# microsoft/ANCE

Measured on AMD Instinct MI355X. Metric: passages_encoded_per_sec, higher is better.
Workload: dtype f16 pair operands on the fp16 MFMA, f32 accumulate (fp32-grade: <= 2e-5 from the reference's fp32 forward); 1 GPU; MS MARCO passage 8841823 x 768-d, roberta-base rdot_nll FirstP seq_len=128, encode + brute-force IP top-200 (BASELINE configs[1]); encode_block_per_gpu=16384, query_block=32768, layers=12, parallelism=dp1 (corpus rows sharded, top-k all-to-all by query owner + merge)

## Files before the change

ance_amd/_lib.py:

```python
import ctypes
import os
import subprocess

_HERE = os.path.dirname(os.path.abspath(__file__))
LIB_PATH = os.environ.get("ANCE_AMD_LIB") or os.path.join(_HERE, "libance_amd.so")
CSRC = os.path.join(_HERE, "csrc")

ANCE_OK = 0
ANCE_E_INVALID = -1
ABI_VERSION = 7

c_i32p = ctypes.POINTER(ctypes.c_int32)
c_i64p = ctypes.POINTER(ctypes.c_int64)
c_f32p = ctypes.POINTER(ctypes.c_float)


class AnceEncoderDesc(ctypes.Structure):
    _fields_ = [
        ("arch", ctypes.c_int32), ("n_layers", ctypes.c_int32), ("hidden", ctypes.c_int32),
        ("n_heads", ctypes.c_int32), ("intermediate", ctypes.c_int32), ("vocab_size", ctypes.c_int32),
        ("max_position", ctypes.c_int32), ("pad_token_id", ctypes.c_int32), ("ln_eps", ctypes.c_float),
        ("has_head", ctypes.c_int32), ("max_seq_len", ctypes.c_int32), ("max_tokens", ctypes.c_int32),
        ("precision", ctypes.c_int32),
    ]


class AnceGemmDebugArgs(ctypes.Structure):
    _fields_ = [
        ("a", ctypes.c_void_p), ("b", ctypes.c_void_p), ("lda", ctypes.c_int32), ("ldb", ctypes.c_int32),
        ("M", ctypes.c_int32), ("N", ctypes.c_int32), ("K", ctypes.c_int32),
        ("bias", ctypes.c_void_p), ("csum", ctypes.c_void_p), ("part_in", ctypes.c_void_p), ("ln_eps", ctypes.c_float),
        ("tok_lo", ctypes.c_void_p), ("scale", ctypes.c_float), ("scale_cols", ctypes.c_int32), ("col_map", ctypes.c_void_p),
        ("n_valid", ctypes.c_int32), ("ldc", ctypes.c_int32), ("out", ctypes.c_void_p), ("res_hi", ctypes.c_void_p),
        ("res_lo", ctypes.c_void_p), ("res_gamma", ctypes.c_void_p), ("res_beta", ctypes.c_void_p), ("out_lo", ctypes.c_void_p),
        ("part_out", ctypes.c_void_p), ("ldr", ctypes.c_int32), ("wscale_inv", ctypes.c_void_p), ("n_split", ctypes.c_int32),
    ]


class AnceAttnDebugArgs(ctypes.Structure):
    _fields_ = [
        ("kind", ctypes.c_int32), ("n_heads", ctypes.c_int32), ("n_seq", ctypes.c_int32), ("max_seq_len", ctypes.c_int32),
        ("cls_only", ctypes.c_int32), ("q_compact", ctypes.c_int32), ("h_desc", ctypes.c_void_p), ("d_desc", ctypes.c_void_p),
        ("d_desc_bytes", ctypes.c_int64), ("qk", ctypes.c_void_p), ("ld_qk", ctypes.c_int32), ("qk_rows", ctypes.c_int32),
        ("vt", ctypes.c_void_p), ("ld_vt", ctypes.c_int32), ("ctx", ctypes.c_void_p), ("ld_ctx", ctypes.c_int32),
        ("ctx_rows", ctypes.c_int32),
    ]


class AnceLambTensor(ctypes.Structure):
    _fields_ = [("p", ctypes.c_void_p), ("g", ctypes.c_void_p), ("m", ctypes.c_void_p), ("v", ctypes.c_void_p),
                ("numel", ctypes.c_int64), ("group", ctypes.c_int32), ("reserved", ctypes.c_int32)]


class AnceAdamwTensor(ctypes.Structure):
    _fields_ = [("p", ctypes.c_void_p), ("g", ctypes.c_void_p), ("m", ctypes.c_void_p), ("v", ctypes.c_void_p),
                ("step", ctypes.c_void_p), ("numel", ctypes.c_int64), ("group", ctypes.c_int32), ("reserved", ctypes.c_int32)]


class AnceLambGroup(ctypes.Structure):
    _fields_ = [("lr", ctypes.c_double), ("beta1", ctypes.c_double), ("beta2", ctypes.c_double), ("eps", ctypes.c_double),
                ("weight_decay", ctypes.c_double)]


class AnceGatherSegment(ctypes.Structure):
    _fields_ = [("d_records", ctypes.c_void_p), ("n_records", ctypes.c_int64), ("d_index", ctypes.c_void_p),
                ("n_index", ctypes.c_int64), ("d_ids", ctypes.c_void_p), ("d_mask", ctypes.c_void_p), ("d_types", ctypes.c_void_p),
                ("L", ctypes.c_int32), ("mask_rule", ctypes.c_int32), ("type_rule", ctypes.c_int32), ("reserved", ctypes.c_int32)]


class AnceAttnTrainArgs(ctypes.Structure):
    _fields_ = [("q", ctypes.c_void_p), ("k", ctypes.c_void_p), ("v", ctypes.c_void_p), ("ctx", ctypes.c_void_p),
                ("ld_q", ctypes.c_int32), ("ld_k", ctypes.c_int32), ("ld_v", ctypes.c_int32), ("ld_ctx", ctypes.c_int32),
                ("d_seq_first", ctypes.c_void_p), ("d_seq_len", ctypes.c_void_p), ("n_seq", ctypes.c_int32),
                ("max_seq_len", ctypes.c_int32), ("n_rows", ctypes.c_int32), ("n_heads", ctypes.c_int32),
                ("seq_rows", ctypes.c_int32), ("reserved", ctypes.c_int32),
                ("dropout_p", ctypes.c_float), ("training", ctypes.c_int32), ("seed", ctypes.c_uint64), ("offset", ctypes.c_uint64),
                ("d_workspace", ctypes.c_void_p), ("workspace_bytes", ctypes.c_size_t)]


class AnceAttnGradArgs(ctypes.Structure):
    _fields_ = [("dctx", ctypes.c_void_p), ("dq", ctypes.c_void_p), ("dk", ctypes.c_void_p), ("dv", ctypes.c_void_p),
                ("ld_dctx", ctypes.c_int32), ("ld_dq", ctypes.c_int32), ("ld_dk", ctypes.c_int32), ("ld_dv", ctypes.c_int32)]


ANCE_DTYPE_F32, ANCE_DTYPE_F16, ANCE_DTYPE_BF16 = 0, 1, 2


class AnceAttn16Args(ctypes.Structure):
    _fields_ = [("q", ctypes.c_void_p), ("k", ctypes.c_void_p), ("v", ctypes.c_void_p), ("ctx", ctypes.c_void_p),
                ("ld_q", ctypes.c_int32), ("ld_k", ctypes.c_int32), ("ld_v", ctypes.c_int32), ("ld_ctx", ctypes.c_int32),
                ("d_seq_first", ctypes.c_void_p), ("d_seq_len", ctypes.c_void_p), ("n_seq", ctypes.c_int32),
                ("max_seq_len", ctypes.c_int32), ("n_rows", ctypes.c_int32), ("n_heads", ctypes.c_int32),
                ("seq_rows", ctypes.c_int32), ("dtype", ctypes.c_int32),
                ("dropout_p", ctypes.c_float), ("training", ctypes.c_int32), ("seed", ctypes.c_uint64), ("offset", ctypes.c_uint64),
                ("d_workspace", ctypes.c_void_p), ("workspace_bytes", ctypes.c_size_t)]


class AnceAttn16GradArgs(ctypes.Structure):
    _fields_ = [("dctx", ctypes.c_void_p), ("dq", ctypes.c_void_p), ("dk", ctypes.c_void_p), ("dv", ctypes.c_void_p),
                ("ld_dctx", ctypes.c_int32), ("ld_dq", ctypes.c_int32), ("ld_dk", ctypes.c_int32), ("ld_dv", ctypes.c_int32)]


class AnceLayerTailArgs(ctypes.Structure):
    _fields_ = [("x", ctypes.c_void_p), ("res", ctypes.c_void_p), ("bias", ctypes.c_void_p), ("gamma", ctypes.c_void_p),
                ("beta", ctypes.c_void_p), ("y", ctypes.c_void_p), ("ld_x", ctypes.c_int32), ("ld_res", ctypes.c_int32),
                ("ld_y", ctypes.c_int32), ("H", ctypes.c_int32), ("n_rows", ctypes.c_int32), ("eps", ctypes.c_float),
                ("dropout_p", ctypes.c_float), ("training", ctypes.c_int32), ("seed", ctypes.c_uint64), ("offset", ctypes.c_uint64),
                ("d_workspace", ctypes.c_void_p), ("workspace_bytes", ctypes.c_size_t)]


class AnceLayerTailGradArgs(ctypes.Structure):
    _fields_ = [("dy", ctypes.c_void_p), ("dx", ctypes.c_void_p), ("dres", ctypes.c_void_p), ("dgamma", ctypes.c_void_p),
                ("dbeta", ctypes.c_void_p), ("dbias", ctypes.c_void_p), ("ld_dy", ctypes.c_int32), ("ld_dx", ctypes.c_int32),
                ("ld_dres", ctypes.c_int32), ("reserved", ctypes.c_int32)]


class AnceBiasGeluArgs(ctypes.Structure):
    _fields_ = [("x", ctypes.c_void_p), ("bias", ctypes.c_void_p), ("y", ctypes.c_void_p), ("ld_x", ctypes.c_int32),
                ("ld_y", ctypes.c_int32), ("N", ctypes.c_int32), ("n_rows", ctypes.c_int32), ("d_workspace", ctypes.c_void_p),
                ("workspace_bytes", ctypes.c_size_t)]


class AnceBiasGeluGradArgs(ctypes.Structure):
    _fields_ = [("dy", ctypes.c_void_p), ("dx", ctypes.c_void_p), ("dbias", ctypes.c_void_p), ("ld_dy", ctypes.c_int32),
                ("ld_dx", ctypes.c_int32)]


class AnceLayerTail16Args(ctypes.Structure):
    _fields_ = [("x", ctypes.c_void_p), ("res", ctypes.c_void_p), ("bias", ctypes.c_void_p), ("gamma", ctypes.c_void_p),
                ("beta", ctypes.c_void_p), ("y", ctypes.c_void_p), ("y16", ctypes.c_void_p), ("ld_x", ctypes.c_int32),
                ("ld_res", ctypes.c_int32), ("ld_y", ctypes.c_int32), ("ld_y16", ctypes.c_int32), ("H", ctypes.c_int32),
                ("n_rows", ctypes.c_int32), ("dtype", ctypes.c_int32), ("eps", ctypes.c_float), ("dropout_p", ctypes.c_float),
                ("training", ctypes.c_int32), ("seed", ctypes.c_uint64), ("offset", ctypes.c_uint64),
                ("d_workspace", ctypes.c_void_p), ("workspace_bytes", ctypes.c_size_t)]


class AnceLayerTail16GradArgs(ctypes.Structure):
    _fields_ = [("dy", ctypes.c_void_p), ("dy16", ctypes.c_void_p), ("dx", ctypes.c_void_p), ("dres", ctypes.c_void_p),
                ("dgamma", ctypes.c_void_p), ("dbeta", ctypes.c_void_p), ("dbias", ctypes.c_void_p), ("ld_dy", ctypes.c_int32),
                ("ld_dy16", ctypes.c_int32), ("ld_dx", ctypes.c_int32), ("ld_dres", ctypes.c_int32)]


class AnceBiasGelu16Args(ctypes.Structure):
    _fields_ = [("x", ctypes.c_void_p), ("bias", ctypes.c_void_p), ("y", ctypes.c_void_p), ("ld_x", ctypes.c_int32),
                ("ld_y", ctypes.c_int32), ("N", ctypes.c_int32), ("n_rows", ctypes.c_int32), ("dtype", ctypes.c_int32),
                ("reserved", ctypes.c_int32), ("d_workspace", ctypes.c_void_p), ("workspace_bytes", ctypes.c_size_t)]


class AnceBiasGelu16GradArgs(ctypes.Structure):
    _fields_ = [("dy", ctypes.c_void_p), ("dx", ctypes.c_void_p), ("dbias", ctypes.c_void_p), ("ld_dy", ctypes.c_int32),
                ("ld_dx", ctypes.c_int32)]


class AnceEmbedArgs(ctypes.Structure):
    _fields_ = [("ids", ctypes.c_void_p), ("type_ids", ctypes.c_void_p), ("word", ctypes.c_void_p), ("pos", ctypes.c_void_p),
                ("type", ctypes.c_void_p), ("gamma", ctypes.c_void_p), ("beta", ctypes.c_void_p), ("y", ctypes.c_void_p),
                ("positions", ctypes.c_void_p), ("n_seq", ctypes.c_int32), ("L", ctypes.c_int32), ("H", ctypes.c_int32),
                ("vocab", ctypes.c_int32), ("max_pos", ctypes.c_int32), ("n_types", ctypes.c_int32),
                ("position_mode", ctypes.c_int32), ("padding_idx", ctypes.c_int32), ("eps", ctypes.c_float),
                ("dropout_p", ctypes.c_float), ("training", ctypes.c_int32), ("reserved", ctypes.c_int32),
                ("seed", ctypes.c_uint64), ("offset", ctypes.c_uint64), ("d_workspace", ctypes.c_void_p),
                ("workspace_bytes", ctypes.c_size_t)]


class AnceEmbedGradArgs(ctypes.Structure):
    _fields_ = [("dy", ctypes.c_void_p), ("dword", ctypes.c_void_p), ("dpos", ctypes.c_void_p), ("dtype", ctypes.c_void_p),
                ("dgamma", ctypes.c_void_p), ("dbeta", ctypes.c_void_p), ("word_keys", ctypes.c_void_p), ("word_perm", ctypes.c_void_p),
                ("pos_keys", ctypes.c_void_p), ("pos_perm", ctypes.c_void_p), ("type_keys", ctypes.c_void_p),
                ("type_perm", ctypes.c_void_p)]


class AncePackArgs(ctypes.Structure):
    _fields_ = [("ids", ctypes.c_void_p), ("type_ids", ctypes.c_void_p), ("d_seq_len", ctypes.c_void_p), ("d_seq_off", ctypes.c_void_p),
                ("d_seq_kept", ctypes.c_void_p), ("d_dropped", ctypes.c_void_p), ("packed_ids", ctypes.c_void_p),
                ("packed_type_ids", ctypes.c_void_p), ("packed_positions", ctypes.c_void_p), ("n_seq", ctypes.c_int32),
                ("L", ctypes.c_int32), ("rows", ctypes.c_int32), ("position_mode", ctypes.c_int32), ("padding_idx", ctypes.c_int32),
                ("vocab", ctypes.c_int32), ("max_pos", ctypes.c_int32), ("reserved", ctypes.c_int32)]


class AnceFirstRowsArgs(ctypes.Structure):
    _fields_ = [("rows_matrix", ctypes.c_void_p), ("first", ctypes.c_void_p), ("d_seq_off", ctypes.c_void_p),
                ("d_seq_kept", ctypes.c_void_p), ("ld_rows", ctypes.c_int32), ("ld_first", ctypes.c_int32), ("n_seq", ctypes.c_int32),
                ("rows", ctypes.c_int32), ("H", ctypes.c_int32), ("dtype", ctypes.c_int32)]


class AncePackedGatherSegment(ctypes.Structure):
    _fields_ = [("d_records", ctypes.c_void_p), ("n_records", ctypes.c_int64), ("d_index", ctypes.c_void_p),
                ("n_index", ctypes.c_int64), ("d_cum", ctypes.c_void_p), ("packed_ids", ctypes.c_void_p),
                ("packed_positions", ctypes.c_void_p), ("d_seq_off", ctypes.c_void_p), ("d_seq_kept", ctypes.c_void_p),
                ("d_dropped", ctypes.c_void_p), ("L", ctypes.c_int32), ("chunk_len", ctypes.c_int32), ("rows", ctypes.c_int32),
                ("position_mode", ctypes.c_int32), ("padding_idx", ctypes.c_int32), ("vocab", ctypes.c_int32),
                ("max_pos", ctypes.c_int32), ("reserved", ctypes.c_int32)]


EMBED_SEGMENT_CHUNK = 64
EMBED_POSITION_MODES = {"absolute": 0, "roberta": 1}

LAYER_TAIL_ROWS_PER_WORKGROUP = 16

GATHER_MASK_LENGTH, GATHER_MASK_NONZERO = 0, 1
GATHER_TYPES_ZERO, GATHER_TYPES_LENGTH = 0, 1
GATHER_REFERENCE, GATHER_WIDE = 0, 1

PRECISION_CODES = {None: 0, "split": 1, "fp16": 2, "fp32": 3}
PRECISION_NAMES = {1: "split", 2: "fp16", 3: "fp32"}


SYMBOLS = {
    "ance_abi_version": (ctypes.c_int, []),
    "ance_last_error": (ctypes.c_char_p, []),
    "ance_profile_enable": (None, [ctypes.c_int]),
    "ance_profile_read": (ctypes.c_int, [ctypes.POINTER(ctypes.c_double), ctypes.POINTER(ctypes.c_double),
                                         ctypes.POINTER(ctypes.c_longlong), ctypes.c_int]),
    "ance_ip_topk_workspace_bytes": (ctypes.c_size_t, [ctypes.c_int64, ctypes.c_int64, ctypes.c_int, ctypes.c_int]),
    "ance_ip_topk": (ctypes.c_int, [ctypes.c_void_p, ctypes.c_int64, ctypes.c_int64, ctypes.c_void_p, ctypes.c_int64,
                                    ctypes.c_int, ctypes.c_int, ctypes.c_void_p, ctypes.c_void_p, ctypes.c_void_p,
                                    ctypes.c_size_t, ctypes.c_void_p]),
    "ance_ip_topk_scan_workspace_bytes": (ctypes.c_size_t, [ctypes.c_int64, ctypes.c_int64, ctypes.c_int, ctypes.c_int]),
    "ance_ip_topk_scan": (ctypes.c_int, [ctypes.c_void_p, ctypes.c_int64, ctypes.c_int64, ctypes.c_void_p, ctypes.c_int64,
                                         ctypes.c_int, ctypes.c_int, ctypes.c_void_p, ctypes.c_void_p, ctypes.c_void_p,
                                         ctypes.c_size_t, ctypes.c_void_p]),
    "ance_ip_index_bytes": (ctypes.c_size_t, [ctypes.c_int64, ctypes.c_int]),
    "ance_ip_index_build": (ctypes.c_int, [ctypes.c_void_p, ctypes.c_int64, ctypes.c_int, ctypes.c_void_p, ctypes.c_size_t,
                                           ctypes.c_void_p]),
    "ance_ip_topk_indexed_workspace_bytes": (ctypes.c_size_t, [ctypes.c_int64, ctypes.c_int64, ctypes.c_int, ctypes.c_int]),
    "ance_ip_topk_indexed": (ctypes.c_int, [ctypes.c_void_p, ctypes.c_int64, ctypes.c_int64, ctypes.c_void_p, ctypes.c_void_p,
                                            ctypes.c_int64, ctypes.c_int, ctypes.c_int, ctypes.c_void_p, ctypes.c_void_p,
                                            ctypes.c_void_p, ctypes.c_size_t, ctypes.c_void_p]),
    "ance_topk_merge_workspace_bytes": (ctypes.c_size_t, [ctypes.c_int, ctypes.c_int64, ctypes.c_int]),
    "ance_topk_merge": (ctypes.c_int, [ctypes.c_void_p, ctypes.c_void_p, ctypes.c_int, ctypes.c_int64, ctypes.c_int,
                                       ctypes.c_void_p, ctypes.c_void_p, ctypes.c_void_p, ctypes.c_size_t,
                                       ctypes.c_void_p]),
    "ance_ip_score_rows": (ctypes.c_int, [ctypes.c_void_p, ctypes.c_int64, ctypes.c_void_p, ctypes.c_int64, ctypes.c_int,
                                          ctypes.c_void_p, ctypes.c_void_p, ctypes.c_void_p, ctypes.c_void_p]),
    "ance_encoder_weight_bytes": (ctypes.c_size_t, [ctypes.POINTER(AnceEncoderDesc)]),
    "ance_encoder_workspace_bytes": (ctypes.c_size_t, [ctypes.POINTER(AnceEncoderDesc)]),
    "ance_encoder_create": (ctypes.c_int, [ctypes.POINTER(AnceEncoderDesc), ctypes.POINTER(ctypes.c_void_p),
                                           ctypes.c_int, ctypes.c_void_p, ctypes.c_size_t, ctypes.c_void_p,
                                           ctypes.c_size_t, ctypes.c_void_p, ctypes.POINTER(ctypes.c_void_p)]),
    "ance_encoder_destroy": (None, [ctypes.c_void_p]),
    "ance_encoder_precision": (ctypes.c_int, [ctypes.c_void_p]),
    "ance_encoder_range_faults": (ctypes.c_int, [ctypes.c_void_p, ctypes.c_void_p, ctypes.c_int, ctypes.c_void_p]),
    "ance_encode_records": (ctypes.c_int, [ctypes.c_void_p, ctypes.c_void_p, ctypes.c_void_p, ctypes.c_int64,
                                           ctypes.c_int, ctypes.c_int, ctypes.c_void_p, ctypes.c_void_p]),
    "ance_encode_ids": (ctypes.c_int, [ctypes.c_void_p, ctypes.c_void_p, ctypes.c_int64, ctypes.c_void_p,
                                       ctypes.c_void_p, ctypes.c_int64, ctypes.c_int, ctypes.c_int, ctypes.c_void_p,
                                       ctypes.c_void_p]),
    "ance_encoder_flops_per_sequence": (ctypes.c_double, [ctypes.c_int]),
    "ance_host_py_shuffle": (ctypes.c_int, [ctypes.c_void_p, ctypes.c_int64, ctypes.c_void_p]),
    "ance_host_select_negatives": (ctypes.c_int, [ctypes.c_void_p, ctypes.c_void_p, ctypes.c_int64, ctypes.c_int,
                                                  ctypes.c_void_p, ctypes.c_int64, ctypes.c_void_p, ctypes.c_void_p,
                                                  ctypes.c_int, ctypes.c_int, ctypes.c_int, ctypes.c_void_p,
                                                  ctypes.c_void_p, ctypes.POINTER(ctypes.c_double)]),
    "ance_host_write_ann_training": (ctypes.c_int, [ctypes.c_char_p, ctypes.c_void_p, ctypes.c_int64, ctypes.c_void_p,
                                                    ctypes.c_void_p, ctypes.c_void_p, ctypes.c_void_p, ctypes.c_void_p,
                                                    ctypes.c_int, ctypes.POINTER(ctypes.c_int64)]),
    "ance_reload_env": (None, []),
    "ance_debug_search_stamps": (None, [ctypes.c_void_p]),
    "ance_debug_gemm": (ctypes.c_int, [ctypes.c_int, ctypes.c_int, ctypes.c_void_p, ctypes.c_void_p, ctypes.c_int,
                                       ctypes.c_int, ctypes.c_int, ctypes.c_void_p, ctypes.c_void_p, ctypes.c_void_p,
                                       ctypes.c_void_p]),
    "ance_search_bad_image_calls": (ctypes.c_int, [ctypes.POINTER(ctypes.c_ulonglong)]),
    "ance_nll_forward": (ctypes.c_int, [ctypes.c_void_p, ctypes.c_void_p, ctypes.c_void_p, ctypes.c_void_p, ctypes.c_void_p,
                                        ctypes.c_int64, ctypes.c_int, ctypes.c_int, ctypes.c_void_p, ctypes.c_void_p, ctypes.c_void_p,
                                        ctypes.c_void_p]),
    "ance_debug_gemm_split": (ctypes.c_int, [ctypes.c_int, ctypes.c_void_p, ctypes.c_void_p, ctypes.c_int, ctypes.c_int, ctypes.c_int,
                                             ctypes.c_void_p, ctypes.c_void_p, ctypes.c_void_p, ctypes.c_void_p, ctypes.c_float,
                                             ctypes.c_void_p, ctypes.c_void_p, ctypes.c_void_p, ctypes.c_void_p, ctypes.c_void_p]),
    "ance_debug_gemm_hw": (ctypes.c_int, [ctypes.c_int, ctypes.c_int, ctypes.POINTER(AnceGemmDebugArgs), ctypes.c_void_p]),
    "ance_debug_attention": (ctypes.c_int, [ctypes.POINTER(AnceAttnDebugArgs), ctypes.c_void_p]),
    "ance_lamb_workspace_bytes": (ctypes.c_size_t, [ctypes.c_int, ctypes.c_int, ctypes.c_int64]),
    "ance_lamb_step": (ctypes.c_int, [ctypes.POINTER(AnceLambTensor), ctypes.c_int, ctypes.POINTER(AnceLambGroup), ctypes.c_int,
                                      ctypes.c_int, ctypes.c_void_p, ctypes.c_void_p, ctypes.c_size_t, ctypes.c_void_p]),
    "ance_lamb_clipped_workspace_bytes": (ctypes.c_size_t, [ctypes.c_int, ctypes.c_int, ctypes.c_int64]),
    "ance_lamb_step_clipped": (ctypes.c_int, [ctypes.POINTER(AnceLambTensor), ctypes.c_int, ctypes.POINTER(AnceLambGroup), ctypes.c_int,
                                              ctypes.c_int, ctypes.c_double, ctypes.c_void_p, ctypes.c_void_p, ctypes.c_void_p,
                                              ctypes.c_size_t, ctypes.c_void_p]),
    "ance_lamb_amp_workspace_bytes": (ctypes.c_size_t, [ctypes.c_int, ctypes.c_int, ctypes.c_int64]),
    "ance_lamb_step_amp": (ctypes.c_int, [ctypes.POINTER(AnceLambTensor), ctypes.c_int, ctypes.POINTER(AnceLambGroup), ctypes.c_int,
                                          ctypes.c_int, ctypes.c_double, ctypes.c_void_p, ctypes.c_void_p, ctypes.c_void_p,
                                          ctypes.c_void_p, ctypes.c_void_p, ctypes.c_void_p, ctypes.c_void_p, ctypes.c_size_t,
                                          ctypes.c_void_p]),
    "ance_adamw_workspace_bytes": (ctypes.c_size_t, [ctypes.c_int, ctypes.c_int, ctypes.c_int64, ctypes.c_int]),
    "ance_adamw_step": (ctypes.c_int, [ctypes.POINTER(AnceAdamwTensor), ctypes.c_int, ctypes.POINTER(AnceLambGroup), ctypes.c_int,
                                       ctypes.c_int, ctypes.c_double, ctypes.c_void_p, ctypes.c_void_p, ctypes.c_void_p,
                                       ctypes.c_void_p, ctypes.c_void_p, ctypes.c_size_t, ctypes.c_void_p]),
    "ance_nll_backward": (ctypes.c_int, [ctypes.c_void_p, ctypes.c_void_p, ctypes.c_void_p, ctypes.c_void_p, ctypes.c_void_p,
                                         ctypes.c_int64, ctypes.c_int, ctypes.c_int, ctypes.c_void_p, ctypes.c_void_p, ctypes.c_void_p,
                                         ctypes.c_void_p, ctypes.c_void_p]),
    "ance_inbatch_nll_workspace_bytes": (ctypes.c_size_t, [ctypes.c_int64, ctypes.c_int64, ctypes.c_int]),
    "ance_inbatch_nll_forward": (ctypes.c_int, [ctypes.c_void_p, ctypes.c_void_p, ctypes.c_void_p, ctypes.c_int64, ctypes.c_int64,
                                                ctypes.c_int, ctypes.c_void_p, ctypes.c_void_p, ctypes.c_void_p, ctypes.c_size_t,
                                                ctypes.c_void_p]),
    "ance_inbatch_nll_backward": (ctypes.c_int, [ctypes.c_void_p, ctypes.c_void_p, ctypes.c_void_p, ctypes.c_int64, ctypes.c_int64,
                                                 ctypes.c_int, ctypes.c_void_p, ctypes.c_void_p, ctypes.c_void_p, ctypes.c_void_p,
                                                 ctypes.c_size_t, ctypes.c_void_p]),
    "ance_gather_batch": (ctypes.c_int, [ctypes.POINTER(AnceGatherSegment), ctypes.c_int, ctypes.c_int64, ctypes.c_int64, ctypes.c_int,
                                         ctypes.c_void_p]),
    "ance_record_lengths": (ctypes.c_int, [ctypes.c_void_p, ctypes.c_int64, ctypes.c_int, ctypes.c_int, ctypes.c_int, ctypes.c_void_p,
                                           ctypes.c_void_p]),
    "ance_gather_batch_packed": (ctypes.c_int, [ctypes.POINTER(AncePackedGatherSegment), ctypes.c_int, ctypes.c_int64, ctypes.c_int64,
                                                ctypes.c_void_p, ctypes.c_void_p]),
    "ance_attention_workspace_bytes": (ctypes.c_size_t, [ctypes.c_int64, ctypes.c_int]),
    "ance_attention_forward": (ctypes.c_int, [ctypes.POINTER(AnceAttnTrainArgs), ctypes.c_void_p]),
    "ance_attention_backward": (ctypes.c_int, [ctypes.POINTER(AnceAttnTrainArgs), ctypes.POINTER(AnceAttnGradArgs), ctypes.c_void_p]),
    "ance_attention16_workspace_bytes": (ctypes.c_size_t, [ctypes.c_int64, ctypes.c_int]),
    "ance_attention16_forward": (ctypes.c_int, [ctypes.POINTER(AnceAttn16Args), ctypes.c_void_p]),
    "ance_attention16_backward": (ctypes.c_int, [ctypes.POINTER(AnceAttn16Args), ctypes.POINTER(AnceAttn16GradArgs), ctypes.c_void_p]),
    "ance_layer_tail_rows_per_workgroup": (ctypes.c_int, []),
    "ance_layer_tail_workspace_bytes": (ctypes.c_size_t, [ctypes.c_int64, ctypes.c_int]),
    "ance_bias_gelu_workspace_bytes": (ctypes.c_size_t, [ctypes.c_int64, ctypes.c_int]),
    "ance_layer_tail_forward": (ctypes.c_int, [ctypes.POINTER(AnceLayerTailArgs), ctypes.c_void_p]),
    "ance_layer_tail_backward": (ctypes.c_int, [ctypes.POINTER(AnceLayerTailArgs), ctypes.POINTER(AnceLayerTailGradArgs), ctypes.c_void_p]),
    "ance_bias_gelu_forward": (ctypes.c_int, [ctypes.POINTER(AnceBiasGeluArgs), ctypes.c_void_p]),
    "ance_bias_gelu_backward": (ctypes.c_int, [ctypes.POINTER(AnceBiasGeluArgs), ctypes.POINTER(AnceBiasGeluGradArgs), ctypes.c_void_p]),
    "ance_layer_tail16_workspace_bytes": (ctypes.c_size_t, [ctypes.c_int64, ctypes.c_int]),
    "ance_bias_gelu16_workspace_bytes": (ctypes.c_size_t, [ctypes.c_int64, ctypes.c_int]),
    "ance_layer_tail16_forward": (ctypes.c_int, [ctypes.POINTER(AnceLayerTail16Args), ctypes.c_void_p]),
    "ance_layer_tail16_backward": (ctypes.c_int, [ctypes.POINTER(AnceLayerTail16Args), ctypes.POINTER(AnceLayerTail16GradArgs), ctypes.c_void_p]),
    "ance_bias_gelu16_forward": (ctypes.c_int, [ctypes.POINTER(AnceBiasGelu16Args), ctypes.c_void_p]),
    "ance_bias_gelu16_backward": (ctypes.c_int, [ctypes.POINTER(AnceBiasGelu16Args), ctypes.POINTER(AnceBiasGelu16GradArgs), ctypes.c_void_p]),
    "ance_embed_segment_chunk": (ctypes.c_int, []),
    "ance_embed_workspace_bytes": (ctypes.c_size_t, [ctypes.c_int64, ctypes.c_int]),
    "ance_embed_forward": (ctypes.c_int, [ctypes.POINTER(AnceEmbedArgs), ctypes.c_void_p]),
    "ance_embed_backward": (ctypes.c_int, [ctypes.POINTER(AnceEmbedArgs), ctypes.POINTER(AnceEmbedGradArgs), ctypes.c_void_p]),
    "ance_attention_forward_dstream": (ctypes.c_int, [ctypes.POINTER(AnceAttnTrainArgs), ctypes.c_void_p, ctypes.c_void_p]),
    "ance_attention_backward_dstream": (ctypes.c_int, [ctypes.POINTER(AnceAttnTrainArgs), ctypes.POINTER(AnceAttnGradArgs), ctypes.c_void_p, ctypes.c_void_p]),
    "ance_attention16_forward_dstream": (ctypes.c_int, [ctypes.POINTER(AnceAttn16Args), ctypes.c_void_p, ctypes.c_void_p]),
    "ance_attention16_backward_dstream": (ctypes.c_int, [ctypes.POINTER(AnceAttn16Args), ctypes.POINTER(AnceAttn16GradArgs), ctypes.c_void_p, ctypes.c_void_p]),
    "ance_attention_row0_workspace_bytes": (ctypes.c_size_t, [ctypes.c_int64, ctypes.c_int]),
    "ance_attention_row0_forward": (ctypes.c_int, [ctypes.POINTER(AnceAttn16Args), ctypes.c_void_p]),
    "ance_attention_row0_backward": (ctypes.c_int, [ctypes.POINTER(AnceAttn16Args), ctypes.POINTER(AnceAttn16GradArgs), ctypes.c_void_p]),
    "ance_attention_row0_forward_dstream": (ctypes.c_int, [ctypes.POINTER(AnceAttn16Args), ctypes.c_void_p, ctypes.c_void_p]),
    "ance_attention_row0_backward_dstream": (ctypes.c_int, [ctypes.POINTER(AnceAttn16Args), ctypes.POINTER(AnceAttn16GradArgs), ctypes.c_void_p, ctypes.c_void_p]),
    "ance_layer_tail_forward_dstream": (ctypes.c_int, [ctypes.POINTER(AnceLayerTailArgs), ctypes.c_void_p, ctypes.c_void_p]),
    "ance_layer_tail_backward_dstream": (ctypes.c_int, [ctypes.POINTER(AnceLayerTailArgs), ctypes.POINTER(AnceLayerTailGradArgs), ctypes.c_void_p, ctypes.c_void_p]),
    "ance_layer_tail16_forward_dstream": (ctypes.c_int, [ctypes.POINTER(AnceLayerTail16Args), ctypes.c_void_p, ctypes.c_void_p]),
    "ance_layer_tail16_backward_dstream": (ctypes.c_int, [ctypes.POINTER(AnceLayerTail16Args), ctypes.POINTER(AnceLayerTail16GradArgs), ctypes.c_void_p, ctypes.c_void_p]),
    "ance_embed_forward_dstream": (ctypes.c_int, [ctypes.POINTER(AnceEmbedArgs), ctypes.c_void_p, ctypes.c_void_p]),
    "ance_embed_backward_dstream": (ctypes.c_int, [ctypes.POINTER(AnceEmbedArgs), ctypes.POINTER(AnceEmbedGradArgs), ctypes.c_void_p, ctypes.c_void_p]),
    "ance_pack_tokens": (ctypes.c_int, [ctypes.POINTER(AncePackArgs), ctypes.c_void_p]),
    "ance_embed_rows_forward": (ctypes.c_int, [ctypes.POINTER(AnceEmbedArgs), ctypes.c_void_p]),
    "ance_embed_rows_backward": (ctypes.c_int, [ctypes.POINTER(AnceEmbedArgs), ctypes.POINTER(AnceEmbedGradArgs), ctypes.c_void_p]),
    "ance_embed_rows_forward_dstream": (ctypes.c_int, [ctypes.POINTER(AnceEmbedArgs), ctypes.c_void_p, ctypes.c_void_p]),
    "ance_embed_rows_backward_dstream": (ctypes.c_int, [ctypes.POINTER(AnceEmbedArgs), ctypes.POINTER(AnceEmbedGradArgs), ctypes.c_void_p, ctypes.c_void_p]),
    "ance_first_rows_gather": (ctypes.c_int, [ctypes.POINTER(AnceFirstRowsArgs), ctypes.c_void_p]),
    "ance_first_rows_scatter": (ctypes.c_int, [ctypes.POINTER(AnceFirstRowsArgs), ctypes.c_void_p]),
    "ance_dropout_stream_advance": (ctypes.c_int, [ctypes.c_void_p, ctypes.c_uint64, ctypes.c_void_p]),
    "ance_lamb_plan_table_bytes": (ctypes.c_size_t, [ctypes.c_int, ctypes.c_int, ctypes.c_int64]),
    "ance_lamb_plan_build": (ctypes.c_int, [ctypes.POINTER(AnceLambTensor), ctypes.c_int, ctypes.POINTER(AnceLambGroup), ctypes.c_void_p,
                                            ctypes.c_int, ctypes.c_void_p, ctypes.c_size_t, ctypes.POINTER(ctypes.c_int64),
                                            ctypes.POINTER(ctypes.c_size_t)]),
    "ance_lamb_step_planned": (ctypes.c_int, [ctypes.c_int, ctypes.c_int, ctypes.c_int64, ctypes.c_int, ctypes.c_double, ctypes.c_void_p,
                                              ctypes.c_void_p, ctypes.c_void_p, ctypes.c_void_p, ctypes.c_void_p, ctypes.c_void_p,
                                              ctypes.c_void_p, ctypes.c_size_t, ctypes.c_void_p]),
    "ance_adamw_plan_table_bytes": (ctypes.c_size_t, [ctypes.c_int, ctypes.c_int, ctypes.c_int64]),
    "ance_adamw_plan_build": (ctypes.c_int, [ctypes.POINTER(AnceAdamwTensor), ctypes.c_int, ctypes.POINTER(AnceLambGroup), ctypes.c_void_p,
                                             ctypes.c_int, ctypes.c_void_p, ctypes.c_size_t, ctypes.POINTER(ctypes.c_int64),
                                             ctypes.POINTER(ctypes.c_size_t)]),
    "ance_adamw_step_planned": (ctypes.c_int, [ctypes.c_int, ctypes.c_int, ctypes.c_int64, ctypes.c_int, ctypes.c_double, ctypes.c_void_p,
                                               ctypes.c_void_p, ctypes.c_void_p, ctypes.c_void_p, ctypes.c_void_p, ctypes.c_size_t,
                                               ctypes.c_void_p]),
    "ance_debug_staging_sends": (ctypes.c_longlong, []),
    "ance_linear_warmup_step": (ctypes.c_int, [ctypes.c_void_p, ctypes.c_void_p, ctypes.c_void_p, ctypes.c_int, ctypes.c_int64,
                                               ctypes.c_int64, ctypes.c_void_p]),
    "ance_pair_layout": (None, [ctypes.c_int, ctypes.c_int, ctypes.POINTER(ctypes.c_int), ctypes.POINTER(ctypes.c_int),
                                ctypes.POINTER(ctypes.c_float)]),
}

_lib = None


class AnceLibraryError(RuntimeError):
    pass


class AnceRangeError(AnceLibraryError):
    """The split (default) arithmetic met a value outside the fp16 range -- its stated precondition -- or produced NaN rows."""


def build(verbose=False, force=False):
    cmd = ["make", "-C", CSRC, "-j8"] + (["-B"] if force else [])
    res = subprocess.run(cmd, stdout=subprocess.PIPE, stderr=subprocess.STDOUT, text=True)
    if verbose or res.returncode != 0:
        print(res.stdout)
    if res.returncode != 0:
        raise AnceLibraryError("hipcc build of libance_amd.so failed")
    return LIB_PATH


def lib():
    global _lib
    if _lib is not None:
        return _lib
    if not os.path.exists(LIB_PATH):
        raise AnceLibraryError(
            "%s not found: the HIP extension is required (run `python -c 'import __graft_entry__ as g; g.build()'` "
            "or `make -C ance_amd/csrc`); there is no CPU fallback" % LIB_PATH)
    try:
        import torch
    except Exception:
        pass
    try:
        L = ctypes.CDLL(LIB_PATH)
    except OSError as e:
        raise AnceLibraryError("cannot load %s: %s" % (LIB_PATH, e))
    for name, (res, args) in SYMBOLS.items():
        try:
            fn = getattr(L, name)
        except AttributeError:
            raise AnceLibraryError("%s does not export %s" % (LIB_PATH, name))
        fn.restype = res
        fn.argtypes = args
    if L.ance_abi_version() != ABI_VERSION:
        raise AnceLibraryError("ABI version mismatch: library %d, binding %d" % (L.ance_abi_version(), ABI_VERSION))
    _lib = L
    return L


def reload_env():
    lib().ance_reload_env()


def check(rc, what):
    if rc != ANCE_OK:
        msg = lib().ance_last_error()
        raise AnceLibraryError("%s failed (%d): %s" % (what, rc, msg.decode() if msg else ""))


PROFILE_CATEGORIES = ("plan", "embed_ln", "gemm_qk", "gemm_vt", "attention", "gemm_attn_out", "layernorm",
                      "gemm_ffn1", "gemm_ffn2", "head", "ip_topk_scan", "topk_finalize", "ip_topk_rescore")


def profile_enable(on=True):
    lib().ance_profile_enable(1 if on else 0)


def profile_read():
    n = len(PROFILE_CATEGORIES)
    ms = (ctypes.c_double * n)()
    work = (ctypes.c_double * n)()
    cnt = (ctypes.c_longlong * n)()
    lib().ance_profile_read(ms, work, cnt, n)
    return {c: dict(ms=ms[i], work=work[i], count=int(cnt[i])) for i, c in enumerate(PROFILE_CATEGORIES)}


def current_stream_ptr():
    import torch
    return ctypes.c_void_p(torch.cuda.current_stream().cuda_stream)


def require_cuda_tensor(t, dtype, what):
    import torch
    if not isinstance(t, torch.Tensor) or not t.is_cuda:
        raise AnceLibraryError("%s must be a CUDA(HIP) tensor" % what)
    if t.dtype != dtype:
        raise AnceLibraryError("%s must have dtype %s, got %s" % (what, dtype, t.dtype))
    if not t.is_contiguous():
        raise AnceLibraryError("%s must be contiguous" % what)
    return t
```

ance_amd/csrc/attention.h:

```cpp
#pragma once
#include "common.h"

namespace ance {

struct AttnArgs {
    const _Float16 *qk;
    const _Float16 *vt;
    _Float16 *ctx;
    const int4 *desc;
    int ld_qk, ld_vt, ld_ctx;
    int n_heads;
    int cls_only;
    int q_compact;
};

size_t attention_lds_bytes(int max_seq_len, int n_waves);
int launch_attention_split(const float *qkv, _Float16 *ctx_pair, const int4 *desc, int n_seq, int n_heads, int max_seq_len,
                           int cls_only, hipStream_t stream);
int launch_attention(const AttnArgs &args, int n_seq, int max_seq_len, hipStream_t stream);

}
```

ance_amd/csrc/attention.hip:

```cpp
#include <stdio.h>
#include <stdlib.h>
#include <type_traits>
#include <vector>

#include "common.h"
#include "attention.h"
#include "precise32.h"

namespace ance {
namespace {

constexpr int HD = 64;

__device__ __forceinline__ int kswz(int row, int chunk) { return chunk ^ ((row >> 1) & 7); }

__device__ __forceinline__ void wave_lds_sync() {
    __builtin_amdgcn_fence(__ATOMIC_SEQ_CST, "wavefront");
    __builtin_amdgcn_wave_barrier();
}

__device__ __forceinline__ void attend_qblock(const AttnArgs &A, const _Float16 *Ks, const _Float16 *Vs, const f16x8 (&qf)[4], int s,
                                              int h, int tok0, int T, int Tk, int vld, int qb0, int q_end, int g, int i,
                                              _Float16 *slab) {
    const int nkb = Tk >> 5;
    float m_run = -INFINITY, l_run = 0.0f;
    f32x16 o0 = {0}, o1 = {0};
    for (int kb = 0; kb < nkb; ++kb) {
        const int krow = kb * 32 + i;
        const int ksw = (krow >> 1) & 7;
        f32x16 st = {0};
#pragma unroll
        for (int sx = 0; sx < 4; ++sx) {
            const f16x8 kf = *reinterpret_cast<const f16x8 *>(Ks + krow * HD + (((4 * g + sx) ^ ksw) * 8));
            st = __builtin_amdgcn_mfma_f32_32x32x16_f16(kf, qf[sx], st, 0, 0, 0);
        }
        const int key_base = kb * 32 + 4 * g;
        float bm = -INFINITY;
#pragma unroll
        for (int r = 0; r < 16; ++r) {
            const int key = key_base + (r & 3) + 8 * (r >> 2);
            if (kb == nkb - 1) st[r] = key < T ? st[r] : -INFINITY;
            bm = fmaxf(bm, st[r]);
        }
        bm = fmaxf(bm, __shfl_xor(bm, 32));
        const float m_new = fmaxf(m_run, bm);
        const float alpha = __builtin_amdgcn_exp2f(m_run - m_new);
        float psum = 0.0f;
        float p[16];
#pragma unroll
        for (int r = 0; r < 16; ++r) {
            p[r] = __builtin_amdgcn_exp2f(st[r] - m_new);
            psum += p[r];
        }
        l_run = l_run * alpha + psum;
        m_run = m_new;
#pragma unroll
        for (int r = 0; r < 16; ++r) {
            o0[r] *= alpha;
            o1[r] *= alpha;
        }
#pragma unroll
        for (int u = 0; u < 2; ++u) {
            f16x8 pf;
#pragma unroll
            for (int j = 0; j < 8; ++j) pf[j] = (_Float16)p[8 * u + j];
            const int kc = kb * 32 + 16 * u + 4 * g;
            const _Float16 *v0 = Vs + i * vld + kc;
            const _Float16 *v1 = Vs + (i + 32) * vld + kc;
            const f16x4 a0 = *reinterpret_cast<const f16x4 *>(v0);
            const f16x4 a1 = *reinterpret_cast<const f16x4 *>(v0 + 8);
            const f16x4 c0 = *reinterpret_cast<const f16x4 *>(v1);
            const f16x4 c1 = *reinterpret_cast<const f16x4 *>(v1 + 8);
            const f16x8 vf0 = {a0[0], a0[1], a0[2], a0[3], a1[0], a1[1], a1[2], a1[3]};
            const f16x8 vf1 = {c0[0], c0[1], c0[2], c0[3], c1[0], c1[1], c1[2], c1[3]};
            o0 = __builtin_amdgcn_mfma_f32_32x32x16_f16(vf0, pf, o0, 0, 0, 0);
            o1 = __builtin_amdgcn_mfma_f32_32x32x16_f16(vf1, pf, o1, 0, 0, 0);
        }
    }
    const float l_tot = l_run + __shfl_xor(l_run, 32);
    const float inv = 1.0f / l_tot;
    {
        const int l = g * 32 + i;
#pragma unroll
        for (int db = 0; db < 2; ++db) {
            const f32x16 &o = db == 0 ? o0 : o1;
#pragma unroll
            for (int rq = 0; rq < 4; ++rq) {
                const f16x4 v = {(_Float16)(o[4 * rq + 0] * inv), (_Float16)(o[4 * rq + 1] * inv),
                                 (_Float16)(o[4 * rq + 2] * inv), (_Float16)(o[4 * rq + 3] * inv)};
                *reinterpret_cast<f16x4 *>(slab + i * HD + kswz(i, db * 4 + rq) * 8 + 4 * g) = v;
            }
        }
        wave_lds_sync();
#pragma unroll
        for (int j = 0; j < 4; ++j) {
            const int row = j * 8 + (l >> 3), ch = l & 7;
            if (qb0 + row < q_end) {
                const size_t orow = A.cls_only ? (size_t)s : (size_t)(tok0 + qb0 + row);
                *reinterpret_cast<f16x8 *>(A.ctx + orow * A.ld_ctx + h * HD + ch * 8) =
                    *reinterpret_cast<const f16x8 *>(slab + row * HD + kswz(row, ch) * 8);
            }
        }
        wave_lds_sync();
    }
}

template <int NW>
__global__ void __launch_bounds__(64 * NW, 3) attention_kernel(const AttnArgs A) {
    extern __shared__ __attribute__((aligned(16))) float smem_f[];
    constexpr int NT = 64 * NW;
    const int u = blockIdx.x / A.n_heads;
    const int h = blockIdx.x - u * A.n_heads;
    const int4 dsc = A.desc[u];
    const int tok0 = dsc.x;
    const int T = dsc.y;
    const int vcol0 = dsc.z;
    const int s = dsc.w;
    const int Tk = (T + 31) & ~31;
    const int vld = Tk + 4;
    _Float16 *Ks = reinterpret_cast<_Float16 *>(smem_f);
    _Float16 *Vs = Ks + (size_t)Tk * HD;

    const int tid = threadIdx.x;
    const int w = tid >> 6, l = tid & 63, g = l >> 5, i = l & 31;
    const int H = A.n_heads * HD;
    _Float16 *slab = Vs + (size_t)HD * vld + w * (32 * HD);

    const int q_end = A.cls_only ? 1 : T;
    f16x8 qf[4];
    auto q_row = [&](int r) { return A.q_compact ? (size_t)s : (size_t)(tok0 + min(r, T - 1)); };
    auto q_request = [&](int qb0) {
#pragma unroll
        for (int j = 0; j < 4; ++j) {
            const int row = j * 8 + (l >> 3);
            qf[j] = *reinterpret_cast<const f16x8 *>(A.qk + q_row(qb0 + row) * A.ld_qk + h * HD + (l & 7) * 8);
        }
    };
    auto q_to_fragments = [&]() {
#pragma unroll
        for (int j = 0; j < 4; ++j) {
            const int row = j * 8 + (l >> 3);
            *reinterpret_cast<f16x8 *>(slab + row * HD + kswz(row, l & 7) * 8) = qf[j];
        }
        wave_lds_sync();
#pragma unroll
        for (int sx = 0; sx < 4; ++sx) qf[sx] = *reinterpret_cast<const f16x8 *>(slab + i * HD + kswz(i, 4 * g + sx) * 8);
        wave_lds_sync();
    };
    if (w * 32 < q_end) q_request(w * 32);

    {
        const _Float16 *kbase = A.qk + (size_t)tok0 * A.ld_qk + H + h * HD + (tid & 7) * 8;
        const _Float16 *vbase = A.vt + (size_t)(h * HD) * A.ld_vt + vcol0;
        for (int base = 0; base < Tk; base += 32 * NW) {
            f16x8 kv[4], vv[4];
#pragma unroll
            for (int j = 0; j < 4; ++j) {
                const int row = base + j * (8 * NW) + (tid >> 3);
                const int ev = j * NT + tid, dd = ev / (4 * NW);
                const int key0 = base + (ev - dd * (4 * NW)) * 8;
                kv[j] = f16x8{0, 0, 0, 0, 0, 0, 0, 0};
                vv[j] = f16x8{0, 0, 0, 0, 0, 0, 0, 0};
                if (row < T) kv[j] = *reinterpret_cast<const f16x8 *>(kbase + (size_t)row * A.ld_qk);
                if (key0 < T) vv[j] = *reinterpret_cast<const f16x8 *>(vbase + (size_t)dd * A.ld_vt + key0);
            }
#pragma unroll
            for (int j = 0; j < 4; ++j) {
                const int row = base + j * (8 * NW) + (tid >> 3);
                const int ev = j * NT + tid, dd = ev / (4 * NW);
                const int key0 = base + (ev - dd * (4 * NW)) * 8;
                if (row < Tk) *reinterpret_cast<f16x8 *>(Ks + row * HD + kswz(row, tid & 7) * 8) = kv[j];
                if (key0 < Tk) {
                    if (key0 + 8 > T) {
#pragma unroll
                        for (int e = 0; e < 8; ++e)
                            if (key0 + e >= T) vv[j][e] = (_Float16)0.0f;
                    }
                    _Float16 *dst = Vs + dd * vld + key0;
                    *reinterpret_cast<f16x4 *>(dst) = f16x4{vv[j][0], vv[j][1], vv[j][2], vv[j][3]};
                    *reinterpret_cast<f16x4 *>(dst + 4) = f16x4{vv[j][4], vv[j][5], vv[j][6], vv[j][7]};
                }
            }
        }
    }
    if (w * 32 < q_end) q_to_fragments();
    __syncthreads();

    for (int qb0 = w * 32; qb0 < q_end; qb0 += 32 * NW) {
        if (qb0 != w * 32) {
            q_request(qb0);
            q_to_fragments();
        }
        attend_qblock(A, Ks, Vs, qf, s, h, tok0, T, Tk, vld, qb0, q_end, g, i, slab);
    }
}



constexpr int VS = HD;
__device__ __forceinline__ int vswz(int key, int d) { return d ^ (((key >> 1) & 1) << 5); }
typedef short s16x4_t __attribute__((ext_vector_type(4)));
typedef s16x4_t __attribute__((address_space(3))) lds_s16x4_t;
__device__ __forceinline__ f16x4 lds_read_tr16(const _Float16 *p) {
    const s16x4_t v = __builtin_amdgcn_ds_read_tr16_b64_v4i16((lds_s16x4_t *)(p));
    return __builtin_bit_cast(f16x4, v);
}

__device__ __forceinline__ void permlane32_swap(float &x, float &y) {
    asm volatile("s_nop 1\n\tv_permlane32_swap_b32 %0, %1\n\ts_nop 1" : "+v"(x), "+v"(y));
}

template <int NW>
__global__ void __launch_bounds__(64 * NW, 2) attention_split_kernel(const float *qkv, _Float16 *ctx_pair, const int4 *desc, int n_heads,
                                                                     int cls_only, int kchunk) {
    extern __shared__ __attribute__((aligned(16))) float smem_f[];
    const int u = blockIdx.x / n_heads;
    const int h = blockIdx.x - u * n_heads;
    const int4 dsc = desc[u];
    const int tok0 = dsc.x, T = dsc.y, s = dsc.w;
    const int Tk = (T + 31) & ~31;
    const int kc = Tk < kchunk ? Tk : kchunk;
    _Float16 *Kh = reinterpret_cast<_Float16 *>(smem_f);
    _Float16 *Kl = Kh + (size_t)kc * HD;
    _Float16 *Vh = Kl + (size_t)kc * HD;
    _Float16 *Vl = Vh + (size_t)kc * VS;
    const int tid = threadIdx.x;
    const int w = tid >> 6, l = tid & 63, g = l >> 5, i = l & 31;
    constexpr int NT = 64 * NW;
    const int ld = 3 * n_heads * HD;
    constexpr float SC = 2048.0f, SI = 1.0f / 2048.0f;
    auto stage = [&](int k0, auto unr_tag) {
        constexpr int UNR = decltype(unr_tag)::value;
        for (int e0 = tid; e0 < kc * 8; e0 += UNR * NT) {
            f32x4 kv[UNR][4];
#pragma unroll
            for (int it = 0; it < UNR; ++it) {
                const int e = e0 + it * NT;
                const int kl_ = e >> 3, ch = e & 7, key = k0 + kl_;
#pragma unroll
                for (int q = 0; q < 4; ++q) kv[it][q] = f32x4{0.f, 0.f, 0.f, 0.f};
                if (e < kc * 8 && key < T) {
                    const float *kp = qkv + (size_t)(tok0 + key) * ld + n_heads * HD + h * HD + ch * 8;
                    kv[it][0] = *reinterpret_cast<const f32x4 *>(kp);
                    kv[it][1] = *reinterpret_cast<const f32x4 *>(kp + 4);
                    kv[it][2] = *reinterpret_cast<const f32x4 *>(kp + n_heads * HD);
                    kv[it][3] = *reinterpret_cast<const f32x4 *>(kp + n_heads * HD + 4);
                }
            }
#pragma unroll
            for (int it = 0; it < UNR; ++it) {
                const int e = e0 + it * NT;
                if (e >= kc * 8) break;
                const int kl_ = e >> 3, ch = e & 7;
                const f32x4 k0v = kv[it][0], k1v = kv[it][1], v0 = kv[it][2], v1 = kv[it][3];
                const f16x4 a0 = cvt_f16x4_pinned(k0v), a1 = cvt_f16x4_pinned(k1v), b0 = cvt_f16x4_pinned(v0), b1 = cvt_f16x4_pinned(v1);
                f16x8 kh, kl;
#pragma unroll
                for (int j = 0; j < 4; ++j) {
                    kh[j] = a0[j]; kh[4 + j] = a1[j];
                    kl[j] = (_Float16)((k0v[j] - (float)a0[j]) * SC);
                    kl[4 + j] = (_Float16)((k1v[j] - (float)a1[j]) * SC);
                }
                *reinterpret_cast<f16x8 *>(Kh + kl_ * HD + kswz(kl_, ch) * 8) = kh;
                *reinterpret_cast<f16x8 *>(Kl + kl_ * HD + kswz(kl_, ch) * 8) = kl;
                f16x8 vh, vl;
#pragma unroll
                for (int j = 0; j < 4; ++j) {
                    vh[j] = b0[j]; vh[4 + j] = b1[j];
                    vl[j] = (_Float16)((v0[j] - (float)b0[j]) * SC);
                    vl[4 + j] = (_Float16)((v1[j] - (float)b1[j]) * SC);
                }
                *reinterpret_cast<f16x8 *>(Vh + kl_ * VS + vswz(kl_, ch * 8)) = vh;
                *reinterpret_cast<f16x8 *>(Vl + kl_ * VS + vswz(kl_, ch * 8)) = vl;
            }
        }
    };
    const bool single = Tk <= kc;
    const int q_end = cls_only ? 1 : T;
    const float qscale = 0.125f * 1.44269504088896340736f;
    for (int qp0 = 0; qp0 < q_end; qp0 += 32 * NW) {
        const int qb0 = qp0 + w * 32;
        const bool active = qb0 < q_end;
        f16x8 qh[4], ql[4];
        {
            const float *qp = qkv + (cls_only ? (size_t)s : (size_t)(tok0 + min(qb0 + i, T - 1))) * ld + h * HD + 32 * g;
            f32x4 xq[8];
#pragma unroll
            for (int sx = 0; sx < 8; ++sx) xq[sx] = *reinterpret_cast<const f32x4 *>(qp + sx * 4);
            if (single && qp0 == 0) {
                stage(0, std::integral_constant<int, 4>{});
                __syncthreads();
            }
#pragma unroll
            for (int sx = 0; sx < 4; ++sx) {
                f32x4 x0 = xq[2 * sx], x1 = xq[2 * sx + 1];
                x0 = x0 * qscale;
                x1 = x1 * qscale;
                const f16x4 a0 = cvt_f16x4_pinned(x0), a1 = cvt_f16x4_pinned(x1);
#pragma unroll
                for (int j = 0; j < 4; ++j) {
                    qh[sx][j] = a0[j]; qh[sx][4 + j] = a1[j];
                    ql[sx][j] = (_Float16)((x0[j] - (float)a0[j]) * SC);
                    ql[sx][4 + j] = (_Float16)((x1[j] - (float)a1[j]) * SC);
                }
            }
        }
        float m_run = -INFINITY, l_run = 0.0f;
        f32x16 om0 = {0}, om1 = {0}, oc0 = {0}, oc1 = {0};
        for (int k0 = 0; k0 < Tk; k0 += kc) {
            if (!single) {
                __syncthreads();
                stage(k0, std::integral_constant<int, 1>{});
                __syncthreads();
            }
            if (!active) continue;
            const int nkb = min(kc, Tk - k0) >> 5;
            for (int kb = 0; kb < nkb; ++kb) {
                const int krow = kb * 32 + i;
                const int ksw = (krow >> 1) & 7;
                f32x16 st = {0};
                f16x8 kfh[4];
#pragma unroll
                for (int sx = 0; sx < 4; ++sx) {
                    kfh[sx] = *reinterpret_cast<const f16x8 *>(Kh + krow * HD + (((4 * g + sx) ^ ksw) * 8));
                    const f16x8 kfl = *reinterpret_cast<const f16x8 *>(Kl + krow * HD + (((4 * g + sx) ^ ksw) * 8));
                    st = __builtin_amdgcn_mfma_f32_32x32x16_f16(kfh[sx], ql[sx], st, 0, 0, 0);
                    st = __builtin_amdgcn_mfma_f32_32x32x16_f16(kfl, qh[sx], st, 0, 0, 0);
                }
                st *= SI;
#pragma unroll
                for (int sx = 0; sx < 4; ++sx) st = __builtin_amdgcn_mfma_f32_32x32x16_f16(kfh[sx], qh[sx], st, 0, 0, 0);
                const int key_base = k0 + kb * 32 + 4 * g;
                float bm = -INFINITY;
#pragma unroll
                for (int r = 0; r < 16; ++r) {
                    const int key = key_base + (r & 3) + 8 * (r >> 2);
                    if (k0 + kb * 32 + 32 > T) st[r] = key < T ? st[r] : -INFINITY;
                    bm = fmaxf(bm, st[r]);
                }
                bm = fmaxf(bm, __shfl_xor(bm, 32));
                const float m_new = fmaxf(m_run, bm);
                const float alpha = __builtin_amdgcn_exp2f(m_run - m_new);
                float psum = 0.0f;
                float p[16];
#pragma unroll
                for (int r = 0; r < 16; ++r) {
                    p[r] = __builtin_amdgcn_exp2f(st[r] - m_new);
                    psum += p[r];
                }
                l_run = l_run * alpha + psum;
                m_run = m_new;
                om0 *= alpha; om1 *= alpha; oc0 *= alpha; oc1 *= alpha;
#pragma unroll
                for (int uu = 0; uu < 2; ++uu) {
                    const f16x4 h0 = cvt_f16x4_pinned(f32x4{p[8 * uu], p[8 * uu + 1], p[8 * uu + 2], p[8 * uu + 3]});
                    const f16x4 h1 = cvt_f16x4_pinned(f32x4{p[8 * uu + 4], p[8 * uu + 5], p[8 * uu + 6], p[8 * uu + 7]});
                    f16x8 ph, pl;
#pragma unroll
                    for (int j = 0; j < 4; ++j) {
                        ph[j] = h0[j]; ph[4 + j] = h1[j];
                        pl[j] = (_Float16)((p[8 * uu + j] - (float)h0[j]) * SC);
                        pl[4 + j] = (_Float16)((p[8 * uu + 4 + j] - (float)h1[j]) * SC);
                    }
                    const int kcol = kb * 32 + 16 * uu + 4 * g;
                    auto vfrag = [&](const _Float16 *V, int row) {
                        const int q = l & 15, key = kcol + (q >> 2);
                        const _Float16 *vp = V + key * VS + vswz(key, (row - i) + 16 * ((l >> 4) & 1) + 4 * (q & 3));
                        const f16x4 a = lds_read_tr16(vp), b = lds_read_tr16(vp + 8 * VS);
                        return f16x8{a[0], a[1], a[2], a[3], b[0], b[1], b[2], b[3]};
                    };
                    const f16x8 v0h = vfrag(Vh, i), v1h = vfrag(Vh, i + 32), v0l = vfrag(Vl, i), v1l = vfrag(Vl, i + 32);
                    oc0 = __builtin_amdgcn_mfma_f32_32x32x16_f16(v0h, pl, oc0, 0, 0, 0);
                    oc0 = __builtin_amdgcn_mfma_f32_32x32x16_f16(v0l, ph, oc0, 0, 0, 0);
                    oc1 = __builtin_amdgcn_mfma_f32_32x32x16_f16(v1h, pl, oc1, 0, 0, 0);
                    oc1 = __builtin_amdgcn_mfma_f32_32x32x16_f16(v1l, ph, oc1, 0, 0, 0);
                    om0 = __builtin_amdgcn_mfma_f32_32x32x16_f16(v0h, ph, om0, 0, 0, 0);
                    om1 = __builtin_amdgcn_mfma_f32_32x32x16_f16(v1h, ph, om1, 0, 0, 0);
                }
            }
        }
        if (!active) continue;
        const float l_tot = l_run + __shfl_xor(l_run, 32);
        const float inv = 1.0f / l_tot;
        {
            const bool store = qb0 + i < q_end;
            const size_t orow = cls_only ? (size_t)s : (size_t)(tok0 + min(qb0 + i, T - 1));
            _Float16 *orp = ctx_pair + orow * (size_t)(2 * n_heads * HD);
#pragma unroll
            for (int db = 0; db < 2; ++db) {
                const f32x16 &om = db == 0 ? om0 : om1;
                const f32x16 &oc = db == 0 ? oc0 : oc1;
#pragma unroll
                for (int k2 = 0; k2 < 2; ++k2) {
                    f32x4 va, vb;
#pragma unroll
                    for (int j = 0; j < 4; ++j) {
                        const float xa = __builtin_fmaf(oc[8 * k2 + j], SI, om[8 * k2 + j]) * inv;
                        const float xb = __builtin_fmaf(oc[8 * k2 + 4 + j], SI, om[8 * k2 + 4 + j]) * inv;
                        float sa = xa, sb = xb;
                        permlane32_swap(sa, sb);
                        va[j] = sa;
                        vb[j] = sb;
                    }
                    if (store) {
                        f16x4 ha, ra, hb, rb;
                        pair_split4(va, &ha, &ra);
                        pair_split4(vb, &hb, &rb);
                        const int n = h * HD + db * 32 + 16 * k2 + 8 * g;
                        *reinterpret_cast<f16x8 *>(orp + pair_hi_col(n, n_heads * HD)) = f16x8{ha[0], ha[1], ha[2], ha[3], hb[0], hb[1], hb[2], hb[3]};
                        *reinterpret_cast<f16x8 *>(orp + pair_lo_col(n, n_heads * HD)) = f16x8{ra[0], ra[1], ra[2], ra[3], rb[0], rb[1], rb[2], rb[3]};
                    }
                }
            }
        }
    }
}

}

size_t attention_split_lds_bytes(int max_seq_len) {
    const int Tk = (max_seq_len + 31) & ~31;
    return (size_t)2 * Tk * HD * 2 + (size_t)2 * Tk * VS * 2;
}

int launch_attention_split(const float *qkv, _Float16 *ctx_pair, const int4 *desc, int n_seq, int n_heads, int max_seq_len,
                           int cls_only, hipStream_t st) {
    if (n_seq <= 0) return ANCE_OK;
    const int Tk = (max_seq_len + 31) & ~31;
    const int kchunk = Tk <= 256 ? Tk : 256;
    const size_t lds = attention_split_lds_bytes(kchunk);
    int dev = 0;
    (void)hipGetDevice(&dev);
    static size_t attr_set[64] = {0};
    const bool tracked = dev >= 0 && dev < 64;
    if (!tracked || lds > __atomic_load_n(&attr_set[dev], __ATOMIC_ACQUIRE)) {
        if (hipFuncSetAttribute(reinterpret_cast<const void *>(attention_split_kernel<4>), hipFuncAttributeMaxDynamicSharedMemorySize,
                                (int)lds) != hipSuccess)
            return check_launch("attention_split attr");
        if (tracked) __atomic_store_n(&attr_set[dev], lds, __ATOMIC_RELEASE);
    }
    hipLaunchKernelGGL((attention_split_kernel<4>), dim3((unsigned)n_seq * n_heads), dim3(256), lds, st, qkv, ctx_pair, desc, n_heads,
                       cls_only, kchunk);
    return ANCE_OK;
}

size_t attention_lds_bytes(int max_seq_len, int n_waves) {
    const int Tk = (max_seq_len + 31) & ~31;
    return (size_t)Tk * HD * 2 + (size_t)HD * (Tk + 4) * 2 + (size_t)n_waves * 32 * HD * 2;
}

int launch_attention(const AttnArgs &A, int n_seq, int max_seq_len, hipStream_t st) {
    if (n_seq <= 0) return ANCE_OK;
    const size_t lds = attention_lds_bytes(max_seq_len, 4);
    if (lds > 160 * 1024) {
        set_last_error("attention: sequence too long for LDS");
        return ANCE_E_INVALID;
    }
    int dev = 0;
    (void)hipGetDevice(&dev);
    static size_t attr_set[64] = {0};
    const bool tracked = dev >= 0 && dev < 64;
    if (!tracked || lds > __atomic_load_n(&attr_set[dev], __ATOMIC_ACQUIRE)) {
        if (hipFuncSetAttribute(reinterpret_cast<const void *>(attention_kernel<4>),
                                hipFuncAttributeMaxDynamicSharedMemorySize, (int)lds) != hipSuccess)
            return check_launch("attention attr");
        if (tracked) __atomic_store_n(&attr_set[dev], lds, __ATOMIC_RELEASE);
    }
    hipLaunchKernelGGL((attention_kernel<4>), dim3((unsigned)n_seq * A.n_heads), dim3(256), lds, st, A);
    return ANCE_OK;
}

}

extern "C" int ance_debug_attention(const AnceAttnDebugArgs *a, void *stream) {
    using namespace ance;
    auto refuse = [](const char *why) {
        char buf[160];
        snprintf(buf, sizeof(buf), "ance_debug_attention: invalid argument (%s)", why);
        set_last_error(buf);
        return ANCE_E_INVALID;
    };
    if (!a) return refuse("null args");
    if (a->kind < 0 || a->kind > 2) return refuse("kind");
    if (a->n_heads != 12 && a->n_heads != 16) return refuse("n_heads");
    if (a->n_seq < 1 || a->n_seq > (1 << 20)) return refuse("n_seq");
    if (a->max_seq_len < 1 || a->max_seq_len > 512) return refuse("max_seq_len");
    if (!a->h_desc || !a->d_desc || !a->qk || !a->ctx || (a->kind == 0 && !a->vt)) return refuse("null pointer");
    const int64_t H = 64 * (int64_t)a->n_heads, n = a->n_seq;
    const int64_t desc_bytes = a->kind == 2 ? 4 * (n + 1) : 16 * n;
    if (a->d_desc_bytes < desc_bytes || (uintptr_t)a->d_desc % 16) return refuse("d_desc");
    if ((uintptr_t)a->qk % 16 || (uintptr_t)a->ctx % 16 || (a->kind == 0 && (uintptr_t)a->vt % 16)) return refuse("alignment");
    if (a->qk_rows < 1 || a->ctx_rows < 1) return refuse("rows");
    if (a->kind == 0) {
        if (a->ld_qk % 8 || a->ld_qk < 2 * H || a->ld_vt % 8 || a->ld_vt < 8 || a->ld_ctx % 8 || a->ld_ctx < H) return refuse("stride");
    } else {
        if (a->ld_qk != 3 * H || a->ld_ctx != (a->kind == 1 ? 2 * H : H)) return refuse("stride");
    }
    if (a->kind == 2 && (a->cls_only || a->q_compact)) return refuse("cls_only on kind 2");
    if (a->kind == 1 && a->q_compact != a->cls_only) return refuse("kind 1: q_compact != cls_only");
    if (a->kind == 0 && a->q_compact && !a->cls_only) return refuse("q_compact without cls_only");
    const int32_t *d = a->h_desc;
    if (a->kind == 2) {
        if (d[0] < 0) return refuse("tokens outside the allocation");
        for (int64_t s = 0; s < n; ++s) {
            const int64_t len = (int64_t)d[s + 1] - d[s];
            if (len < 1 || len > a->max_seq_len) return refuse("length");
        }
        if (d[n] > a->qk_rows || d[n] > a->ctx_rows) return refuse("tokens outside the allocation");
    } else {
        std::vector<char> seen((size_t)n, 0);
        const bool compact = a->cls_only && (a->q_compact || a->kind == 1);
        for (int64_t u = 0; u < n; ++u) {
            const int64_t tok0 = d[4 * u], len = d[4 * u + 1], vcol = d[4 * u + 2], s = d[4 * u + 3];
            if (len < 1 || len > a->max_seq_len) return refuse("length");
            if (s < 0 || s >= n || seen[(size_t)s]) return refuse("sequence index");
            seen[(size_t)s] = 1;
            if (tok0 < 0 || tok0 + len > a->qk_rows) return refuse("tokens outside the allocation");
            if (compact && s >= a->qk_rows) return refuse("Q row s past the allocation");
            if (a->cls_only ? s >= a->ctx_rows : tok0 + len > a->ctx_rows) return refuse("output row past the allocation");
            if (a->kind == 0 && (vcol < 0 || vcol % 8 || vcol + ((len + 7) & ~7) > a->ld_vt)) return refuse("V^T columns");
        }
    }
    hipStream_t st = (hipStream_t)stream;
    if (hipMemcpyAsync(a->d_desc, a->h_desc, (size_t)desc_bytes, hipMemcpyHostToDevice, st) != hipSuccess)
        return check_launch("ance_debug_attention: descriptors");
    int rc;
    if (a->kind == 0) {
        AttnArgs A;
        A.qk = (const _Float16 *)a->qk; A.vt = (const _Float16 *)a->vt; A.ctx = (_Float16 *)a->ctx; A.desc = (const int4 *)a->d_desc;
        A.ld_qk = a->ld_qk; A.ld_vt = a->ld_vt; A.ld_ctx = a->ld_ctx; A.n_heads = a->n_heads;
        A.cls_only = a->cls_only ? 1 : 0; A.q_compact = a->q_compact ? 1 : 0;
        rc = launch_attention(A, a->n_seq, a->max_seq_len, st);
    } else if (a->kind == 1) {
        rc = launch_attention_split((const float *)a->qk, (_Float16 *)a->ctx, (const int4 *)a->d_desc, a->n_seq, a->n_heads,
                                    a->max_seq_len, a->cls_only ? 1 : 0, st);
    } else {
        rc = launch_attention32((const float *)a->qk, (float *)a->ctx, (const int *)a->d_desc, a->n_seq, a->n_heads, st);
    }
    return rc ? rc : check_launch("ance_debug_attention");
}
```

ance_amd/csrc/common.h:

```cpp
#pragma once
#include <hip/hip_runtime.h>
#include <stdint.h>
#include <float.h>
#include <stdio.h>

#include "../../include/ance_amd.h"

typedef float f32x4 __attribute__((ext_vector_type(4)));
typedef float f32x16 __attribute__((ext_vector_type(16)));
typedef _Float16 f16x4 __attribute__((ext_vector_type(4)));
typedef _Float16 f16x8 __attribute__((ext_vector_type(8)));
typedef unsigned long long u64;

namespace ance {

void set_last_error(const char *msg);
int check_launch(const char *what);
inline int refuse(const char *fn, const char *why) {
    char buf[200];
    snprintf(buf, sizeof(buf), "%s: invalid argument (%s)", fn, why);
    set_last_error(buf);
    return ANCE_E_INVALID;
}

enum ProfCat {
    PC_PLAN = 0, PC_EMBED, PC_GEMM_QK, PC_GEMM_VT, PC_ATTN, PC_GEMM_OUT, PC_LN, PC_GEMM_FFN1, PC_GEMM_FFN2, PC_HEAD,
    PC_SCAN, PC_FINALIZE, PC_RESCORE, PC_COUNT
};
bool prof_enabled();
void prof_begin(int cat, hipStream_t st, double work);
void prof_end(hipStream_t st);
struct ProfScope {
    hipStream_t st;
    bool on;
    ProfScope(int cat, hipStream_t s, double work = 0.0) : st(s), on(prof_enabled()) {
        if (on) prof_begin(cat, st, work);
    }
    ~ProfScope() {
        if (on) prof_end(st);
    }
};

__host__ __device__ inline uint32_t order_f32(float s) {
    s = s + 0.0f;
    uint32_t u = __builtin_bit_cast(uint32_t, s);
    return (u & 0x80000000u) ? ~u : (u | 0x80000000u);
}
__host__ __device__ inline float unorder_f32(uint32_t o) {
    uint32_t u = (o & 0x80000000u) ? (o & 0x7FFFFFFFu) : ~o;
    return __builtin_bit_cast(float, u);
}
__host__ __device__ inline u64 pack_key(float s, uint32_t row) {
    return ((u64)order_f32(s) << 32) | (u64)(0xFFFFFFFFu - row);
}
__host__ __device__ inline float key_score(u64 k) { return unorder_f32((uint32_t)(k >> 32)); }
__host__ __device__ inline uint32_t key_row(u64 k) { return 0xFFFFFFFFu - (uint32_t)(k & 0xFFFFFFFFull); }

__device__ __forceinline__ f16x4 cvt_f16x4_pinned(const f32x4 v) {
    f16x4 h = f16x4{(_Float16)v[0], (_Float16)v[1], (_Float16)v[2], (_Float16)v[3]};
    asm volatile("" : "+v"(h));
    return h;
}

constexpr float PAIR_LO_SCALE = 1.0f, PAIR_LO_INV = 1.0f;
__host__ __device__ __forceinline__ int pair_hi_col(int n, int W) { (void)W; return ((n >> 5) << 6) + (n & 31); }
__host__ __device__ __forceinline__ int pair_lo_col(int n, int W) { (void)W; return ((n >> 5) << 6) + (n & 31) + 32; }
__device__ __forceinline__ void pair_split4(const f32x4 v, f16x4 *hi, f16x4 *lo) {
#pragma clang fp contract(off)
    const f16x4 h = cvt_f16x4_pinned(v);
    *hi = h;
    *lo = f16x4{(_Float16)((v[0] - (float)h[0]) * PAIR_LO_SCALE), (_Float16)((v[1] - (float)h[1]) * PAIR_LO_SCALE),
                (_Float16)((v[2] - (float)h[2]) * PAIR_LO_SCALE), (_Float16)((v[3] - (float)h[3]) * PAIR_LO_SCALE)};
}
__device__ __forceinline__ void pair_store4(const f32x4 v, _Float16 *row, int W, int n) {
    f16x4 h, r;
    pair_split4(v, &h, &r);
    *reinterpret_cast<f16x4 *>(row + pair_hi_col(n, W)) = h;
    *reinterpret_cast<f16x4 *>(row + pair_lo_col(n, W)) = r;
}
__device__ __forceinline__ f32x4 pair_load4(const _Float16 *row, int W, int n) {
    const f16x4 h = *reinterpret_cast<const f16x4 *>(row + pair_hi_col(n, W)), r = *reinterpret_cast<const f16x4 *>(row + pair_lo_col(n, W));
    return f32x4{(float)h[0] + (float)r[0] * PAIR_LO_INV, (float)h[1] + (float)r[1] * PAIR_LO_INV, (float)h[2] + (float)r[2] * PAIR_LO_INV,
                 (float)h[3] + (float)r[3] * PAIR_LO_INV};
}

constexpr float RANGE_LIMIT = 65504.0f;
__device__ __forceinline__ void range_track4(const f32x4 v, float *mx) {
    float m = *mx;
    asm("v_max3_f32 %0, |%1|, |%2|, %0" : "+v"(m) : "v"(v[0]), "v"(v[1]));
    asm("v_max3_f32 %0, |%1|, |%2|, %0" : "+v"(m) : "v"(v[2]), "v"(v[3]));
    *mx = m;
}
__device__ __forceinline__ void range_report(float mx, unsigned *faults) {
    const u64 bad = __builtin_amdgcn_ballot_w64(!(mx <= RANGE_LIMIT));
    if (bad != 0 && faults != nullptr && (threadIdx.x & 63) == (unsigned)__builtin_ctzll(bad)) atomicAdd(faults, (unsigned)__builtin_popcountll(bad));
}

__device__ inline int lane_id() { return (int)(threadIdx.x & 63); }

inline size_t align_up(size_t v, size_t a) { return (v + a - 1) / a * a; }

inline int attr_device_bit() {
    int dev = 0;
    (void)hipGetDevice(&dev);
    return (dev < 0 || dev >= 63) ? -1 : dev;
}
inline bool attr_needed(unsigned long long *done) {
    const int bit = attr_device_bit();
    return bit < 0 || !(__atomic_load_n(done, __ATOMIC_ACQUIRE) & (1ull << bit));
}
inline void attr_mark(unsigned long long *done) {
    const int bit = attr_device_bit();
    if (bit >= 0) (void)__atomic_fetch_or(done, 1ull << bit, __ATOMIC_RELEASE);
}

}
```

ance_amd/csrc/encoder.hip:

```cpp
#include <stdlib.h>
#include <type_traits>
#include <vector>

#include "attention.h"
#include "common.h"
#include "encoder_kernels.h"
#include "encoder_plan.h"
#include "gemm_f16.h"
#include "precise32.h"

namespace ance {
namespace {

template <typename F>
auto with_hidden(int hidden, F &&f) {
    return hidden == 1024 ? f(std::integral_constant<int, 1024>()) : f(std::integral_constant<int, 768>());
}

constexpr int S_CAP_MAX = 8192;
constexpr int FETCH_CHUNK = 262144;
constexpr int MAX_LANES = 2;


bool precise_env() {
    const char *p = getenv("ANCE_ENCODER_PRECISE");
    return p && p[0] == '1';
}

bool split_env() {
    if (precise_env()) return false;
    const char *s = getenv("ANCE_ENCODER_SPLIT");
    if (s && s[0] == '1') return true;
    if (s && s[0] == '0') return false;
    const char *f = getenv("ANCE_ENCODER_FP16");
    return !(f && f[0] == '1');
}

int resolve_precision(const AnceEncoderDesc *d) {
    if (d->precision == ANCE_PRECISION_SPLIT || d->precision == ANCE_PRECISION_FP16 || d->precision == ANCE_PRECISION_FP32)
        return d->precision;
    if (precise_env()) return ANCE_PRECISION_FP32;
    return split_env() ? ANCE_PRECISION_SPLIT : ANCE_PRECISION_FP16;
}

struct LayerW {
    _Float16 *wqk, *wv, *wo, *w1, *w2;
    _Float16 *wqkv_s, *wo_s, *w1_s, *w2_s;
    float *bqkv_s, *cqkv_s, *b1_s, *c1_s;
    float *sc_s;
    float *bqk, *bv, *bo, *b1, *b2, *ln1w, *ln1b, *ln2w, *ln2b;
    float *cqk, *cv, *c1;
    float *wqkv32, *bqkv32, *wo32, *w132, *w232;
};

struct Arena {
    size_t off = 0;
    char *base = nullptr;
    template <typename T>
    T *take(size_t n) {
        T *p = base ? reinterpret_cast<T *>(base + off) : nullptr;
        off = align_up(off + n * sizeof(T), 256);
        return p;
    }
};

}
}

using namespace ance;

struct AnceEncoder {
    AnceEncoderDesc d;
    float *word, *pos, *type0, *eln_w, *eln_b;
    std::vector<LayerW> layers;
    float *head_w, *head_b, *norm_w, *norm_b;
    int tcap, vcap, scap;
    int *lens_fetch;
    unsigned *faults;
    struct Lane {
        int *seq_off, *seq_vtcol, *seq_len, *tok_id, *tok_pos, *tok_vtcol;
        int4 *desc;
        struct Fp16 {
            Rows<FORM_PLANES> xa, xb;
            _Float16 *qk, *vt, *ctx, *ffn;
            Rows<FORM_PLANES> cls(int S_pad, int H) const {
                _Float16 *const lo = ffn + (size_t)S_pad * H;
                return {ffn, lo, reinterpret_cast<float *>(lo + (size_t)S_pad * H)};
            }
        } f16;
        struct Split {
            Rows<FORM_PAIR> xa, xb;
            float *qkv;
            _Float16 *ctx, *ffn;
            Rows<FORM_PAIR> cls(int S_pad, int H) const { return {ffn, reinterpret_cast<float *>(ffn + (size_t)S_pad * 2 * H)}; }
        } sp;
        struct Fp32 {
            Rows<FORM_F32> xa, xb;
            float *h, *ha, *qkv, *ctx, *ffn;
        } f32;
    } lane[MAX_LANES];
    int n_lanes;
    hipStream_t side[MAX_LANES];
    hipEvent_t ev_fork, ev_join[MAX_LANES];
    std::vector<int32_t> host_lens;
    bool cls_tail;
    int mode;
};

namespace {

bool desc_ok(const AnceEncoderDesc *d) {
    if (!d || d->n_heads <= 0 || d->hidden != 64 * d->n_heads || (d->hidden != 768 && d->hidden != 1024)) return false;
    if (d->hidden == 1024 && (d->arch != ANCE_ARCH_ROBERTA || d->has_head != 1 || d->intermediate % 256 != 0)) return false;
    return d->intermediate > 0 && d->intermediate % 128 == 0 &&
           d->n_layers >= 1 && d->vocab_size > 0 && d->max_position > 0 && d->max_seq_len >= 1 &&
           d->max_seq_len <= 512 && d->max_tokens >= 512 && d->max_tokens % 256 == 0 && d->precision >= 0 && d->precision <= 3 &&
           (d->arch == ANCE_ARCH_ROBERTA || d->arch == ANCE_ARCH_BERT || d->arch == ANCE_ARCH_SEED);
}

void layout_weights(const AnceEncoderDesc *d, Arena &a, AnceEncoder *e) {
    const size_t I = d->intermediate;
    const int H = d->hidden, HP = 2 * H;
    const int mode = resolve_precision(d);
    float *word = a.take<float>((size_t)d->vocab_size * H);
    float *pos = a.take<float>((size_t)d->max_position * H);
    float *type0 = a.take<float>(H);
    float *ew = a.take<float>(H), *eb = a.take<float>(H);
    if (e) { e->word = word; e->pos = pos; e->type0 = type0; e->eln_w = ew; e->eln_b = eb; e->layers.resize(d->n_layers); }
    for (int i = 0; i < d->n_layers; ++i) {
        LayerW w;
        w.wqk = a.take<_Float16>((size_t)2 * H * H);
        w.bqk = a.take<float>(2 * H);
        w.wv = a.take<_Float16>((size_t)H * H);
        w.bv = a.take<float>(H);
        w.wo = a.take<_Float16>((size_t)H * H);
        w.bo = a.take<float>(H);
        w.ln1w = a.take<float>(H);
        w.ln1b = a.take<float>(H);
        w.w1 = a.take<_Float16>(I * H);
        w.b1 = a.take<float>(I);
        w.w2 = a.take<_Float16>((size_t)H * I);
        w.b2 = a.take<float>(H);
        w.ln2w = a.take<float>(H);
        w.ln2b = a.take<float>(H);
        w.cqk = a.take<float>(2 * H);
        w.cv = a.take<float>(H);
        w.c1 = a.take<float>(I);
        w.wqkv_s = w.wo_s = w.w1_s = w.w2_s = nullptr;
        w.bqkv_s = w.cqkv_s = w.b1_s = w.c1_s = w.sc_s = nullptr;
        if (mode == ANCE_PRECISION_SPLIT) {
            w.sc_s = a.take<float>(8);
            w.wqkv_s = a.take<_Float16>((size_t)3 * H * HP);
            w.bqkv_s = a.take<float>(3 * H);
            w.cqkv_s = a.take<float>(3 * H);
            w.wo_s = a.take<_Float16>((size_t)H * HP);
            w.w1_s = a.take<_Float16>(I * HP);
            w.b1_s = a.take<float>(I);
            w.c1_s = a.take<float>(I);
            w.w2_s = a.take<_Float16>((size_t)H * 2 * I);
        }
        w.wqkv32 = w.bqkv32 = w.wo32 = w.w132 = w.w232 = nullptr;
        if (mode == ANCE_PRECISION_FP32) {
            w.wqkv32 = a.take<float>((size_t)3 * H * H);
            w.bqkv32 = a.take<float>(3 * H);
            w.wo32 = a.take<float>((size_t)H * H);
            w.w132 = a.take<float>(I * H);
            w.w232 = a.take<float>((size_t)H * I);
        }
        if (e) e->layers[i] = w;
    }
    float *hw = nullptr, *hb = nullptr, *nw = nullptr, *nb = nullptr;
    if (d->has_head) {
        hw = a.take<float>((size_t)HEAD_OUT * H);
        hb = a.take<float>(HEAD_OUT);
        nw = a.take<float>(HEAD_OUT);
        nb = a.take<float>(HEAD_OUT);
    }
    if (e) { e->head_w = hw; e->head_b = hb; e->norm_w = nw; e->norm_b = nb; }
}

void layout_workspace(const AnceEncoderDesc *d, Arena &a, AnceEncoder *e) {
    const int tcap = d->max_tokens;
    const int scap = tcap < S_CAP_MAX ? tcap : S_CAP_MAX;
    const int vcap = (int)align_up((size_t)tcap + tcap / 4 + 256, 256);
    const int mode = resolve_precision(d);
    const size_t H = d->hidden, I = d->intermediate;
    unsigned *faults = a.take<unsigned>(64);
    int *lens_fetch = a.take<int>(FETCH_CHUNK);
    if (e) { e->tcap = tcap; e->scap = scap; e->vcap = vcap; e->lens_fetch = lens_fetch; e->faults = faults; }
    auto halves = [](float *p) { return reinterpret_cast<_Float16 *>(p); };
    for (int ln = 0; ln < MAX_LANES; ++ln) {
        AnceEncoder::Lane L;
        L.seq_off = a.take<int>(scap + 1); L.seq_vtcol = a.take<int>(scap); L.seq_len = a.take<int>(scap);
        L.tok_id = a.take<int>(tcap); L.tok_pos = a.take<int>(tcap); L.tok_vtcol = a.take<int>(tcap);
        L.desc = a.take<int4>(scap);
        float *const preB = a.take<float>(tcap * H), *const preA = a.take<float>(tcap * H);
        float *const statsA = a.take<float>((size_t)tcap * 2), *const statsB = a.take<float>((size_t)tcap * 2);
        (void)a.take<_Float16>(tcap * H);
        _Float16 *const qk16 = a.take<_Float16>(tcap * 2 * H);
        _Float16 *const vt16 = a.take<_Float16>(H * vcap);
        _Float16 *const ctx16 = a.take<_Float16>(tcap * H);
        _Float16 *const ffn16 = a.take<_Float16>(tcap * I);
        float *const partA = a.take<float>((size_t)tcap * PART_FLOATS), *const partB = a.take<float>((size_t)tcap * PART_FLOATS);
        const bool f32 = mode == ANCE_PRECISION_FP32, wide = f32 || mode == ANCE_PRECISION_SPLIT;
        float *const h32 = f32 ? a.take<float>(tcap * H) : nullptr, *const ha32 = f32 ? a.take<float>(tcap * H) : nullptr;
        float *const qkv32 = wide ? a.take<float>(tcap * 3 * H) : nullptr, *const ctx32 = wide ? a.take<float>(tcap * H) : nullptr;
        float *const ffn32 = wide ? a.take<float>(tcap * I) : nullptr;
        if (!e) continue;
        L.f16 = {{halves(preA), halves(preA) + tcap * H, partA}, {halves(preB), halves(preB) + tcap * H, partB}, qk16, vt16, ctx16, ffn16};
        L.sp = {{halves(preA), partA}, {halves(preB), partB}, qkv32, halves(ctx32), halves(ffn32)};
        L.f32 = {{preA, statsA}, {preB, statsB}, h32, ha32, qkv32, ctx32, ffn32};
        e->lane[ln] = L;
    }
}

void cvt16(const void *src, _Float16 *dst, size_t n, hipStream_t st) {
    const unsigned blocks = (unsigned)((n + 256 * 8 - 1) / (256 * 8));
    hipLaunchKernelGGL(cvt_f32_f16_kernel, dim3(blocks > 4096 ? 4096 : (blocks ? blocks : 1)), dim3(256), 0, st,
                       (const float *)src, dst, n);
}
void cpy32(const void *src, float *dst, size_t n, hipStream_t st) {
    (void)hipMemcpyAsync(dst, src, n * sizeof(float), hipMemcpyDeviceToDevice, st);
}

template <int H, int FORM>
void encoder_output(AnceEncoder *e, const AnceEncoder::Lane &LN, hipStream_t st, const MicroPlan &mb, float *out,
                    const Rows<FORM> &pre, int compact) {
    const AnceEncoderDesc &D = e->d;
    const LayerW &WL = e->layers[D.n_layers - 1];
    ProfScope ps(PC_HEAD, st);
    if (D.has_head) {
        hipLaunchKernelGGL((head_gemm_kernel<H, FORM>), dim3((mb.S + 31) / 32, HEAD_OUT / 128), dim3(256), HEAD_LDS_BYTES<H>, st, pre,
                           D.ln_eps, WL.ln2w, WL.ln2b, LN.seq_off, compact, mb.S, e->head_w, e->head_b, out);
        hipLaunchKernelGGL(head_ln_kernel, dim3((mb.S + 3) / 4), dim3(256), 0, st, out, mb.S, e->norm_w, e->norm_b, e->faults);
    } else {
        hipLaunchKernelGGL((head_kernel<H, FORM>), dim3(mb.S), dim3(256), 0, st, pre, D.ln_eps, WL.ln2w, WL.ln2b, LN.seq_off, compact,
                           out, e->faults);
    }
}

template <int H>
int forward_fp32(AnceEncoder *e, const AnceEncoder::Lane &LN, hipStream_t st, const MicroPlan &mb, float *out) {
    const AnceEncoderDesc &D = e->d;
    const AnceEncoder::Lane::Fp32 &V = LN.f32;
    const int I = D.intermediate, T = mb.T, Tpad = mb.Tpad;
    float *const no_stats = nullptr;
    {
        ProfScope pe(PC_EMBED, st);
        hipLaunchKernelGGL(embed32_kernel<H>, dim3(Tpad / 4), dim3(256), 0, st, LN.tok_id, LN.tok_pos, Tpad, e->word, e->pos,
                           e->type0, D.vocab_size, D.max_position, V.xb.x);
        hipLaunchKernelGGL(ln32_kernel<H>, dim3(Tpad / 4), dim3(256), 0, st, V.xb.x, Tpad, e->eln_w, e->eln_b, D.ln_eps, V.h, no_stats);
    }
    for (int li = 0; li < D.n_layers; ++li) {
        const LayerW &W = e->layers[li];
        const bool last = li == D.n_layers - 1;
        if (ProfScope ps(PC_GEMM_QK, st, 2.0 * T * (3.0 * H) * H);
            int rc = launch_gemm32(P_EPI_BIAS, V.h, H, W.wqkv32, H, W.bqkv32, nullptr, 0, V.qkv, 3 * H, Tpad, 3 * H, H, st))
            return rc;
        if (ProfScope ps(PC_ATTN, st); int rc = launch_attention32(V.qkv, V.ctx, LN.seq_off, mb.S, D.n_heads, st)) return rc;
        if (ProfScope ps(PC_GEMM_OUT, st, 2.0 * T * (double)H * H);
            int rc = launch_gemm32(P_EPI_RES, V.ctx, H, W.wo32, H, W.bo, V.h, H, V.xa.x, H, Tpad, H, H, st))
            return rc;
        {
            ProfScope ps(PC_LN, st);
            hipLaunchKernelGGL(ln32_kernel<H>, dim3(Tpad / 4), dim3(256), 0, st, V.xa.x, Tpad, W.ln1w, W.ln1b, D.ln_eps, V.ha, no_stats);
        }
        if (ProfScope ps(PC_GEMM_FFN1, st, 2.0 * T * (double)I * H);
            int rc = launch_gemm32(P_EPI_GELU, V.ha, H, W.w132, H, W.b1, nullptr, 0, V.ffn, I, Tpad, I, H, st))
            return rc;
        if (ProfScope ps(PC_GEMM_FFN2, st, 2.0 * T * (double)I * H);
            int rc = launch_gemm32(P_EPI_RES, V.ffn, I, W.w232, I, W.b2, V.ha, H, V.xb.x, H, Tpad, H, I, st))
            return rc;
        {
            ProfScope ps(PC_LN, st);
            hipLaunchKernelGGL(ln32_kernel<H>, dim3(Tpad / 4), dim3(256), 0, st, V.xb.x, Tpad, W.ln2w, W.ln2b, D.ln_eps, V.h,
                               last ? V.xb.stats : no_stats);
        }
    }
    encoder_output<H>(e, LN, st, mb, out, V.xb, 0);
    return ANCE_OK;
}


template <int H, int FORM>
GemmArgs folded_args(const Rows<FORM> &x, int M, float eps, const _Float16 *B, int N, const float *bias, const float *csum,
                     const float *wscale_inv = nullptr, unsigned *faults = nullptr) {
    constexpr int ld = FORM == FORM_PAIR ? 2 * H : H;
    GemmArgs G = {};
    if constexpr (FORM == FORM_PAIR) G.A = x.xp;
    else { G.A = x.hi; G.tok_lo = x.lo; }
    G.lda = ld; G.B = B; G.ldb = ld; G.M = M; G.N = N; G.K = H;
    G.bias = bias; G.csum = csum; G.part_in = x.part; G.ln_eps = eps; G.wscale_inv = wscale_inv; G.range_faults = faults;
    return G;
}

template <int H>
GemmArgs qk_args(const Rows<FORM_PLANES> &x, int M, float eps, const LayerW &W, int c0, int n, _Float16 *qk) {
    GemmArgs G = folded_args<H>(x, M, eps, W.wqk + (size_t)c0 * H, n, W.bqk + c0, W.cqk + c0);
    G.out16 = qk + c0; G.ldc = 2 * H;
    G.scale = 0.125f * 1.44269504088896340736f; G.scale_cols = c0 == 0 ? H : 0;
    return G;
}
template <int H>
GemmArgs qkv_args(const Rows<FORM_PAIR> &x, int M, float eps, const LayerW &W, int c0, int n, float *qkv, unsigned *faults) {
    GemmArgs G = folded_args<H>(x, M, eps, W.wqkv_s + (size_t)c0 * 2 * H, n, W.bqkv_s + c0, W.cqkv_s + c0, W.sc_s + 4, faults);
    G.out32 = qkv + c0; G.ldc = 3 * H;
    return G;
}

template <int H>
GemmArgs vt_args(const Rows<FORM_PLANES> &x, int Tpad, int T, float eps, const LayerW &W, _Float16 *vt, int ldvt, const int *col_map) {
    GemmArgs G = {};
    G.A = W.wv; G.lda = H; G.B = x.hi; G.tok_lo = x.lo; G.ldb = H; G.M = H; G.N = Tpad; G.K = H;
    G.bias = W.bv; G.csum = W.cv; G.part_in = x.part; G.ln_eps = eps;
    G.out16 = vt; G.ldc = ldvt; G.col_map = col_map; G.n_valid = T;
    return G;
}

template <int H, int FORM>
GemmArgs ffn1_args(const Rows<FORM> &xa, int M, float eps, const LayerW &W, int I, _Float16 *ffn, int n_split, unsigned *faults) {
    constexpr bool P = FORM == FORM_PAIR;
    GemmArgs G = folded_args<H>(xa, M, eps, P ? W.w1_s : W.w1, I, P ? W.b1_s : W.b1, P ? W.c1_s : W.c1, P ? W.sc_s + 6 : nullptr, faults);
    G.out16 = ffn; G.ldc = P ? 2 * I : I; G.n_split = n_split;
    return G;
}

template <int H, int FORM>
GemmArgs resln_args(const _Float16 *A, const _Float16 *B, int K, const float *bias, int M, const Rows<FORM> &res, const float *gamma,
                    const float *beta, float eps, const Rows<FORM> &out, const float *wscale_inv, unsigned *faults) {
    constexpr int w = FORM == FORM_PAIR ? 2 : 1;
    GemmArgs G = {};
    G.A = A; G.lda = w * K; G.B = B; G.ldb = w * K; G.M = M; G.N = H; G.K = K; G.bias = bias; G.ldc = w * H;
    G.res_gamma = gamma; G.res_beta = beta; G.part_in = res.part; G.ln_eps = eps; G.part_out = out.part;
    G.wscale_inv = wscale_inv; G.range_faults = faults;
    if constexpr (FORM == FORM_PAIR) { G.res_hi = res.xp; G.ldr = 2 * H; G.out16 = out.xp; }
    else { G.res_hi = res.hi; G.res_lo = res.lo; G.out16 = out.hi; G.out_lo = out.lo; }
    return G;
}

template <int H>
int forward_split(AnceEncoder *e, const AnceEncoder::Lane &LN, hipStream_t st, const MicroPlan &mb, float *out) {
    constexpr int HP = 2 * H;
    const AnceEncoderDesc &D = e->d;
    const AnceEncoder::Lane::Split &V = LN.sp;
    const int I = D.intermediate, S = mb.S, T = mb.T, Tpad = mb.Tpad;
    {
        ProfScope pe(PC_EMBED, st);
        hipLaunchKernelGGL((embed_kernel<H, FORM_PAIR>), dim3(Tpad / 4), dim3(256), 0, st, LN.tok_id, LN.tok_pos, Tpad, e->word,
                           e->pos, e->type0, D.vocab_size, D.max_position, V.xb, e->faults);
    }
    const bool cls_tail = e->cls_tail;
    const int S_pad = (int)align_up((size_t)S, 256);
    const Rows<FORM_PAIR> cls = V.cls(S_pad, H);
    const int n_split = (I / 256) % 2 == 0 ? 2 : 0;
    for (int li = 0; li < D.n_layers; ++li) {
        const LayerW &W = e->layers[li];
        const bool tail = cls_tail && li == D.n_layers - 1;
        const int Mrows = tail ? S_pad : Tpad;
        const double Mwork = tail ? (double)S : (double)T;
        const float eps_b = li == 0 ? D.ln_eps * (EMB_SCALE * EMB_SCALE) : D.ln_eps;
        const float *const gamma_b = li == 0 ? e->eln_w : e->layers[li - 1].ln2w, *const beta_b = li == 0 ? e->eln_b : e->layers[li - 1].ln2b;
        if (tail) {
            ProfScope ps(PC_LN, st);
            hipLaunchKernelGGL((gather_cls_kernel<H, FORM_PAIR>), dim3(S_pad / 4), dim3(256), 0, st, V.xb, LN.seq_off, S, S_pad, cls);
        }
        {
            ProfScope ps(PC_GEMM_QK, st, tail ? 2.0 * T * (2.0 * H) * H + 2.0 * S * (double)H * H : 2.0 * T * (3.0 * H) * H);
            const int c0 = tail ? H : 0;
            int rc = launch_gemm_f16(EPI_S_QKV, qkv_args<H>(V.xb, Tpad, eps_b, W, c0, 3 * H - c0, V.qkv, e->faults), st, H);
            if (tail && !rc) rc = launch_gemm_f16(EPI_S_QKV, qkv_args<H>(cls, S_pad, eps_b, W, 0, H, V.qkv, e->faults), st, H);
            if (rc) return rc;
        }
        {
            ProfScope ps(PC_ATTN, st);
            if (tail && S_pad > S)
                (void)hipMemsetAsync(V.ctx + (size_t)S * HP, 0, (size_t)(S_pad - S) * HP * sizeof(_Float16), st);
            if (int rc = launch_attention_split(V.qkv, V.ctx, LN.desc, S, D.n_heads, mb.maxlen, tail ? 1 : 0, st)) return rc;
        }
        if (ProfScope ps(PC_GEMM_OUT, st, 2.0 * Mwork * (double)H * H);
            int rc = launch_gemm_f16(EPI_S_RESLN, resln_args<H>(V.ctx, W.wo_s, H, W.bo, Mrows, tail ? cls : V.xb, gamma_b, beta_b, eps_b,
                                                                V.xa, W.sc_s + 5, e->faults), st, H))
            return rc;
        if (ProfScope ps(PC_GEMM_FFN1, st, 2.0 * Mwork * (double)I * H);
            int rc = launch_gemm_f16(EPI_S_GELU, ffn1_args<H>(V.xa, Mrows, D.ln_eps, W, I, V.ffn, n_split, e->faults), st, H))
            return rc;
        if (ProfScope ps(PC_GEMM_FFN2, st, 2.0 * Mwork * (double)I * H);
            int rc = launch_gemm_f16(EPI_S_RESLN, resln_args<H>(V.ffn, W.w2_s, I, W.b2, Mrows, V.xa, W.ln1w, W.ln1b, D.ln_eps, V.xb,
                                                                W.sc_s + 7, e->faults), st, H))
            return rc;
    }
    encoder_output<H>(e, LN, st, mb, out, V.xb, cls_tail ? 1 : 0);
    return ANCE_OK;
}

template <int H>
int forward_fp16(AnceEncoder *e, const AnceEncoder::Lane &LN, hipStream_t st, const MicroPlan &mb, float *out) {
    const AnceEncoderDesc &D = e->d;
    const AnceEncoder::Lane::Fp16 &V = LN.f16;
    const int I = D.intermediate, S = mb.S, T = mb.T, Tpad = mb.Tpad;
    {
        ProfScope pe(PC_EMBED, st);
        hipLaunchKernelGGL((embed_kernel<H, FORM_PLANES>), dim3(Tpad / 4), dim3(256), 0, st, LN.tok_id, LN.tok_pos, Tpad, e->word,
                           e->pos, e->type0, D.vocab_size, D.max_position, V.xb, (unsigned *)nullptr);
    }
    const bool cls_tail = e->cls_tail;
    const int S_pad = (int)align_up((size_t)S, 256);
    const Rows<FORM_PLANES> cls = V.cls(S_pad, H);
    const int n_split = (I / 256) % 2 == 0 ? 2 : 0;
    for (int li = 0; li < D.n_layers; ++li) {
        const LayerW &W = e->layers[li];
        const bool tail = cls_tail && li == D.n_layers - 1;
        const int Mrows = tail ? S_pad : Tpad;
        const double Mwork = tail ? (double)S : (double)T;
        const float *const gamma_b = li == 0 ? e->eln_w : e->layers[li - 1].ln2w, *const beta_b = li == 0 ? e->eln_b : e->layers[li - 1].ln2b;
        if (tail) {
            ProfScope ps(PC_LN, st);
            hipLaunchKernelGGL((gather_cls_kernel<H, FORM_PLANES>), dim3(S_pad / 4), dim3(256), 0, st, V.xb, LN.seq_off, S, S_pad, cls);
        }
        {
            ProfScope ps(PC_GEMM_QK, st, tail ? 2.0 * T * (double)H * H + 2.0 * S * (double)H * H : 2.0 * T * (2.0 * H) * H);
            const int c0 = tail ? H : 0;
            int rc = launch_gemm_f16(EPI_QK_F, qk_args<H>(V.xb, Tpad, D.ln_eps, W, c0, 2 * H - c0, V.qk), st, H);
            if (tail && !rc) rc = launch_gemm_f16(EPI_QK_F, qk_args<H>(cls, S_pad, D.ln_eps, W, 0, H, V.qk), st, H);
            if (rc) return rc;
        }
        if (ProfScope ps(PC_GEMM_VT, st, 2.0 * T * (double)H * H);
            int rc = launch_gemm_f16(EPI_VT_F, vt_args<H>(V.xb, Tpad, T, D.ln_eps, W, V.vt, mb.ldvt, LN.tok_vtcol), st, H))
            return rc;
        AttnArgs A;
        A.qk = V.qk; A.vt = V.vt; A.ctx = V.ctx; A.desc = LN.desc;
        A.ld_qk = 2 * H; A.ld_vt = mb.ldvt; A.ld_ctx = H; A.n_heads = D.n_heads; A.cls_only = tail ? 1 : 0; A.q_compact = tail ? 1 : 0;
        if (ProfScope ps(PC_ATTN, st, 0.0); int rc = launch_attention(A, S, mb.maxlen, st)) return rc;
        if (ProfScope ps(PC_GEMM_OUT, st, 2.0 * Mwork * (double)H * H);
            int rc = launch_gemm_f16(EPI_RESLN, resln_args<H>(V.ctx, W.wo, H, W.bo, Mrows, tail ? cls : V.xb, gamma_b, beta_b, D.ln_eps,
                                                              V.xa, nullptr, nullptr), st, H))
            return rc;
        if (ProfScope ps(PC_GEMM_FFN1, st, 2.0 * Mwork * (double)I * H);
            int rc = launch_gemm_f16(EPI_GELU_F, ffn1_args<H>(V.xa, Mrows, D.ln_eps, W, I, V.ffn, n_split, nullptr), st, H))
            return rc;
        if (ProfScope ps(PC_GEMM_FFN2, st, 2.0 * Mwork * (double)I * H);
            int rc = launch_gemm_f16(EPI_RESLN, resln_args<H>(V.ffn, W.w2, I, W.b2, Mrows, V.xa, W.ln1w, W.ln1b, D.ln_eps, V.xb,
                                                              nullptr, nullptr), st, H))
            return rc;
    }
    encoder_output<H>(e, LN, st, mb, out, V.xb, cls_tail ? 1 : 0);
    return ANCE_OK;
}

struct LaneFork {
    AnceEncoder *e;
    hipStream_t caller_st;
    bool forked = false;
    void fork() {
        (void)hipEventRecord(e->ev_fork, caller_st);
        for (int ln = 0; ln < e->n_lanes; ++ln) (void)hipStreamWaitEvent(e->side[ln], e->ev_fork, 0);
        forked = true;
    }
    void join_lanes() {
        for (int ln = 0; forked && ln < e->n_lanes; ++ln) {
            (void)hipEventRecord(e->ev_join[ln], e->side[ln]);
            (void)hipStreamWaitEvent(caller_st, e->ev_join[ln], 0);
        }
        forked = false;
    }
    ~LaneFork() { join_lanes(); }
};

int encode_impl(AnceEncoder *e, const int32_t *base, int64_t ld, const int32_t *d_lens, const int32_t *h_lens, int hdr,
                int64_t n, int L, int n_chunks, float *d_out, hipStream_t caller_st) {
    if (!e || !base || !d_out || n < 0 || L < 1 || n_chunks < 1 || L % n_chunks) {
        set_last_error("ance_encode: invalid argument");
        return ANCE_E_INVALID;
    }
    const int Lc = L / n_chunks;
    if (Lc > e->d.max_seq_len) {
        set_last_error("ance_encode: chunk length exceeds desc.max_seq_len");
        return ANCE_E_INVALID;
    }
    const AnceEncoderDesc &D = e->d;
    const bool seed = D.arch == ANCE_ARCH_SEED;
    if (seed && n_chunks != 1) {
        set_last_error("ance_encode: ANCE_ARCH_SEED encodes whole records (n_chunks must be 1)");
        return ANCE_E_INVALID;
    }
    int mb_index = 0;
    LaneFork lanes{e, caller_st};

    for (int64_t r0 = 0; r0 < n; r0 += FETCH_CHUNK) {
        const int nr = (int)((n - r0) < FETCH_CHUNK ? (n - r0) : FETCH_CHUNK);
        const int32_t *hl;
        if (h_lens) {
            hl = h_lens + r0;
        } else {
            e->host_lens.resize(nr);
            hipLaunchKernelGGL(fetch_lens_kernel, dim3((nr + 255) / 256), dim3(256), 0, caller_st, base, ld, d_lens, r0, nr, L,
                               e->lens_fetch);
            if (hipMemcpyAsync(e->host_lens.data(), e->lens_fetch, (size_t)nr * 4, hipMemcpyDeviceToHost, caller_st) != hipSuccess ||
                hipStreamSynchronize(caller_st) != hipSuccess)
                return check_launch("ance_encode: length read-back");
            hl = e->host_lens.data();
        }
        if (seed)
            for (int i = 0; i < nr; ++i)
                if (hl[i] <= 0) {
                    set_last_error("ance_encode: empty record under ANCE_ARCH_SEED (the reference defines no output for it)");
                    return ANCE_E_INVALID;
                }
        if (e->n_lanes > 1 && !lanes.forked) lanes.fork();
        const int64_t gs_end = (int64_t)nr * n_chunks;
        int64_t gs = 0;
        while (gs < gs_end) {
            const AnceEncoder::Lane &LN = e->lane[mb_index % e->n_lanes];
            hipStream_t st = e->n_lanes > 1 ? e->side[mb_index % e->n_lanes] : caller_st;
            ++mb_index;
            const MicroPlan mb = plan_micro_batch(hl, gs, gs_end, n_chunks, L, Lc, e->scap, e->tcap, e->vcap, seed);
            if (mb.S == 0) {
                set_last_error("ance_encode: max_tokens too small for one sequence");
                return ANCE_E_INVALID;
            }
            PlanArgs P;
            P.base = base; P.ld = ld; P.lens = d_lens; P.hdr = hdr;
            P.g0 = r0 * n_chunks + gs; P.S = mb.S; P.L = L; P.n_chunks = n_chunks; P.Lc = Lc;
            P.pad_id = D.pad_token_id; P.arch = D.arch; P.T = mb.T; P.Tpad = mb.Tpad; P.vt_spare = mb.V;
            P.seq_off = LN.seq_off; P.seq_vtcol = LN.seq_vtcol; P.seq_len = LN.seq_len;
            P.tok_id = LN.tok_id; P.tok_pos = LN.tok_pos; P.tok_vtcol = LN.tok_vtcol;
            P.desc = LN.desc; P.faults = e->faults;
            {
                ProfScope ps(PC_PLAN, st);
                if (seed) hipLaunchKernelGGL(seed_count_kernel, dim3((mb.S + 3) / 4), dim3(256), 0, st, P);
                hipLaunchKernelGGL(plan_kernel, dim3(1), dim3(1024), 0, st, P);
                const int nb_seq = (mb.S + 3) / 4, nb_pad = ((seed ? mb.Tpad : mb.Tpad - mb.T) + 255) / 256;
                hipLaunchKernelGGL(pack_kernel, dim3(nb_seq > nb_pad ? nb_seq : nb_pad), dim3(256), 0, st, P);
            }
            float *const out = d_out + (size_t)(r0 * n_chunks + gs) * HEAD_OUT;
            const int rc = with_hidden(D.hidden, [&](auto h) {
                constexpr int H = decltype(h)::value;
                return e->mode == ANCE_PRECISION_FP32    ? forward_fp32<H>(e, LN, st, mb, out)
                       : e->mode == ANCE_PRECISION_SPLIT ? forward_split<H>(e, LN, st, mb, out)
                                                         : forward_fp16<H>(e, LN, st, mb, out);
            });
            if (rc) return rc;
            gs = mb.next;
        }
        if (r0 + FETCH_CHUNK < n && !h_lens) lanes.join_lanes();
    }
    lanes.join_lanes();
    return check_launch("ance_encode");
}

}

extern "C" size_t ance_encoder_weight_bytes(const AnceEncoderDesc *desc) {
    if (!desc_ok(desc)) return 0;
    Arena a;
    layout_weights(desc, a, nullptr);
    return a.off + 256;
}

extern "C" size_t ance_encoder_workspace_bytes(const AnceEncoderDesc *desc) {
    if (!desc_ok(desc)) return 0;
    Arena a;
    layout_workspace(desc, a, nullptr);
    return a.off + 256;
}

extern "C" int ance_encoder_create(const AnceEncoderDesc *desc, const void *const *w, int n_weights, void *d_weight_arena,
                                   size_t weight_bytes, void *d_workspace, size_t workspace_bytes, void *stream,
                                   AnceEncoder **out) {
    if (!desc_ok(desc) || !w || !out || !d_weight_arena || !d_workspace ||
        n_weights != ANCE_ENCODER_N_WEIGHTS(desc->n_layers, desc->has_head)) {
        set_last_error("ance_encoder_create: invalid descriptor or weight list");
        return ANCE_E_INVALID;
    }
    for (int i = 0; i < n_weights; ++i)
        if (!w[i]) {
            set_last_error("ance_encoder_create: null weight pointer");
            return ANCE_E_INVALID;
        }
    if (weight_bytes < ance_encoder_weight_bytes(desc) || workspace_bytes < ance_encoder_workspace_bytes(desc)) {
        set_last_error("ance_encoder_create: arena or workspace too small");
        return ANCE_E_WORKSPACE;
    }
    AnceEncoder *e = new (std::nothrow) AnceEncoder();
    if (!e) return ANCE_E_NOMEM;
    e->d = *desc;
    {
        const char *ct = getenv("ANCE_CLS_TAIL");
        e->cls_tail = !(ct && ct[0] == '0');
        e->mode = resolve_precision(desc);
        const char *ns = getenv("ANCE_ENCODER_STREAMS");
        e->n_lanes = (ns && ns[0] >= '1' && ns[0] <= '0' + MAX_LANES) ? ns[0] - '0' : 2;
    }
    for (int ln = 0; ln < MAX_LANES; ++ln) {
        e->side[ln] = nullptr;
        e->ev_join[ln] = nullptr;
    }
    e->ev_fork = nullptr;
    if (e->n_lanes > 1) {
        bool ok = hipEventCreateWithFlags(&e->ev_fork, hipEventDisableTiming) == hipSuccess;
        for (int ln = 0; ln < e->n_lanes && ok; ++ln)
            ok = hipStreamCreateWithFlags(&e->side[ln], hipStreamNonBlocking) == hipSuccess &&
                 hipEventCreateWithFlags(&e->ev_join[ln], hipEventDisableTiming) == hipSuccess;
        if (!ok) {
            delete e;
            return check_launch("ance_encoder_create: streams");
        }
    }
    const int H = desc->hidden, HP = 2 * H;
    const hipError_t head_attr = with_hidden(H, [&](auto h) {
        constexpr int HW = decltype(h)::value;
        const void *k = e->mode == ANCE_PRECISION_FP32    ? reinterpret_cast<const void *>(head_gemm_kernel<HW, FORM_F32>)
                        : e->mode == ANCE_PRECISION_SPLIT ? reinterpret_cast<const void *>(head_gemm_kernel<HW, FORM_PAIR>)
                                                          : reinterpret_cast<const void *>(head_gemm_kernel<HW, FORM_PLANES>);
        return hipFuncSetAttribute(k, hipFuncAttributeMaxDynamicSharedMemorySize, (int)HEAD_LDS_BYTES<HW>);
    });
    if (head_attr != hipSuccess) {
        delete e;
        return check_launch("ance_encoder_create: head attr");
    }
    Arena wa, xa;
    wa.base = reinterpret_cast<char *>(align_up((uintptr_t)d_weight_arena, 256));
    xa.base = reinterpret_cast<char *>(align_up((uintptr_t)d_workspace, 256));
    layout_weights(desc, wa, e);
    layout_workspace(desc, xa, e);
    hipStream_t st = (hipStream_t)stream;
    (void)hipMemsetAsync(xa.base, 0, xa.off, st);

    const size_t I = desc->intermediate;
    cpy32(w[0], e->word, (size_t)desc->vocab_size * H, st);
    cpy32(w[1], e->pos, (size_t)desc->max_position * H, st);
    cpy32(w[2], e->type0, H, st);
    cpy32(w[3], e->eln_w, H, st);
    cpy32(w[4], e->eln_b, H, st);
    for (int i = 0; i < desc->n_layers; ++i) {
        const void *const *p = w + 5 + 16 * i;
        LayerW &L = e->layers[i];
        const float *gin = (const float *)(i == 0 ? w[3] : w[5 + 16 * (i - 1) + 14]);
        const float *bin = (const float *)(i == 0 ? w[4] : w[5 + 16 * (i - 1) + 15]);
        cpy32(p[7], L.bo, H, st);
        cpy32(p[8], L.ln1w, H, st);
        cpy32(p[9], L.ln1b, H, st);
        cpy32(p[13], L.b2, H, st);
        cpy32(p[14], L.ln2w, H, st);
        cpy32(p[15], L.ln2b, H, st);
        if (e->mode == ANCE_PRECISION_FP16) {
            auto foldw = [&](const void *W, const void *b, const float *g, const float *be, int N, _Float16 *W16, float *cs,
                             float *bo) {
                with_hidden(H, [&](auto h) {
                    hipLaunchKernelGGL(fold_weight_kernel<decltype(h)::value>, dim3((N + 3) / 4), dim3(256), 0, st, (const float *)W,
                                       (const float *)b, g, be, N, W16, cs, bo);
                });
            };
            foldw(p[0], p[1], gin, bin, H, L.wqk, L.cqk, L.bqk);
            foldw(p[2], p[3], gin, bin, H, L.wqk + (size_t)H * H, L.cqk + H, L.bqk + H);
            foldw(p[4], p[5], gin, bin, H, L.wv, L.cv, L.bv);
            foldw(p[10], p[11], (const float *)p[8], (const float *)p[9], (int)I, L.w1, L.c1, L.b1);
            cvt16(p[6], L.wo, (size_t)H * H, st);
            cvt16(p[12], L.w2, (size_t)H * I, st);
        } else if (e->mode == ANCE_PRECISION_SPLIT) {
            unsigned *slots = reinterpret_cast<unsigned *>(L.sc_s);
            (void)hipMemsetAsync(L.sc_s, 0, 4 * sizeof(float), st);
            auto mx = [&](const void *W, const float *g, int N, int K, int slot) {
                hipLaunchKernelGGL(wabsmax_kernel, dim3(256), dim3(256), 0, st, (const float *)W, g, N, K, slots + slot);
            };
            auto sw = [&](const void *W, const void *b, const float *g, const float *be, int N, int K, int slot, _Float16 *Wp, float *cs,
                          float *bo) {
                hipLaunchKernelGGL(split_weight_kernel, dim3((N + 3) / 4), dim3(256), 0, st, (const float *)W, (const float *)b, g, be,
                                   N, K, (const unsigned *)(slots + slot), Wp, cs, bo, L.sc_s + 4 + slot);
            };
            mx(p[0], gin, H, H, 0);
            mx(p[2], gin, H, H, 0);
            mx(p[4], gin, H, H, 0);
            mx(p[6], nullptr, H, H, 1);
            mx(p[10], (const float *)p[8], (int)I, H, 2);
            mx(p[12], nullptr, H, (int)I, 3);
            sw(p[0], p[1], gin, bin, H, H, 0, L.wqkv_s, L.cqkv_s, L.bqkv_s);
            sw(p[2], p[3], gin, bin, H, H, 0, L.wqkv_s + (size_t)H * HP, L.cqkv_s + H, L.bqkv_s + H);
            sw(p[4], p[5], gin, bin, H, H, 0, L.wqkv_s + (size_t)2 * H * HP, L.cqkv_s + 2 * H, L.bqkv_s + 2 * H);
            sw(p[6], nullptr, nullptr, nullptr, H, H, 1, L.wo_s, nullptr, nullptr);
            sw(p[10], p[11], (const float *)p[8], (const float *)p[9], (int)I, H, 2, L.w1_s, L.c1_s, L.b1_s);
            sw(p[12], nullptr, nullptr, nullptr, H, (int)I, 3, L.w2_s, nullptr, nullptr);
        } else {
            cpy32(p[0], L.wqkv32, (size_t)H * H, st);
            cpy32(p[2], L.wqkv32 + (size_t)H * H, (size_t)H * H, st);
            cpy32(p[4], L.wqkv32 + (size_t)2 * H * H, (size_t)H * H, st);
            cpy32(p[1], L.bqkv32, H, st);
            cpy32(p[3], L.bqkv32 + H, H, st);
            cpy32(p[5], L.bqkv32 + 2 * H, H, st);
            cpy32(p[6], L.wo32, (size_t)H * H, st);
            cpy32(p[10], L.w132, I * H, st);
            cpy32(p[11], L.b1, I, st);
            cpy32(p[12], L.w232, (size_t)H * I, st);
        }
    }
    if (desc->has_head) {
        const void *const *p = w + 5 + 16 * desc->n_layers;
        cpy32(p[0], e->head_w, (size_t)HEAD_OUT * H, st);
        cpy32(p[1], e->head_b, HEAD_OUT, st);
        cpy32(p[2], e->norm_w, HEAD_OUT, st);
        cpy32(p[3], e->norm_b, HEAD_OUT, st);
    }
    int rc = check_launch("ance_encoder_create");
    if (rc) {
        delete e;
        return rc;
    }
    *out = e;
    return ANCE_OK;
}

extern "C" void ance_encoder_destroy(AnceEncoder *enc) {
    if (!enc) return;
    for (int ln = 0; ln < MAX_LANES; ++ln) {
        if (enc->side[ln]) {
            (void)hipStreamSynchronize(enc->side[ln]);
            (void)hipStreamDestroy(enc->side[ln]);
        }
        if (enc->ev_join[ln]) (void)hipEventDestroy(enc->ev_join[ln]);
    }
    if (enc->ev_fork) (void)hipEventDestroy(enc->ev_fork);
    delete enc;
}

extern "C" int ance_encoder_precision(const AnceEncoder *enc) {
    if (!enc) return ANCE_E_INVALID;
    return enc->mode;
}

extern "C" int ance_encoder_range_faults(AnceEncoder *enc, uint32_t *h_out, int reset, void *stream) {
    if (!enc || !h_out) {
        set_last_error("ance_encoder_range_faults: invalid argument");
        return ANCE_E_INVALID;
    }
    hipStream_t st = (hipStream_t)stream;
    if (hipMemcpyAsync(h_out, enc->faults, 2 * sizeof(uint32_t), hipMemcpyDeviceToHost, st) != hipSuccess)
        return check_launch("ance_encoder_range_faults");
    if (reset) (void)hipMemsetAsync(enc->faults, 0, 2 * sizeof(uint32_t), st);
    return check_launch("ance_encoder_range_faults");
}

extern "C" int ance_encode_records(AnceEncoder *enc, const void *d_records, const int32_t *h_lens, int64_t n, int L,
                                   int n_chunks, float *d_out, void *stream) {
    return encode_impl(enc, (const int32_t *)d_records, (int64_t)L + 1, nullptr, h_lens, 1, n, L, n_chunks, d_out,
                       (hipStream_t)stream);
}

extern "C" int ance_encode_ids(AnceEncoder *enc, const int32_t *d_ids, int64_t ld_ids, const int32_t *d_lens,
                               const int32_t *h_lens, int64_t n, int L, int n_chunks, float *d_out, void *stream) {
    if (!d_lens) {
        set_last_error("ance_encode_ids: d_lens is required");
        return ANCE_E_INVALID;
    }
    return encode_impl(enc, d_ids, ld_ids, d_lens, h_lens, 0, n, L, n_chunks, d_out, (hipStream_t)stream);
}

extern "C" double ance_encoder_flops_per_sequence(int T) {
    const double t = T;
    return 169869312.0 * t + 36864.0 * t * t + 1179648.0;
}
```

ance_amd/csrc/gemm256_epilogue_split.h:

```cpp
#pragma once
#include "gemm256_epilogue.h"

namespace ance {

__device__ __forceinline__ f16x8 cat_f16x4(const f16x4 a, const f16x4 b) { return f16x8{a[0], a[1], a[2], a[3], b[0], b[1], b[2], b[3]}; }
__device__ __forceinline__ void epi_pair_store8_nt(const f32x4 va, const f32x4 vb, _Float16 *row, int W, int n) {
    f16x4 ha, ra, hb, rb;
    pair_split4(va, &ha, &ra);
    pair_split4(vb, &hb, &rb);
    __builtin_nontemporal_store(cat_f16x4(ha, hb), reinterpret_cast<f16x8 *>(row + pair_hi_col(n, W)));
    __builtin_nontemporal_store(cat_f16x4(ra, rb), reinterpret_cast<f16x8 *>(row + pair_lo_col(n, W)));
}

__device__ __forceinline__ float quad_sum(float x) {
    x += __builtin_amdgcn_update_dpp(0.f, x, 0xB1, 0xF, 0xF, true);
    x += __builtin_amdgcn_update_dpp(0.f, x, 0x4E, 0xF, 0xF, true);
    return x;
}
__device__ __forceinline__ float half_mirror(float x) { return __builtin_amdgcn_update_dpp(0.f, x, 0x141, 0xF, 0xF, true); }
__device__ __forceinline__ float sum8(const f32x4 a, const f32x4 b) { return ((a[0] + a[1]) + (a[2] + a[3])) + ((b[0] + b[1]) + (b[2] + b[3])); }
__device__ __forceinline__ float sumsq8(const f32x4 a, const f32x4 b, float m) {
    const float a0 = a[0] - m, a1 = a[1] - m, a2 = a[2] - m, a3 = a[3] - m, b0 = b[0] - m, b1 = b[1] - m, b2 = b[2] - m, b3 = b[3] - m;
    return ((a0 * a0 + a1 * a1) + (a2 * a2 + a3 * a3)) + ((b0 * b0 + b1 * b1) + (b2 * b2 + b3 * b3));
}

template <int EPI, int PASS_COLS>
struct SplitLanes {
    static constexpr int CPL = EPI == EPI_S_QKV ? 4 : 8, NV = CPL / 4;
    static constexpr int LPR = PASS_COLS / CPL, RPI = 64 / LPR, ITS = 32 / RPI;
};

template <int EPI>
__device__ __forceinline__ void split_piece_store(const GemmArgs &G, const float *sp, f32x4 (&a)[SplitLanes<EPI, 64>::NV],
                                                  const f32x4 (&b)[SplitLanes<EPI, 64>::NV], const f32x4 (&c)[SplitLanes<EPI, 64>::NV],
                                                  float mean, float rstd, float winv, size_t row, int n, float *vmax) {
#pragma clang fp contract(off)
    constexpr int NV = SplitLanes<EPI, 64>::NV;
    if constexpr (EPI != EPI_S_RESLN) {
#pragma unroll
        for (int h = 0; h < NV; ++h) a[h] = *reinterpret_cast<const f32x4 *>(sp + 4 * h);
    }
    const float mr = mean * rstd, rw = rstd * winv;
#pragma unroll
    for (int h = 0; h < NV; ++h) {
        if constexpr (EPI != EPI_S_RESLN) {
#pragma unroll
            for (int e = 0; e < 4; ++e) a[h][e] = __builtin_fmaf(a[h][e], rw, __builtin_fmaf(-mr, c[h][e], b[h][e]));
            if constexpr (EPI == EPI_S_GELU) a[h] = gelu_exact4(a[h]);
        }
        range_track4(a[h], vmax);
    }
    if constexpr (EPI == EPI_S_QKV) __builtin_nontemporal_store(a[0], reinterpret_cast<f32x4 *>(G.out32 + row * G.ldc + n));
    else epi_pair_store8_nt(a[0], a[NV - 1], G.out16 + row * G.ldc, G.N, n);
}

template <int EPI, int HW = 768>
__device__ __forceinline__ void gemm256_epilogue_split(const GemmArgs &G, f32x4 (&acc)[4][8], float *smem_f, int m0, int n0,
                                                       int w, int l, float winv) {
#pragma clang fp contract(off)
    const int i = l & 15, c4 = 4 * (l >> 4);
    const int wm = w >> 2, wn = w & 3;
    const int mw0 = m0 + wm * 128, nw0 = n0 + wn * 64;
    float *slab = smem_f + w * 4096;
    constexpr int LS = 68;
    typedef SplitLanes<EPI, 64> LN;
    constexpr int CPL = LN::CPL, NV = LN::NV, LPR = LN::LPR, RPI = LN::RPI, ITS = LN::ITS;
    const int cl = l % LPR, rl_ = l / LPR;
    const int nc = nw0 + cl * CPL;
    const float *pb = smem_f + EPB_OFF;
    const float *vp = pb + EPB_VEC + wn * 64 + cl * CPL;
    f32x4 v0[NV], v1[NV], v2[NV];
#pragma unroll
    for (int h = 0; h < NV; ++h) {
        v0[h] = *reinterpret_cast<const f32x4 *>(vp + 4 * h);
        v1[h] = *reinterpret_cast<const f32x4 *>(vp + 256 + 4 * h);
        v2[h] = f32x4{0.f, 0.f, 0.f, 0.f};
        if constexpr (EPI == EPI_S_RESLN) v2[h] = *reinterpret_cast<const f32x4 *>(vp + 512 + 4 * h);
    }
    const int n_parts = G.N >> 6, slice = nw0 >> 6;
    float vmax = 0.f;
#pragma unroll
    for (int y = 0; y < 4; ++y) {
        f16x8 rh[ITS], rl[ITS];
        float mean[ITS], rstd[ITS];
#pragma unroll
        for (int it = 0; it < ITS; ++it) {
            const int rr = it * RPI + rl_;
            if constexpr (EPI == EPI_S_RESLN) {
                const _Float16 *rp = G.res_hi + (size_t)(mw0 + y * 32 + rr) * G.ldr;
                rh[it] = *reinterpret_cast<const f16x8 *>(rp + pair_hi_col(nc, G.N));
                rl[it] = *reinterpret_cast<const f16x8 *>(rp + pair_lo_col(nc, G.N));
            }
            mean[it] = pb[EPB_STATS + 2 * (wm * 128 + y * 32 + rr)];
            rstd[it] = pb[EPB_STATS + 2 * (wm * 128 + y * 32 + rr) + 1];
        }
        epi_sync();
#pragma unroll
        for (int yb = 0; yb < 2; ++yb)
#pragma unroll
            for (int x = 0; x < 4; ++x) *reinterpret_cast<f32x4 *>(slab + (yb * 16 + i) * LS + x * 16 + c4) = acc[x][2 * y + yb];
        epi_sync();
        f32x4 vv[ITS][NV];
#pragma unroll
        for (int it = 0; it < ITS; ++it) {
            const int rr = it * RPI + rl_;
            const size_t row = (size_t)(mw0 + y * 32 + rr);
            const float *sp = slab + rr * LS + cl * CPL;
            if constexpr (EPI == EPI_S_RESLN) {
#pragma unroll
                for (int h = 0; h < NV; ++h) {
                    f32x4 a = *reinterpret_cast<const f32x4 *>(sp + 4 * h);
#pragma unroll
                    for (int e = 0; e < 4; ++e) {
                        const float ga = rstd[it] * v1[h][e];
                        const float ra = (float)rh[it][4 * h + e] + (float)rl[it][4 * h + e] * PAIR_LO_INV;
                        a[e] = __builtin_fmaf(a[e], winv, __builtin_fmaf(ra - mean[it], ga, v0[h][e] + v2[h][e]));
                    }
                    vv[it][h] = a;
                }
            }
            split_piece_store<EPI>(G, sp, vv[it], v0, v1, mean[it], rstd[it], winv, row, nc, &vmax);
        }
        if constexpr (EPI == EPI_S_RESLN) {
            float s4[ITS], q4[ITS];
#pragma unroll
            for (int it = 0; it < ITS; ++it) {
                const float s = quad_sum(sum8(vv[it][0], vv[it][NV - 1]));
                s4[it] = (s + half_mirror(s)) * (1.0f / 64.0f);
            }
#pragma unroll
            for (int it = 0; it < ITS; ++it) {
                const float q = quad_sum(sumsq8(vv[it][0], vv[it][NV - 1], s4[it]));
                q4[it] = q + half_mirror(q);
            }
            static_assert(ITS == 4 && LPR >= 4, "one lane per row group");
            const float ss = cl == 0 ? s4[0] : cl == 1 ? s4[1] : cl == 2 ? s4[2] : s4[3];
            const float qq = cl == 0 ? q4[0] : cl == 1 ? q4[1] : cl == 2 ? q4[2] : q4[3];
            if constexpr (HW == 1024) {
                if (cl < ITS) epb_park_part(smem_f, wm * 128 + y * 32 + cl * RPI + rl_, wn, ss, qq);
            } else if (cl < ITS) {
                *reinterpret_cast<float2 *>(G.part_out + ((size_t)(mw0 + y * 32 + cl * RPI + rl_) * n_parts + slice) * 2) = make_float2(ss, qq);
            }
        }
    }
    if constexpr (EPI == EPI_S_RESLN && HW == 1024) epb_merge_parts(G, smem_f, m0, n0, w * 64 + l);
    range_report(vmax, G.range_faults);
}

template <int EPI>
__device__ __forceinline__ void gemm256_epilogue_split32(const GemmArgs &G, f32x4 (&acc)[4][8], float *slab, const float *stats,
                                                         const float *vec, int m0, int n0, int w, int l, float winv) {
    static_assert(EPI == EPI_S_QKV || EPI == EPI_S_GELU, "the RESLN GEMMs run the launch-per-tile kernel (DESIGN_REJECTED.md round 6)");
    const int i = l & 15, c4 = 4 * (l >> 4);
    const int wm = w >> 2, wn = w & 3;
    const int mw0 = m0 + wm * 128, nw0 = n0 + wn * 64;
    constexpr int LS = EPS_LS;
    typedef SplitLanes<EPI, 32> LN;
    constexpr int CPL = LN::CPL, NV = LN::NV, LPR = LN::LPR, RPI = LN::RPI, ITS = LN::ITS;
    const int cl = l % LPR, rl_ = l / LPR;
    float vmax = 0.f;
#pragma unroll
    for (int p = 0; p < 8; ++p) {
        const int y = p >> 1, x = p & 1;
        const float *vp = vec + wn * 64 + x * 32 + cl * CPL;
        f32x4 v0[NV], v1[NV];
#pragma unroll
        for (int h = 0; h < NV; ++h) {
            v0[h] = *reinterpret_cast<const f32x4 *>(vp + 4 * h);
            v1[h] = *reinterpret_cast<const f32x4 *>(vp + 256 + 4 * h);
        }
        epi_sync();
#pragma unroll
        for (int yb = 0; yb < 2; ++yb)
#pragma unroll
            for (int xb = 0; xb < 2; ++xb) *reinterpret_cast<f32x4 *>(slab + (yb * 16 + i) * LS + xb * 16 + c4) = acc[2 * x + xb][2 * y + yb];
        epi_sync();
#pragma unroll
        for (int it = 0; it < ITS; ++it) {
            const int rr = it * RPI + rl_;
            const float mean = stats[2 * (wm * 128 + y * 32 + rr)], rstd = stats[2 * (wm * 128 + y * 32 + rr) + 1];
            f32x4 vv[NV];
            split_piece_store<EPI>(G, slab + rr * LS + cl * CPL, vv, v0, v1, mean, rstd, winv, (size_t)(mw0 + y * 32 + rr), nw0 + x * 32 + cl * CPL, &vmax);
        }
    }
    range_report(vmax, G.range_faults);
}

}
```

ance_amd/csrc/gemm256_f16.hip:

```cpp
#include "common.h"
#include "gemm_f16.h"
#include "gemm256_epilogue.h"
#include "gemm256_epilogue_split.h"
#include "gemm256_tile.h"
#include "pipe256.h"
#include <stdlib.h>

namespace ance {
namespace {

#ifdef ANCE_MEASURE
__device__ unsigned long long *g_gemm_stamps = nullptr;
#define GSTAMP(slot) do { if (stamps_ && tid == 0) stamps_[(size_t)blockIdx.x * 8 + (slot)] = __builtin_amdgcn_s_memrealtime(); } while (0)
#else
#define GSTAMP(slot) do { } while (0)
#endif

template <int EPI, int HW = 768>
__global__ void __launch_bounds__(G256_THREADS, 2) gemm256_f16_desc_kernel(const GemmArgs G) {
    extern __shared__ __attribute__((aligned(16))) float smem_f[];
    _Float16 *smem = reinterpret_cast<_Float16 *>(smem_f);
    int mt, nt;
    if (!tile_of_block(G, blockIdx.x, &mt, &nt)) return;
    const int m0 = mt * TM, n0 = nt * TN;
    const int tid = threadIdx.x;
    const int w = __builtin_amdgcn_readfirstlane(tid >> 6);
    const int l = tid & 63;
    f32x16 acc[2][4];
#pragma unroll
    for (int x = 0; x < 2; ++x)
#pragma unroll
        for (int y = 0; y < 4; ++y) acc[x][y] = f32x16{0};
    Pipe256T<PipeSrcDesc> P;
    P.init(smem, w, l);
    P.S.ra = pipe_rows_rsrc(G.A, m0, G.lda);
    P.S.rb = pipe_rows_rsrc(G.B, n0, G.ldb);
    pipe_fill_voff(P.S.voff, w, l, G.lda, G.ldb);
    constexpr bool EPB = EPI >= EPI_RESLN;
#ifdef ANCE_MEASURE
    unsigned long long *stamps_ = (EPI == EPI_RESLN && G.stamp) ? g_gemm_stamps : nullptr;
#endif
    GSTAMP(0);
    if constexpr (EPB) epb_issue<EPI>(G, smem_f, m0, n0, w, l);
    constexpr bool FOLDK = EPI == EPI_QK_F || EPI == EPI_GELU_F || EPI == EPI_VT_F;
    if constexpr (FOLDK) {
        P.run(G.K / TK, acc);
        GSTAMP(1);
        const bool wide = epb_stats<HW>(G, smem_f, tid);
        if (wide && G.tok_lo) {
            Pipe256T<PipeSrcDesc, false, true> P2;
            P2.init(smem, w, l);
            P2.S = P.S;
            const float *st = smem_f + EPB_OFF + EPB_STATS;
            const int i = l & 31;
            auto tok_wide = [&](int t) { return __builtin_fabsf(st[2 * t]) * st[2 * t + 1] > FOLD_WIDE_MEAN; };
            if constexpr (EPI == EPI_VT_F) {
                P2.S.rb = pipe_rows_rsrc(G.tok_lo, n0, G.ldb);
                P2.keep_b = (tok_wide((w & 3) * 64 + i) ? 1u : 0u) | (tok_wide((w & 3) * 64 + 32 + i) ? 2u : 0u);
            } else {
                P2.S.ra = pipe_rows_rsrc(G.tok_lo, m0, G.lda);
                unsigned k = 0;
#pragma unroll
                for (int y = 0; y < 4; ++y) k |= tok_wide((w >> 2) * 128 + y * 32 + i) ? (1u << y) : 0u;
                P2.keep_a = k;
            }
            P2.run(G.K / TK, acc);
        }
    } else {
        P.run(G.K / TK, acc);
        GSTAMP(1);
        if constexpr (EPB) (void)epb_stats<HW>(G, smem_f, tid);
    }
    GSTAMP(2);
#ifdef ANCE_MEASURE
    gemm256_epilogue<EPI, HW>(G, acc, smem_f, m0, n0, w, l, stamps_ ? stamps_ + (size_t)blockIdx.x * 8 + 4 : nullptr);
    asm volatile("s_waitcnt vmcnt(0)" ::: "memory");
#else
    gemm256_epilogue<EPI, HW>(G, acc, smem_f, m0, n0, w, l);
#endif
    GSTAMP(3);
}

template <int EPI, int HW = 768>
__global__ void __launch_bounds__(G256_THREADS, 2) gemm256_split_kernel(const GemmArgs G) {
    extern __shared__ __attribute__((aligned(16))) float smem_f[];
    _Float16 *smem = reinterpret_cast<_Float16 *>(smem_f);
    int mt, nt;
    if (!tile_of_block(G, blockIdx.x, &mt, &nt)) return;
    const int m0 = mt * TM, n0 = nt * TN;
    const int tid = threadIdx.x;
    const int w = __builtin_amdgcn_readfirstlane(tid >> 6);
    const int l = tid & 63;
    f32x4 acc[4][8];
#pragma unroll
    for (int x = 0; x < 4; ++x)
#pragma unroll
        for (int y = 0; y < 8; ++y) acc[x][y] = f32x4{0.f, 0.f, 0.f, 0.f};
    Pipe256T<PipeSrcDesc, true> P;
    P.init(smem, w, l);
    P.S.ra = pipe_rows_rsrc(G.A, m0, G.lda);
    P.S.rb = pipe_rows_rsrc(G.B, n0, G.ldb);
    pipe_fill_voff(P.S.voff, w, l, G.lda, G.ldb);
    const float winv = G.wscale_inv ? *G.wscale_inv : 1.0f;
#ifdef ANCE_MEASURE
    unsigned long long *stamps_ = G.stamp ? g_gemm_stamps : nullptr;
#endif
    GSTAMP(0);
    epb_issue<EPI>(G, smem_f, m0, n0, w, l);
    P.run(G.K / 32, acc);
    GSTAMP(1);
    (void)epb_stats<HW>(G, smem_f, tid);
    GSTAMP(2);
    gemm256_epilogue_split<EPI, HW>(G, acc, smem_f, m0, n0, w, l, winv);
#ifdef ANCE_MEASURE
    if (stamps_) asm volatile("s_waitcnt vmcnt(0)" ::: "memory");
#endif
    GSTAMP(3);
}

template <int EPI, int HW = 768>
__global__ void __launch_bounds__(G256_THREADS, 2) gemm256_split_stream_kernel(const GemmArgs G) {
    extern __shared__ __attribute__((aligned(16))) float smem_f[];
    _Float16 *smem = reinterpret_cast<_Float16 *>(smem_f);
    const int tid = threadIdx.x;
    const int w = __builtin_amdgcn_readfirstlane(tid >> 6);
    const int l = tid & 63;
    const int xcd = blockIdx.x & 7, slot = blockIdx.x >> 3, nslots = gridDim.x >> 3;
    const int n_blocks = gemm256_virtual_blocks(G);
    int round = 0;
    auto next_tile = [&](int *mt, int *nt) -> bool {
        for (;;) {
            const int b = ((round * nslots + slot) << 3) | xcd;
            if (b >= n_blocks) return false;
            ++round;
            if (tile_of_block(G, b, mt, nt)) return true;
        }
    };
    int mt, nt;
    if (!next_tile(&mt, &nt)) return;
    Pipe256T<PipeSrcStream, true> P;
    P.init(smem, w, l);
    P.S.ra = pipe_rows_rsrc(G.A, 0, G.lda, (uint32_t)G.M);
    P.S.rb = pipe_rows_rsrc(G.B, 0, G.ldb, (uint32_t)G.N);
    pipe_fill_voff(P.S.voff, w, l, G.lda, G.ldb);
    const int NK = G.K / 32;
    P.S.NK = NK;
    P.S.a_cur = P.S.a_nxt = (uint32_t)mt * 256u * (uint32_t)G.lda * 2u;
    P.S.b_cur = P.S.b_nxt = (uint32_t)nt * 256u * (uint32_t)G.ldb * 2u;
    const float winv = G.wscale_inv ? *G.wscale_inv : 1.0f;
    pb_issue<EPI>(G, smem_f + EPS_R, smem_f + EPS_VEC, mt * TM, nt * TN, w, l);
    if constexpr (ANCE_STREAM_LOOSE_FIRST) P.prologue_landed(); else P.prologue();
    P.enter();
    for (;;) {
        int mtn = 0, ntn = 0;
        const bool have_n = next_tile(&mtn, &ntn);
        f32x4 acc[4][8];
#pragma unroll
        for (int x = 0; x < 4; ++x)
#pragma unroll
            for (int y = 0; y < 8; ++y) acc[x][y] = f32x4{0.f, 0.f, 0.f, 0.f};
        if (have_n) {
            P.S.a_nxt = (uint32_t)mtn * 256u * (uint32_t)G.lda * 2u;
            P.S.b_nxt = (uint32_t)ntn * 256u * (uint32_t)G.ldb * 2u;
        }
        constexpr int F = ANCE_STREAM_LOOSE_FIRST ? EPS_FOREIGN_OPS : 0;
        constexpr int VM0F = 6 + F > 63 ? 63 : 6 + F, VM1F = 2 + F > 63 ? 63 : 2 + F;
        if (have_n) P.template tiles_streaming<VM0F, VM1F>(NK, acc); else P.template tiles_final<VM0F, VM1F>(NK, acc);
        P.leave();
        int lf = l;
        asm volatile("" : "+v"(lf));
        const int tf = (w << 6) | lf;
        const GemmArgs Ge = kernarg_reload(G);
        if (tf < 256) (void)pb_token_stats<HW>(smem_f + EPS_R, smem_f + EPS_STATS, tf, Ge.ln_eps);
        eps_barrier();
        gemm256_epilogue_split32<EPI>(Ge, acc, eps_slab(smem_f, w), smem_f + EPS_STATS, smem_f + EPS_VEC, mt * TM, nt * TN, w, lf, winv);
        if (!have_n) break;
        eps_barrier();
        mt = mtn;
        nt = ntn;
        P.S.a_cur = P.S.a_nxt;
        P.S.b_cur = P.S.b_nxt;
        pb_issue<EPI>(Ge, smem_f + EPS_R, smem_f + EPS_VEC, mt * TM, nt * TN, w, lf);
        P.enter();
    }
}

#ifdef ANCE_MEASURE
unsigned long long *g_gemm_stamps_host = nullptr;
int g_gemm_stamps_epi = EPI_RESLN;
#endif

int g_gemm_stream = -1;
int gemm_stream_mode() {
    if (g_gemm_stream < 0) {
        const char *e = getenv("ANCE_GEMM_STREAM");
        g_gemm_stream = (e && e[0] == '0') ? 0 : 1;
    }
    return g_gemm_stream;
}
int device_cu_count() {
    static int cus[64] = {0};
    int dev = 0;
    (void)hipGetDevice(&dev);
    if (dev < 0 || dev >= 64) dev = 0;
    if (cus[dev] == 0) {
        int n = 0;
        if (hipDeviceGetAttribute(&n, hipDeviceAttributeMultiprocessorCount, dev) != hipSuccess || n < 8) n = 256;
        cus[dev] = n;
    }
    return cus[dev];
}

typedef void (*gemm_kernel_t)(const GemmArgs);
template <int HW>
gemm_kernel_t gemm_kernel_of(int epi, bool stream) {
    if (stream) {
        switch (epi) {
            case EPI_S_QKV: return gemm256_split_stream_kernel<EPI_S_QKV, HW>;
            case EPI_S_GELU: return gemm256_split_stream_kernel<EPI_S_GELU, HW>;
            default: return nullptr;
        }
    }
    switch (epi) {
        case EPI_QK: return HW == 768 ? gemm256_f16_desc_kernel<EPI_QK> : nullptr;
        case EPI_GELU: return HW == 768 ? gemm256_f16_desc_kernel<EPI_GELU> : nullptr;
        case EPI_RES32: return HW == 768 ? gemm256_f16_desc_kernel<EPI_RES32> : nullptr;
        case EPI_RESLN: return gemm256_f16_desc_kernel<EPI_RESLN, HW>;
        case EPI_QK_F: return gemm256_f16_desc_kernel<EPI_QK_F, HW>;
        case EPI_GELU_F: return gemm256_f16_desc_kernel<EPI_GELU_F, HW>;
        case EPI_VT_F: return gemm256_f16_desc_kernel<EPI_VT_F, HW>;
        case EPI_S_QKV: return gemm256_split_kernel<EPI_S_QKV, HW>;
        case EPI_S_GELU: return gemm256_split_kernel<EPI_S_GELU, HW>;
        case EPI_S_RESLN: return gemm256_split_kernel<EPI_S_RESLN, HW>;
        default: return nullptr;
    }
}

bool dynamic_lds_ready(gemm_kernel_t k, unsigned long long *done, size_t bytes) {
    if (!attr_needed(done)) return true;
    if (hipFuncSetAttribute(reinterpret_cast<const void *>(k), hipFuncAttributeMaxDynamicSharedMemorySize, (int)bytes) != hipSuccess) return false;
    attr_mark(done);
    return true;
}

int launch256(int epi, const GemmArgs &G, hipStream_t st, int hw) {
    if (G.n_split != 0 && (G.n_split != 2 || ((G.N / TN) & 1) || epi < EPI_RESLN)) {
        set_last_error("gemm256: n_split needs an even number of N tiles and a descriptor-form kernel");
        return ANCE_E_INVALID;
    }
    const unsigned blocks = (unsigned)gemm256_virtual_blocks(G);
    const int wi = hw == 1024 ? 1 : 0;
    const bool known = epi >= 0 && epi < EPI_COUNT && (hw == 768 || hw == 1024);
    bool stream = (epi == EPI_S_QKV || epi == EPI_S_GELU) && gemm_stream_mode() == 1 && G.K >= 96 &&
                  (uint64_t)G.M * (uint64_t)G.lda * 2u < (1ull << 31) && (uint64_t)G.N * (uint64_t)G.ldb * 2u < (1ull << 31);
#ifdef ANCE_MEASURE
    const bool stamped = epi == g_gemm_stamps_epi && g_gemm_stamps_host;
    stream = stream && !stamped;
#endif
    const gemm_kernel_t k = !known ? nullptr : wi ? gemm_kernel_of<1024>(epi, stream) : gemm_kernel_of<768>(epi, stream);
    if (!k) {
        set_last_error("gemm256: bad epilogue or hidden width");
        return ANCE_E_INVALID;
    }
    const size_t lds = stream ? GS_LDS_BYTES : epi >= EPI_RESLN ? G256_EPB_LDS_BYTES : G256_LDS_BYTES;
    static unsigned long long attr_done[2][2][EPI_COUNT] = {{{0}}};
    if (!dynamic_lds_ready(k, &attr_done[stream][wi][epi], stream ? GS_LDS_BYTES : G256_EPB_LDS_BYTES)) return check_launch("gemm256 attr");
    if (stream) {
        const unsigned cus = (unsigned)device_cu_count() & ~7u;
        hipLaunchKernelGGL(k, dim3(blocks < cus ? blocks : cus), dim3(G256_THREADS), lds, st, G);
        return ANCE_OK;
    }
#ifdef ANCE_MEASURE
    if (stamped) {
        GemmArgs G2 = G;
        G2.stamp = 1;
        hipLaunchKernelGGL(k, dim3(blocks), dim3(G256_THREADS), lds, st, G2);
        return ANCE_OK;
    }
#endif
    hipLaunchKernelGGL(k, dim3(blocks), dim3(G256_THREADS), lds, st, G);
    return ANCE_OK;
}

}

void reload_gemm_knobs() { g_gemm_stream = -1; }

bool gemm256_applicable(const GemmArgs &G) {
    return G.M > 0 && G.N > 0 && G.K >= 2 * TK && G.M % TM == 0 && G.N % TN == 0 && G.K % TK == 0;
}

int launch_gemm_f16(int epi, const GemmArgs &G, hipStream_t st, int hw) {
    if (!gemm256_applicable(G)) {
        set_last_error("gemm_f16: M,N must be multiples of 256 and K a multiple of 64, >= 128");
        return ANCE_E_INVALID;
    }
    return launch256(epi, G, st, hw);
}

}

#ifdef ANCE_MEASURE
extern "C" void ance_debug_gemm_stamps(void *d_stamps) {
    ance::g_gemm_stamps_host = reinterpret_cast<unsigned long long *>(d_stamps);
    unsigned long long *p = ance::g_gemm_stamps_host;
    (void)hipMemcpyToSymbol(HIP_SYMBOL(ance::g_gemm_stamps), &p, sizeof(p));
}
extern "C" void ance_debug_gemm_stamps_epi(int epi) { ance::g_gemm_stamps_epi = epi; }
#endif
```

ance_amd/csrc/gemm256_hooks.hip:

```cpp
#include "common.h"
#include "gemm_f16.h"
#include <string.h>

extern "C" int ance_debug_gemm(int ablate, int epi, const void *d_a_f16, const void *d_b_f16, int M, int N, int K,
                               const float *d_bias, void *d_out, const float *d_res32, void *stream) {
    using namespace ance;
    if (ablate != 0 || !d_a_f16 || !d_b_f16 || !d_bias || !d_out || epi < 0 || epi > 2 || (epi == EPI_RES32 && !d_res32)) {
        set_last_error("ance_debug_gemm: invalid argument");
        return ANCE_E_INVALID;
    }
    GemmArgs G;
    memset(&G, 0, sizeof(G));
    G.A = (const _Float16 *)d_a_f16; G.lda = K; G.B = (const _Float16 *)d_b_f16; G.ldb = K;
    G.M = M; G.N = N; G.K = K; G.bias = d_bias; G.ldc = N; G.scale = 1.0f; G.scale_cols = 0;
    if (epi == EPI_RES32) { G.out32 = (float *)d_out; G.res32 = d_res32; }
    else G.out16 = (_Float16 *)d_out;
    ProfScope ps(PC_GEMM_FFN1, (hipStream_t)stream, 2.0 * M * (double)N * K);
    int rc = launch_gemm_f16(epi, G, (hipStream_t)stream);
    return rc ? rc : check_launch("ance_debug_gemm");
}

extern "C" int ance_debug_gemm_split(int epi, const void *d_a_pair, const void *d_b_pair, int M, int N, int K, const float *d_bias,
                                     const float *d_vec1, const float *d_vec2, const float *d_part, float ln_eps,
                                     const void *d_res_pair, void *d_out, float *d_part_out, const float *d_wscale_inv, void *stream) {
    using namespace ance;
    if (!d_a_pair || !d_b_pair || !d_bias || !d_vec1 || !d_part || !d_out || epi < EPI_S_QKV || epi > EPI_S_RESLN ||
        (epi == EPI_S_RESLN && (!d_vec2 || !d_res_pair || !d_part_out || (N != 768 && N != 1024))) || K % 64 != 0) {
        set_last_error("ance_debug_gemm_split: invalid argument");
        return ANCE_E_INVALID;
    }
    GemmArgs G;
    memset(&G, 0, sizeof(G));
    G.A = (const _Float16 *)d_a_pair; G.lda = 2 * K; G.B = (const _Float16 *)d_b_pair; G.ldb = 2 * K;
    G.M = M; G.N = N; G.K = K; G.bias = d_bias; G.part_in = d_part; G.ln_eps = ln_eps; G.wscale_inv = d_wscale_inv;
    if (epi == EPI_S_QKV) {
        G.csum = d_vec1; G.out32 = (float *)d_out; G.ldc = N;
    } else if (epi == EPI_S_GELU) {
        G.csum = d_vec1; G.out16 = (_Float16 *)d_out; G.ldc = 2 * N;
    } else {
        G.res_gamma = d_vec1; G.res_beta = d_vec2; G.res_hi = (const _Float16 *)d_res_pair; G.ldr = 2 * N;
        G.out16 = (_Float16 *)d_out; G.ldc = 2 * N; G.part_out = d_part_out;
    }
    int rc = launch_gemm_f16(epi, G, (hipStream_t)stream, epi == EPI_S_RESLN && N == 1024 ? 1024 : 768);
    return rc ? rc : check_launch("ance_debug_gemm_split");
}

extern "C" int ance_debug_gemm_hw(int epi, int hw, const AnceGemmDebugArgs *a, void *stream) {
    using namespace ance;
    const bool fold = epi == EPI_QK_F || epi == EPI_GELU_F || epi == EPI_VT_F;
    const bool bad = !a || (hw != 768 && hw != 1024) || epi < EPI_RESLN || epi > EPI_S_RESLN || (a->n_split != 0 && a->n_split != 2) ||
                     !a->a || !a->b || !a->bias || !a->part_in || !a->out ||
                     ((fold || epi == EPI_S_QKV || epi == EPI_S_GELU) && !a->csum) ||
                     (epi == EPI_QK_F && a->scale_cols % 64 != 0) ||
                     (epi == EPI_VT_F && !a->col_map) ||
                     (epi == EPI_RESLN && (!a->res_hi || !a->res_lo || !a->out_lo)) ||
                     ((epi == EPI_RESLN || epi == EPI_S_RESLN) && (!a->res_gamma || !a->res_beta || !a->part_out || a->N != hw)) ||
                     (epi == EPI_S_RESLN && !a->res_hi);
    if (bad) {
        set_last_error("ance_debug_gemm_hw: invalid argument");
        return ANCE_E_INVALID;
    }
    GemmArgs G;
    memset(&G, 0, sizeof(G));
    G.A = (const _Float16 *)a->a; G.B = (const _Float16 *)a->b; G.lda = a->lda; G.ldb = a->ldb;
    G.M = a->M; G.N = a->N; G.K = a->K;
    G.bias = a->bias; G.csum = a->csum; G.part_in = a->part_in; G.ln_eps = a->ln_eps; G.tok_lo = (const _Float16 *)a->tok_lo;
    G.scale = a->scale; G.scale_cols = a->scale_cols; G.col_map = a->col_map; G.n_valid = a->n_valid; G.ldc = a->ldc;
    if (epi == EPI_S_QKV) G.out32 = (float *)a->out;
    else G.out16 = (_Float16 *)a->out;
    G.res_hi = (const _Float16 *)a->res_hi; G.res_lo = (const _Float16 *)a->res_lo; G.res_gamma = a->res_gamma; G.res_beta = a->res_beta;
    G.out_lo = (_Float16 *)a->out_lo; G.part_out = a->part_out;
    G.ldr = a->ldr; G.wscale_inv = a->wscale_inv; G.n_split = a->n_split;
    int rc = launch_gemm_f16(epi, G, (hipStream_t)stream, hw);
    return rc ? rc : check_launch("ance_debug_gemm_hw");
}

extern "C" void ance_pair_layout(int n, int W, int *hi_col, int *lo_col, float *lo_scale) {
    if (hi_col) *hi_col = ance::pair_hi_col(n, W);
    if (lo_col) *lo_col = ance::pair_lo_col(n, W);
    if (lo_scale) *lo_scale = ance::PAIR_LO_SCALE;
}
```

ance_amd/csrc/gemm_f16.h:

```cpp
#pragma once
#include "common.h"

namespace ance {

enum { EPI_QK = 0, EPI_GELU = 1, EPI_RES32 = 2, EPI_VT = 3, EPI_RESLN = 4, EPI_QK_F = 5, EPI_GELU_F = 6, EPI_VT_F = 7,
       EPI_S_QKV = 8, EPI_S_GELU = 9, EPI_S_RESLN = 10, EPI_COUNT = 11 };

struct GemmArgs {
    const _Float16 *A;
    const _Float16 *B;
    int lda, ldb;
    int M, N, K;
    const float *bias;
    _Float16 *out16;
    float *out32;
    const float *res32;
    const float *res_gamma, *res_beta;
    int ldc;
    float scale;
    int scale_cols;
    const int *col_map;
    int n_valid;
    const float *part_in;
    float ln_eps;
    const float *csum;
    const _Float16 *res_hi, *res_lo;
    _Float16 *out_lo;
    float *part_out;
    const _Float16 *tok_lo;
    int ldr;
    const float *wscale_inv;
    unsigned *range_faults;
    int n_split;
#ifdef ANCE_MEASURE
    int stamp;
#endif
};

__device__ __forceinline__ f32x4 ln_apply4(f32x4 x, float mean, float rstd, f32x4 g, f32x4 b) {
    f32x4 y;
#pragma unroll
    for (int j = 0; j < 4; ++j) y[j] = (x[j] - mean) * rstd * g[j] + b[j];
    return y;
}

__device__ __forceinline__ float row16_sum(float x) {
    x += __builtin_amdgcn_update_dpp(0.f, x, 0xB1, 0xF, 0xF, true);
    x += __builtin_amdgcn_update_dpp(0.f, x, 0x4E, 0xF, 0xF, true);
    x += __builtin_amdgcn_update_dpp(0.f, x, 0x124, 0xF, 0xF, true);
    x += __builtin_amdgcn_update_dpp(0.f, x, 0x128, 0xF, 0xF, true);
    return x;
}
__device__ __forceinline__ void row16_sum8(float (&x)[8]) {
#pragma unroll
    for (int it = 0; it < 8; ++it) x[it] += __builtin_amdgcn_update_dpp(0.f, x[it], 0xB1, 0xF, 0xF, true);
#pragma unroll
    for (int it = 0; it < 8; ++it) x[it] += __builtin_amdgcn_update_dpp(0.f, x[it], 0x4E, 0xF, 0xF, true);
#pragma unroll
    for (int it = 0; it < 8; ++it) x[it] += __builtin_amdgcn_update_dpp(0.f, x[it], 0x124, 0xF, 0xF, true);
#pragma unroll
    for (int it = 0; it < 8; ++it) x[it] += __builtin_amdgcn_update_dpp(0.f, x[it], 0x128, 0xF, 0xF, true);
}

constexpr int PART_FLOATS = 24;
template <int HW>
struct PartFormat {
    static_assert(HW == 768 || HW == 1024, "hidden 768 or 1024");
    static constexpr int N = HW == 768 ? 12 : 8;
    static constexpr int COLS = HW == 768 ? 64 : 128;
    static_assert(2 * N <= PART_FLOATS && N * COLS == HW, "partial layout");
};

__device__ __forceinline__ void part_merge(float ma, float qa, float mb, float qb, float *m, float *q) {
#pragma clang fp contract(off)
    const float d = ma - mb;
    *m = (ma + mb) * 0.5f;
    *q = (qa + qb) + 32.0f * (d * d);
}

template <int HW = 768>
__device__ __forceinline__ void stats_from_parts(const float *pp, float eps, float *mean, float *rstd) {
    constexpr int NP = PartFormat<HW>::N;
    float m = 0.f, q = 0.f;
#pragma unroll
    for (int j = 0; j < NP; ++j) m += pp[2 * j];
    m *= 1.0f / (float)NP;
#pragma unroll
    for (int j = 0; j < NP; ++j) {
        const float d = pp[2 * j] - m;
        q += pp[2 * j + 1] + (float)PartFormat<HW>::COLS * d * d;
    }
    *mean = m;
    *rstd = rsqrtf(q * (1.0f / (float)HW) + eps);
}

int launch_gemm_f16(int epi, const GemmArgs &args, hipStream_t stream, int hw = 768);
bool gemm256_applicable(const GemmArgs &args);
void reload_gemm_knobs();

}
```

include/ance_amd.h:

```cpp
#ifndef ANCE_AMD_H
#define ANCE_AMD_H

#include <stddef.h>
#include <stdint.h>

#ifdef __cplusplus
extern "C" {
#endif

#define ANCE_OK 0
#define ANCE_E_INVALID (-1)
#define ANCE_E_WORKSPACE (-2)
#define ANCE_E_LAUNCH (-3)
#define ANCE_E_NOMEM (-4)

#define ANCE_ABI_VERSION 7
int ance_abi_version(void);
const char *ance_last_error(void);

#define ANCE_PROFILE_CATEGORIES 13
void ance_profile_enable(int on);
int ance_profile_read(double *ms, double *work, long long *count, int n);


#define ANCE_TOPK_MAX_K 1792

size_t ance_ip_topk_workspace_bytes(int64_t n, int64_t nq, int d, int k);

int ance_ip_topk(const float *d_x, int64_t n, int64_t row_base, const float *d_q, int64_t nq, int d, int k,
                 float *d_out_d, int64_t *d_out_i, void *d_workspace, size_t workspace_bytes, void *stream);

size_t ance_ip_topk_scan_workspace_bytes(int64_t n, int64_t nq, int d, int k);
int ance_ip_topk_scan(const float *d_x, int64_t n, int64_t row_base, const float *d_q, int64_t nq, int d, int k,
                      float *d_out_d, int64_t *d_out_i, void *d_workspace, size_t workspace_bytes, void *stream);

size_t ance_ip_index_bytes(int64_t n, int d);
int ance_ip_index_build(const float *d_x, int64_t n, int d, void *d_index, size_t index_bytes, void *stream);
size_t ance_ip_topk_indexed_workspace_bytes(int64_t n, int64_t nq, int d, int k);
int ance_ip_topk_indexed(const float *d_x, int64_t n, int64_t row_base, const void *d_index, const float *d_q,
                         int64_t nq, int d, int k, float *d_out_d, int64_t *d_out_i, void *d_workspace,
                         size_t workspace_bytes, void *stream);

size_t ance_topk_merge_workspace_bytes(int n_parts, int64_t nq, int k);

int ance_topk_merge(const float *d_parts_d, const int64_t *d_parts_i, int n_parts, int64_t nq, int k,
                    float *d_out_d, int64_t *d_out_i, void *d_workspace, size_t workspace_bytes, void *stream);

int ance_ip_score_rows(const float *d_x, int64_t n, const float *d_q, int64_t nq, int d, const int64_t *d_rows,
                       const int64_t *d_offsets, float *d_scores, void *stream);


#define ANCE_ARCH_ROBERTA 0
#define ANCE_ARCH_BERT 1
#define ANCE_ARCH_SEED 2

typedef struct AnceEncoderDesc {
    int32_t arch;
    int32_t n_layers;
    int32_t hidden;
    int32_t n_heads;
    int32_t intermediate;
    int32_t vocab_size;
    int32_t max_position;
    int32_t pad_token_id;
    float ln_eps;
    int32_t has_head;
    int32_t max_seq_len;
    int32_t max_tokens;
    int32_t precision;
} AnceEncoderDesc;

#define ANCE_PRECISION_DEFAULT 0
#define ANCE_PRECISION_SPLIT 1
#define ANCE_PRECISION_FP16 2
#define ANCE_PRECISION_FP32 3

typedef struct AnceEncoder AnceEncoder;

#define ANCE_ENCODER_N_WEIGHTS(n_layers, has_head) (5 + 16 * (n_layers) + ((has_head) ? 4 : 0))

size_t ance_encoder_weight_bytes(const AnceEncoderDesc *desc);
size_t ance_encoder_workspace_bytes(const AnceEncoderDesc *desc);

int ance_encoder_create(const AnceEncoderDesc *desc, const void *const *d_weights_fp32, int n_weights,
                        void *d_weight_arena, size_t weight_bytes, void *d_workspace, size_t workspace_bytes,
                        void *stream, AnceEncoder **out);
void ance_encoder_destroy(AnceEncoder *enc);
int ance_encoder_precision(const AnceEncoder *enc);

int ance_encoder_range_faults(AnceEncoder *enc, uint32_t *h_out, int reset, void *stream);

int ance_encode_records(AnceEncoder *enc, const void *d_records, const int32_t *h_lens, int64_t n, int L,
                        int n_chunks, float *d_out, void *stream);
int ance_encode_ids(AnceEncoder *enc, const int32_t *d_ids, int64_t ld_ids, const int32_t *d_lens,
                    const int32_t *h_lens, int64_t n, int L, int n_chunks, float *d_out, void *stream);

int ance_debug_gemm(int ablate, int epi, const void *d_a_f16, const void *d_b_f16, int M, int N, int K,
                    const float *d_bias, void *d_out, const float *d_res32, void *stream);

int ance_search_bad_image_calls(unsigned long long *out);

int ance_nll_forward(const float *d_q, const float *d_a, const float *d_b, const float *d_mask_a, const float *d_mask_b, int64_t n,
                     int d, int chunks, float *d_logits, float *d_loss_rows, float *d_loss_mean, void *stream);

int ance_nll_backward(const float *d_q, const float *d_a, const float *d_b, const float *d_mask_a, const float *d_mask_b, int64_t n,
                      int d, int chunks, const float *d_grad_output, float *d_gq, float *d_ga, float *d_gb, void *stream);

size_t ance_inbatch_nll_workspace_bytes(int64_t nq, int64_t nc, int d);
int ance_inbatch_nll_forward(const float *d_q, const float *d_ctx, const int64_t *d_positive_idx, int64_t nq, int64_t nc, int d,
                             float *d_loss_mean, int64_t *d_counts, void *d_workspace, size_t workspace_bytes, void *stream);
int ance_inbatch_nll_backward(const float *d_q, const float *d_ctx, const int64_t *d_positive_idx, int64_t nq, int64_t nc, int d,
                              const float *d_grad_output, float *d_gq, float *d_gctx, void *d_workspace, size_t workspace_bytes,
                              void *stream);

typedef struct AnceAttnTrainArgs {
    const float *q, *k, *v;
    float *ctx;
    int32_t ld_q, ld_k, ld_v, ld_ctx;
    const int32_t *d_seq_first, *d_seq_len;
    int32_t n_seq, max_seq_len, n_rows, n_heads;
    int32_t seq_rows;
    int32_t reserved;
    float dropout_p;
    int32_t training;
    uint64_t seed, offset;
    void *d_workspace;
    size_t workspace_bytes;
} AnceAttnTrainArgs;
typedef struct AnceAttnGradArgs {
    const float *dctx;
    float *dq, *dk, *dv;
    int32_t ld_dctx, ld_dq, ld_dk, ld_dv;
} AnceAttnGradArgs;
size_t ance_attention_workspace_bytes(int64_t n_rows, int n_heads);
int ance_attention_forward(const AnceAttnTrainArgs *args, void *stream);
int ance_attention_backward(const AnceAttnTrainArgs *args, const AnceAttnGradArgs *grads, void *stream);
int ance_attention_forward_dstream(const AnceAttnTrainArgs *args, const uint64_t *d_stream, void *stream);
int ance_attention_backward_dstream(const AnceAttnTrainArgs *args, const AnceAttnGradArgs *grads, const uint64_t *d_stream, void *stream);
int ance_dropout_stream_advance(uint64_t *d_stream, uint64_t n, void *stream);

#define ANCE_DTYPE_F16 1
#define ANCE_DTYPE_BF16 2
typedef struct AnceAttn16Args {
    const void *q, *k, *v;
    void *ctx;
    int32_t ld_q, ld_k, ld_v, ld_ctx;
    const int32_t *d_seq_first, *d_seq_len;
    int32_t n_seq, max_seq_len, n_rows, n_heads;
    int32_t seq_rows;
    int32_t dtype;
    float dropout_p;
    int32_t training;
    uint64_t seed, offset;
    void *d_workspace;
    size_t workspace_bytes;
} AnceAttn16Args;
typedef struct AnceAttn16GradArgs {
    const void *dctx;
    void *dq, *dk, *dv;
    int32_t ld_dctx, ld_dq, ld_dk, ld_dv;
} AnceAttn16GradArgs;
size_t ance_attention16_workspace_bytes(int64_t n_rows, int n_heads);
int ance_attention16_forward(const AnceAttn16Args *args, void *stream);
int ance_attention16_backward(const AnceAttn16Args *args, const AnceAttn16GradArgs *grads, void *stream);
int ance_attention16_forward_dstream(const AnceAttn16Args *args, const uint64_t *d_stream, void *stream);
int ance_attention16_backward_dstream(const AnceAttn16Args *args, const AnceAttn16GradArgs *grads, const uint64_t *d_stream, void *stream);

#define ANCE_DTYPE_F32 0
size_t ance_attention_row0_workspace_bytes(int64_t n_seq, int n_heads);
int ance_attention_row0_forward(const AnceAttn16Args *args, void *stream);
int ance_attention_row0_backward(const AnceAttn16Args *args, const AnceAttn16GradArgs *grads, void *stream);
int ance_attention_row0_forward_dstream(const AnceAttn16Args *args, const uint64_t *d_stream, void *stream);
int ance_attention_row0_backward_dstream(const AnceAttn16Args *args, const AnceAttn16GradArgs *grads, const uint64_t *d_stream, void *stream);

#define ANCE_LAYER_TAIL_ROWS_PER_WORKGROUP 16
typedef struct AnceLayerTailArgs {
    const float *x, *res;
    const float *bias;
    const float *gamma, *beta;
    float *y;
    int32_t ld_x, ld_res, ld_y;
    int32_t H, n_rows;
    float eps;
    float dropout_p;
    int32_t training;
    uint64_t seed, offset;
    void *d_workspace;
    size_t workspace_bytes;
} AnceLayerTailArgs;
typedef struct AnceLayerTailGradArgs {
    const float *dy;
    float *dx, *dres;
    float *dgamma, *dbeta, *dbias;
    int32_t ld_dy, ld_dx, ld_dres;
    int32_t reserved;
} AnceLayerTailGradArgs;
typedef struct AnceBiasGeluArgs {
    const float *x, *bias;
    float *y;
    int32_t ld_x, ld_y, N, n_rows;
    void *d_workspace;
    size_t workspace_bytes;
} AnceBiasGeluArgs;
typedef struct AnceBiasGeluGradArgs {
    const float *dy;
    float *dx, *dbias;
    int32_t ld_dy, ld_dx;
} AnceBiasGeluGradArgs;
int ance_layer_tail_rows_per_workgroup(void);
size_t ance_layer_tail_workspace_bytes(int64_t n_rows, int H);
size_t ance_bias_gelu_workspace_bytes(int64_t n_rows, int N);
int ance_layer_tail_forward(const AnceLayerTailArgs *args, void *stream);
int ance_layer_tail_backward(const AnceLayerTailArgs *args, const AnceLayerTailGradArgs *grads, void *stream);
int ance_layer_tail_forward_dstream(const AnceLayerTailArgs *args, const uint64_t *d_stream, void *stream);
int ance_layer_tail_backward_dstream(const AnceLayerTailArgs *args, const AnceLayerTailGradArgs *grads, const uint64_t *d_stream, void *stream);
int ance_bias_gelu_forward(const AnceBiasGeluArgs *args, void *stream);
int ance_bias_gelu_backward(const AnceBiasGeluArgs *args, const AnceBiasGeluGradArgs *grads, void *stream);

typedef struct AnceLayerTail16Args {
    const void *x;
    const float *res;
    const float *bias;
    const float *gamma, *beta;
    float *y;
    void *y16;
    int32_t ld_x, ld_res, ld_y, ld_y16;
    int32_t H, n_rows;
    int32_t dtype;
    float eps;
    float dropout_p;
    int32_t training;
    uint64_t seed, offset;
    void *d_workspace;
    size_t workspace_bytes;
} AnceLayerTail16Args;
typedef struct AnceLayerTail16GradArgs {
    const float *dy;
    const void *dy16;
    void *dx;
    float *dres;
    float *dgamma, *dbeta, *dbias;
    int32_t ld_dy, ld_dy16, ld_dx, ld_dres;
} AnceLayerTail16GradArgs;
typedef struct AnceBiasGelu16Args {
    const void *x;
    const float *bias;
    void *y;
    int32_t ld_x, ld_y, N, n_rows;
    int32_t dtype;
    int32_t reserved;
    void *d_workspace;
    size_t workspace_bytes;
} AnceBiasGelu16Args;
typedef struct AnceBiasGelu16GradArgs {
    const void *dy;
    void *dx;
    float *dbias;
    int32_t ld_dy, ld_dx;
} AnceBiasGelu16GradArgs;
size_t ance_layer_tail16_workspace_bytes(int64_t n_rows, int H);
size_t ance_bias_gelu16_workspace_bytes(int64_t n_rows, int N);
int ance_layer_tail16_forward(const AnceLayerTail16Args *args, void *stream);
int ance_layer_tail16_backward(const AnceLayerTail16Args *args, const AnceLayerTail16GradArgs *grads, void *stream);
int ance_layer_tail16_forward_dstream(const AnceLayerTail16Args *args, const uint64_t *d_stream, void *stream);
int ance_layer_tail16_backward_dstream(const AnceLayerTail16Args *args, const AnceLayerTail16GradArgs *grads, const uint64_t *d_stream, void *stream);
int ance_bias_gelu16_forward(const AnceBiasGelu16Args *args, void *stream);
int ance_bias_gelu16_backward(const AnceBiasGelu16Args *args, const AnceBiasGelu16GradArgs *grads, void *stream);

#define ANCE_EMBED_SEGMENT_CHUNK 64
#define ANCE_EMBED_POSITION_ABSOLUTE 0
#define ANCE_EMBED_POSITION_ROBERTA 1
typedef struct AnceEmbedArgs {
    const int32_t *ids;
    const int32_t *type_ids;
    const float *word, *pos, *type;
    const float *gamma, *beta;
    float *y;
    int32_t *positions;
    int32_t n_seq, L, H;
    int32_t vocab, max_pos, n_types;
    int32_t position_mode;
    int32_t padding_idx;
    float eps;
    float dropout_p;
    int32_t training;
    int32_t reserved;
    uint64_t seed, offset;
    void *d_workspace;
    size_t workspace_bytes;
} AnceEmbedArgs;
typedef struct AnceEmbedGradArgs {
    const float *dy;
    float *dword, *dpos, *dtype;
    float *dgamma, *dbeta;
    const int32_t *word_keys;
    const int64_t *word_perm;
    const int32_t *pos_keys;
    const int64_t *pos_perm;
    const int32_t *type_keys;
    const int64_t *type_perm;
} AnceEmbedGradArgs;
int ance_embed_segment_chunk(void);
size_t ance_embed_workspace_bytes(int64_t n_rows, int H);
int ance_embed_forward(const AnceEmbedArgs *args, void *stream);
int ance_embed_backward(const AnceEmbedArgs *args, const AnceEmbedGradArgs *grads, void *stream);
int ance_embed_forward_dstream(const AnceEmbedArgs *args, const uint64_t *d_stream, void *stream);
int ance_embed_backward_dstream(const AnceEmbedArgs *args, const AnceEmbedGradArgs *grads, const uint64_t *d_stream, void *stream);

typedef struct AncePackArgs {
    const int32_t *ids;
    const int32_t *type_ids;
    const int32_t *d_seq_len;
    int32_t *d_seq_off;
    int32_t *d_seq_kept;
    int64_t *d_dropped;
    int32_t *packed_ids;
    int32_t *packed_type_ids;
    int32_t *packed_positions;
    int32_t n_seq, L, rows;
    int32_t position_mode;
    int32_t padding_idx;
    int32_t vocab, max_pos;
    int32_t reserved;
} AncePackArgs;
typedef struct AnceFirstRowsArgs {
    void *rows_matrix;
    void *first;
    const int32_t *d_seq_off;
    const int32_t *d_seq_kept;
    int32_t ld_rows, ld_first;
    int32_t n_seq, rows, H;
    int32_t dtype;
} AnceFirstRowsArgs;
int ance_pack_tokens(const AncePackArgs *args, void *stream);
int ance_embed_rows_forward(const AnceEmbedArgs *args, void *stream);
int ance_embed_rows_backward(const AnceEmbedArgs *args, const AnceEmbedGradArgs *grads, void *stream);
int ance_embed_rows_forward_dstream(const AnceEmbedArgs *args, const uint64_t *d_stream, void *stream);
int ance_embed_rows_backward_dstream(const AnceEmbedArgs *args, const AnceEmbedGradArgs *grads, const uint64_t *d_stream, void *stream);
int ance_first_rows_gather(const AnceFirstRowsArgs *args, void *stream);
int ance_first_rows_scatter(const AnceFirstRowsArgs *args, void *stream);

int ance_debug_gemm_split(int epi, const void *d_a_pair, const void *d_b_pair, int M, int N, int K, const float *d_bias,
                          const float *d_vec1, const float *d_vec2, const float *d_part, float ln_eps, const void *d_res_pair,
                          void *d_out, float *d_part_out, const float *d_wscale_inv, void *stream);

typedef struct AnceGemmDebugArgs {
    const void *a, *b;
    int32_t lda, ldb, M, N, K;
    const float *bias, *csum, *part_in;
    float ln_eps;
    const void *tok_lo;
    float scale;
    int32_t scale_cols;
    const int32_t *col_map;
    int32_t n_valid, ldc;
    void *out;
    const void *res_hi, *res_lo;
    const float *res_gamma, *res_beta;
    void *out_lo;
    float *part_out;
    int32_t ldr;
    const float *wscale_inv;
    int32_t n_split;
} AnceGemmDebugArgs;
int ance_debug_gemm_hw(int epi, int hw, const AnceGemmDebugArgs *args, void *stream);

typedef struct AnceAttnDebugArgs {
    int32_t kind, n_heads, n_seq, max_seq_len, cls_only, q_compact;
    const int32_t *h_desc;
    void *d_desc;
    int64_t d_desc_bytes;
    const void *qk;
    int32_t ld_qk, qk_rows;
    const void *vt;
    int32_t ld_vt;
    void *ctx;
    int32_t ld_ctx, ctx_rows;
} AnceAttnDebugArgs;
int ance_debug_attention(const AnceAttnDebugArgs *args, void *stream);

void ance_pair_layout(int n, int W, int *hi_col, int *lo_col, float *lo_scale);

typedef struct AnceLambTensor {
    float *p;
    const float *g;
    float *m, *v;
    int64_t numel;
    int32_t group, reserved;
} AnceLambTensor;
typedef struct AnceLambGroup {
    double lr, beta1, beta2, eps, weight_decay;
} AnceLambGroup;
size_t ance_lamb_workspace_bytes(int n_tensors, int n_groups, int64_t total_numel);
int ance_lamb_step(const AnceLambTensor *h_tensors, int n_tensors, const AnceLambGroup *h_groups, int n_groups, int adam,
                   float *d_out, void *d_workspace, size_t workspace_bytes, void *stream);

size_t ance_lamb_clipped_workspace_bytes(int n_tensors, int n_groups, int64_t total_numel);
int ance_lamb_step_clipped(const AnceLambTensor *h_tensors, int n_tensors, const AnceLambGroup *h_groups, int n_groups, int adam,
                           double max_grad_norm, float *d_grad_norm, float *d_out, void *d_workspace, size_t workspace_bytes,
                           void *stream);

size_t ance_lamb_amp_workspace_bytes(int n_tensors, int n_groups, int64_t total_numel);
int ance_lamb_step_amp(const AnceLambTensor *h_tensors, int n_tensors, const AnceLambGroup *h_groups, int n_groups, int adam,
                       double max_grad_norm,
                       const float *d_grad_scale,
                       const float *d_found_inf,
                       const float *d_prev_out,
                       float *d_grad_norm,
                       int64_t *d_skipped,
                       float *d_out, void *d_workspace, size_t workspace_bytes, void *stream);

size_t ance_lamb_plan_table_bytes(int n_tensors, int n_groups, int64_t total_numel);
int ance_lamb_plan_build(const AnceLambTensor *h_tensors, int n_tensors, const AnceLambGroup *h_groups, const double *const *d_lrs,
                         int n_groups, void *h_tables, size_t h_tables_bytes, int64_t *n_chunks_out, size_t *table_bytes_out);
int ance_lamb_step_planned(int n_tensors, int n_groups, int64_t n_chunks, int adam, double max_grad_norm, const float *d_grad_scale,
                           const float *d_found_inf, const float *d_prev_out, float *d_grad_norm, int64_t *d_skipped, float *d_out,
                           void *d_workspace, size_t workspace_bytes, void *stream);

int ance_linear_warmup_step(int64_t *d_n, const double *d_base_lrs, double *d_lrs, int n_groups, int64_t num_warmup_steps,
                            int64_t num_training_steps, void *stream);

typedef struct AnceAdamwTensor {
    float *p;
    const float *g;
    float *m, *v;
    float *step;
    int64_t numel;
    int32_t group, reserved;
} AnceAdamwTensor;
size_t ance_adamw_workspace_bytes(int n_tensors, int n_groups, int64_t total_numel, int clip);
int ance_adamw_step(const AnceAdamwTensor *h_tensors, int n_tensors, const AnceLambGroup *h_groups, int n_groups, int correct_bias,
                    double max_grad_norm,
                    const float *d_grad_scale,
                    const float *d_found_inf,
                    float *d_grad_norm,
                    int64_t *d_skipped,
                    void *d_workspace, size_t workspace_bytes, void *stream);
long long ance_debug_staging_sends(void);
size_t ance_adamw_plan_table_bytes(int n_tensors, int n_groups, int64_t total_numel);
int ance_adamw_plan_build(const AnceAdamwTensor *h_tensors, int n_tensors, const AnceLambGroup *h_groups, const double *const *d_lrs,
                          int n_groups, void *h_tables, size_t h_tables_bytes, int64_t *n_chunks_out, size_t *table_bytes_out);
int ance_adamw_step_planned(int n_tensors, int n_groups, int64_t n_chunks, int correct_bias, double max_grad_norm,
                            const float *d_grad_scale, const float *d_found_inf, float *d_grad_norm, int64_t *d_skipped,
                            void *d_workspace, size_t workspace_bytes, void *stream);

#define ANCE_GATHER_MASK_LENGTH 0
#define ANCE_GATHER_MASK_NONZERO 1
#define ANCE_GATHER_TYPES_ZERO 0
#define ANCE_GATHER_TYPES_LENGTH 1
#define ANCE_GATHER_REFERENCE 0
#define ANCE_GATHER_WIDE 1
typedef struct AnceGatherSegment {
    const void *d_records;
    int64_t n_records;
    const int64_t *d_index;
    int64_t n_index;
    void *d_ids, *d_mask;
    void *d_types;
    int32_t L, mask_rule, type_rule, reserved;
} AnceGatherSegment;
int ance_gather_batch(const AnceGatherSegment *h_segs, int n_segs, int64_t first, int64_t B, int width, void *stream);

typedef struct AncePackedGatherSegment {
    const void *d_records;
    int64_t n_records;
    const int64_t *d_index;
    int64_t n_index;
    const int64_t *d_cum;
    int32_t *packed_ids;
    int32_t *packed_positions;
    int32_t *d_seq_off;
    int32_t *d_seq_kept;
    int64_t *d_dropped;
    int32_t L, chunk_len, rows;
    int32_t position_mode;
    int32_t padding_idx;
    int32_t vocab, max_pos;
    int32_t reserved;
} AncePackedGatherSegment;
int ance_record_lengths(const void *d_records, int64_t n_records, int L, int chunk_len, int rule, int32_t *d_out, void *stream);
int ance_gather_batch_packed(const AncePackedGatherSegment *h_segs, int n_segs, int64_t first, int64_t B, const int64_t *d_first,
                             void *stream);

void ance_reload_env(void);

void ance_debug_search_stamps(void *d_stamps);

double ance_encoder_flops_per_sequence(int T);


int ance_host_py_shuffle(uint32_t *mt_state, int64_t n, int64_t *out);

int ance_host_select_negatives(uint32_t *mt_state, const int64_t *I, int64_t nq, int k, const int64_t *p2id,
                               int64_t n_rows, const int64_t *pos_pid, const uint8_t *active, int negative_sample,
                               int select_topk, int n_threads, int64_t *out_neg, int32_t *out_cnt, double *out_mrr);

int ance_host_write_ann_training(const char *path, const int64_t *order, int64_t n_order, const int64_t *qid,
                                 const int64_t *pos_pid, const int64_t *src_row, const int64_t *neg, const int32_t *cnt,
                                 int negative_sample, int64_t *out_lines);

#ifdef __cplusplus
}
#endif
#endif
```

Before: 33430 passages/s.

## Emit QKV as f16 hi/lo pair image from GEMM epilogue, stage via global_load_lds

The QKV GEMM epilogue now applies the Q scale and writes an f16 hi/lo split image directly, replacing the fp32 QKV output. The attention kernel no longer loads fp32 and splits K/V/Q itself; it copies the precomputed pair image into LDS with global_load_lds DMA, using a zero buffer for padded keys. This removes repeated per-head conversion work and halves nothing in bytes (the hi+lo image is the same size as fp32) but moves the split out of the attention hot loop. The cost is extra epilogue ALU work in the GEMM, and the per-layer conversion becomes dependent on the new store layout.

```diff
diff --git a/ance_amd/_lib.py b/ance_amd/_lib.py
--- a/ance_amd/_lib.py
+++ b/ance_amd/_lib.py
@@ -269,6 +269,8 @@
                                              ctypes.c_void_p, ctypes.c_void_p, ctypes.c_void_p, ctypes.c_void_p, ctypes.c_void_p]),
     "ance_debug_gemm_hw": (ctypes.c_int, [ctypes.c_int, ctypes.c_int, ctypes.POINTER(AnceGemmDebugArgs), ctypes.c_void_p]),
     "ance_debug_attention": (ctypes.c_int, [ctypes.POINTER(AnceAttnDebugArgs), ctypes.c_void_p]),
+    "ance_debug_attention_pair": (ctypes.c_int, [ctypes.POINTER(AnceAttnDebugArgs), ctypes.c_void_p]),
+    "ance_debug_gemm_qkv_pair": (ctypes.c_int, [ctypes.c_int, ctypes.POINTER(AnceGemmDebugArgs), ctypes.c_void_p]),
     "ance_lamb_workspace_bytes": (ctypes.c_size_t, [ctypes.c_int, ctypes.c_int, ctypes.c_int64]),
     "ance_lamb_step": (ctypes.c_int, [ctypes.POINTER(AnceLambTensor), ctypes.c_int, ctypes.POINTER(AnceLambGroup), ctypes.c_int,
                                       ctypes.c_int, ctypes.c_void_p, ctypes.c_void_p, ctypes.c_size_t, ctypes.c_void_p]),
diff --git a/ance_amd/csrc/attention.h b/ance_amd/csrc/attention.h
--- a/ance_amd/csrc/attention.h
+++ b/ance_amd/csrc/attention.h
@@ -15,8 +15,9 @@
 };
 
 size_t attention_lds_bytes(int max_seq_len, int n_waves);
-int launch_attention_split(const float *qkv, _Float16 *ctx_pair, const int4 *desc, int n_seq, int n_heads, int max_seq_len,
+int launch_attention_split(const _Float16 *qkv_image, _Float16 *ctx_pair, const int4 *desc, int n_seq, int n_heads, int max_seq_len,
                            int cls_only, hipStream_t stream);
+void launch_qkv_image(const float *qkv, _Float16 *image, long long rows, int n_heads, hipStream_t stream);
 int launch_attention(const AttnArgs &args, int n_seq, int max_seq_len, hipStream_t stream);
 
 }
diff --git a/ance_amd/csrc/attention.hip b/ance_amd/csrc/attention.hip
--- a/ance_amd/csrc/attention.hip
+++ b/ance_amd/csrc/attention.hip
@@ -210,8 +210,12 @@
     asm volatile("s_nop 1\n\tv_permlane32_swap_b32 %0, %1\n\ts_nop 1" : "+v"(x), "+v"(y));
 }
 
+__device__ __attribute__((aligned(16))) unsigned g_zero16[4];
+typedef __attribute__((address_space(3))) void attn_lds_t;
+typedef const __attribute__((address_space(1))) void attn_glb_t;
+
 template <int NW>
-__global__ void __launch_bounds__(64 * NW, 2) attention_split_kernel(const float *qkv, _Float16 *ctx_pair, const int4 *desc, int n_heads,
+__global__ void __launch_bounds__(64 * NW, 2) attention_split_kernel(const _Float16 *img, _Float16 *ctx_pair, const int4 *desc, int n_heads,
                                                                      int cls_only, int kchunk) {
     extern __shared__ __attribute__((aligned(16))) float smem_f[];
     const int u = blockIdx.x / n_heads;
@@ -226,92 +230,52 @@
     _Float16 *Vl = Vh + (size_t)kc * VS;
     const int tid = threadIdx.x;
     const int w = tid >> 6, l = tid & 63, g = l >> 5, i = l & 31;
-    constexpr int NT = 64 * NW;
-    const int ld = 3 * n_heads * HD;
-    constexpr float SC = 2048.0f, SI = 1.0f / 2048.0f;
-    auto stage = [&](int k0, auto unr_tag) {
-        constexpr int UNR = decltype(unr_tag)::value;
-        for (int e0 = tid; e0 < kc * 8; e0 += UNR * NT) {
-            f32x4 kv[UNR][4];
-#pragma unroll
-            for (int it = 0; it < UNR; ++it) {
-                const int e = e0 + it * NT;
-                const int kl_ = e >> 3, ch = e & 7, key = k0 + kl_;
-#pragma unroll
-                for (int q = 0; q < 4; ++q) kv[it][q] = f32x4{0.f, 0.f, 0.f, 0.f};
-                if (e < kc * 8 && key < T) {
-                    const float *kp = qkv + (size_t)(tok0 + key) * ld + n_heads * HD + h * HD + ch * 8;
-                    kv[it][0] = *reinterpret_cast<const f32x4 *>(kp);
-                    kv[it][1] = *reinterpret_cast<const f32x4 *>(kp + 4);
-                    kv[it][2] = *reinterpret_cast<const f32x4 *>(kp + n_heads * HD);
-                    kv[it][3] = *reinterpret_cast<const f32x4 *>(kp + n_heads * HD + 4);
-                }
-            }
-#pragma unroll
-            for (int it = 0; it < UNR; ++it) {
-                const int e = e0 + it * NT;
-                if (e >= kc * 8) break;
-                const int kl_ = e >> 3, ch = e & 7;
-                const f32x4 k0v = kv[it][0], k1v = kv[it][1], v0 = kv[it][2], v1 = kv[it][3];
-                const f16x4 a0 = cvt_f16x4_pinned(k0v), a1 = cvt_f16x4_pinned(k1v), b0 = cvt_f16x4_pinned(v0), b1 = cvt_f16x4_pinned(v1);
-                f16x8 kh, kl;
-#pragma unroll
-                for (int j = 0; j < 4; ++j) {
-                    kh[j] = a0[j]; kh[4 + j] = a1[j];
-                    kl[j] = (_Float16)((k0v[j] - (float)a0[j]) * SC);
-                    kl[4 + j] = (_Float16)((k1v[j] - (float)a1[j]) * SC);
-                }
-                *reinterpret_cast<f16x8 *>(Kh + kl_ * HD + kswz(kl_, ch) * 8) = kh;
-                *reinterpret_cast<f16x8 *>(Kl + kl_ * HD + kswz(kl_, ch) * 8) = kl;
-                f16x8 vh, vl;
-#pragma unroll
-                for (int j = 0; j < 4; ++j) {
-                    vh[j] = b0[j]; vh[4 + j] = b1[j];
-                    vl[j] = (_Float16)((v0[j] - (float)b0[j]) * SC);
-                    vl[4 + j] = (_Float16)((v1[j] - (float)b1[j]) * SC);
-                }
-                *reinterpret_cast<f16x8 *>(Vh + kl_ * VS + vswz(kl_, ch * 8)) = vh;
-                *reinterpret_cast<f16x8 *>(Vl + kl_ * VS + vswz(kl_, ch * 8)) = vl;
-            }
-        }
+    const int H = n_heads * HD;
+    const int ld = 6 * H;
+    constexpr float SC = ATTN_LO_SCALE, SI = ATTN_LO_INV;
+    const int wu = __builtin_amdgcn_readfirstlane(w);
+    const int koff = pair_hi_col(H + h * HD, 0), voff = pair_hi_col(2 * H + h * HD, 0);
+    const _Float16 *zero16 = reinterpret_cast<const _Float16 *>(g_zero16);
+    asm volatile("" : "+s"(zero16));
+    auto stage = [&](int k0) {
+        const int ngroups = min(kc, Tk - k0) >> 3;
+        const int r8 = l >> 3, pc = l & 7;
+        for (int g8 = wu; g8 < ngroups; g8 += NW) {
+            const int kl_ = g8 * 8 + r8, key = k0 + kl_;
+            const int ck = kswz(kl_, pc), cv = vswz(kl_, pc * 8) >> 3;
+            const bool real = key < T;
+            const _Float16 *src = real ? img + (size_t)(tok0 + key) * ld : zero16;
+            const int ko = real ? koff + (ck >> 2) * 64 + (ck & 3) * 8 : 0, vo = real ? voff + (cv >> 2) * 64 + (cv & 3) * 8 : 0;
+            const int lo = real ? 32 : 0;
+            __builtin_amdgcn_global_load_lds((attn_glb_t *)(src + ko), (attn_lds_t *)(Kh + g8 * 8 * HD), 16, 0, 0);
+            __builtin_amdgcn_global_load_lds((attn_glb_t *)(src + ko + lo), (attn_lds_t *)(Kl + g8 * 8 * HD), 16, 0, 0);
+            __builtin_amdgcn_global_load_lds((attn_glb_t *)(src + vo), (attn_lds_t *)(Vh + g8 * 8 * VS), 16, 0, 0);
+            __builtin_amdgcn_global_load_lds((attn_glb_t *)(src + vo + lo), (attn_lds_t *)(Vl + g8 * 8 * VS), 16, 0, 0);
+        }
+        asm volatile("s_waitcnt vmcnt(0)" ::: "memory");
+        __syncthreads();
     };
     const bool single = Tk <= kc;
     const int q_end = cls_only ? 1 : T;
-    const float qscale = 0.125f * 1.44269504088896340736f;
     for (int qp0 = 0; qp0 < q_end; qp0 += 32 * NW) {
         const int qb0 = qp0 + w * 32;
         const bool active = qb0 < q_end;
         f16x8 qh[4], ql[4];
         {
-            const float *qp = qkv + (cls_only ? (size_t)s : (size_t)(tok0 + min(qb0 + i, T - 1))) * ld + h * HD + 32 * g;
-            f32x4 xq[8];
-#pragma unroll
-            for (int sx = 0; sx < 8; ++sx) xq[sx] = *reinterpret_cast<const f32x4 *>(qp + sx * 4);
-            if (single && qp0 == 0) {
-                stage(0, std::integral_constant<int, 4>{});
-                __syncthreads();
-            }
+            const _Float16 *qp = img + (cls_only ? (size_t)s : (size_t)(tok0 + min(qb0 + i, T - 1))) * ld + (2 * h + g) * 64;
 #pragma unroll
             for (int sx = 0; sx < 4; ++sx) {
-                f32x4 x0 = xq[2 * sx], x1 = xq[2 * sx + 1];
-                x0 = x0 * qscale;
-                x1 = x1 * qscale;
-                const f16x4 a0 = cvt_f16x4_pinned(x0), a1 = cvt_f16x4_pinned(x1);
-#pragma unroll
-                for (int j = 0; j < 4; ++j) {
-                    qh[sx][j] = a0[j]; qh[sx][4 + j] = a1[j];
-                    ql[sx][j] = (_Float16)((x0[j] - (float)a0[j]) * SC);
-                    ql[sx][4 + j] = (_Float16)((x1[j] - (float)a1[j]) * SC);
-                }
-            }
+                qh[sx] = *reinterpret_cast<const f16x8 *>(qp + sx * 8);
+                ql[sx] = *reinterpret_cast<const f16x8 *>(qp + 32 + sx * 8);
+            }
+            if (single && qp0 == 0) stage(0);
         }
         float m_run = -INFINITY, l_run = 0.0f;
         f32x16 om0 = {0}, om1 = {0}, oc0 = {0}, oc1 = {0};
         for (int k0 = 0; k0 < Tk; k0 += kc) {
             if (!single) {
                 __syncthreads();
-                stage(k0, std::integral_constant<int, 1>{});
-                __syncthreads();
+                stage(k0);
             }
             if (!active) continue;
             const int nkb = min(kc, Tk - k0) >> 5;
@@ -416,6 +380,17 @@
     }
 }
 
+__global__ void __launch_bounds__(256) qkv_image_kernel(const float *qkv, _Float16 *img, long long rows, int H) {
+    const int per_row = 3 * H / 8;
+    const long long e = (long long)blockIdx.x * 256 + threadIdx.x;
+    if (e >= rows * per_row) return;
+    const long long row = e / per_row;
+    const int n = (int)(e - row * per_row) * 8;
+    const float *p = qkv + row * (3 * H) + n;
+    attn_image_store8<false>(*reinterpret_cast<const f32x4 *>(p), *reinterpret_cast<const f32x4 *>(p + 4), n < H ? ATTN_QSCALE : 1.0f,
+                             img + row * (6 * H), n);
+}
+
 }
 
 size_t attention_split_lds_bytes(int max_seq_len) {
@@ -423,7 +398,7 @@
     return (size_t)2 * Tk * HD * 2 + (size_t)2 * Tk * VS * 2;
 }
 
-int launch_attention_split(const float *qkv, _Float16 *ctx_pair, const int4 *desc, int n_seq, int n_heads, int max_seq_len,
+int launch_attention_split(const _Float16 *qkv_image, _Float16 *ctx_pair, const int4 *desc, int n_seq, int n_heads, int max_seq_len,
                            int cls_only, hipStream_t st) {
     if (n_seq <= 0) return ANCE_OK;
     const int Tk = (max_seq_len + 31) & ~31;
@@ -439,9 +414,15 @@
             return check_launch("attention_split attr");
         if (tracked) __atomic_store_n(&attr_set[dev], lds, __ATOMIC_RELEASE);
     }
-    hipLaunchKernelGGL((attention_split_kernel<4>), dim3((unsigned)n_seq * n_heads), dim3(256), lds, st, qkv, ctx_pair, desc, n_heads,
-                       cls_only, kchunk);
+    hipLaunchKernelGGL((attention_split_kernel<4>), dim3((unsigned)n_seq * n_heads), dim3(256), lds, st, qkv_image, ctx_pair, desc,
+                       n_heads, cls_only, kchunk);
     return ANCE_OK;
+}
+
+void launch_qkv_image(const float *qkv, _Float16 *image, long long rows, int n_heads, hipStream_t st) {
+    const long long n = rows * (3 * n_heads * HD / 8);
+    if (n <= 0) return;
+    hipLaunchKernelGGL(qkv_image_kernel, dim3((unsigned)((n + 255) / 256)), dim3(256), 0, st, qkv, image, rows, n_heads * HD);
 }
 
 size_t attention_lds_bytes(int max_seq_len, int n_waves) {
@@ -472,16 +453,16 @@
 
 }
 
-extern "C" int ance_debug_attention(const AnceAttnDebugArgs *a, void *stream) {
+static int debug_attention(const AnceAttnDebugArgs *a, void *stream, bool image) {
     using namespace ance;
-    auto refuse = [](const char *why) {
+    auto refuse = [image](const char *why) {
         char buf[160];
-        snprintf(buf, sizeof(buf), "ance_debug_attention: invalid argument (%s)", why);
+        snprintf(buf, sizeof(buf), "%s: invalid argument (%s)", image ? "ance_debug_attention_pair" : "ance_debug_attention", why);
         set_last_error(buf);
         return ANCE_E_INVALID;
     };
     if (!a) return refuse("null args");
-    if (a->kind < 0 || a->kind > 2) return refuse("kind");
+    if (a->kind < 0 || a->kind > 2 || (image && a->kind != 1)) return refuse("kind");
     if (a->n_heads != 12 && a->n_heads != 16) return refuse("n_heads");
     if (a->n_seq < 1 || a->n_seq > (1 << 20)) return refuse("n_seq");
     if (a->max_seq_len < 1 || a->max_seq_len > 512) return refuse("max_seq_len");
@@ -494,7 +475,7 @@
     if (a->kind == 0) {
         if (a->ld_qk % 8 || a->ld_qk < 2 * H || a->ld_vt % 8 || a->ld_vt < 8 || a->ld_ctx % 8 || a->ld_ctx < H) return refuse("stride");
     } else {
-        if (a->ld_qk != 3 * H || a->ld_ctx != (a->kind == 1 ? 2 * H : H)) return refuse("stride");
+        if (a->ld_qk != (image ? 6 : 3) * H || a->ld_ctx != (a->kind == 1 ? 2 * H : H)) return refuse("stride");
     }
     if (a->kind == 2 && (a->cls_only || a->q_compact)) return refuse("cls_only on kind 2");
     if (a->kind == 1 && a->q_compact != a->cls_only) return refuse("kind 1: q_compact != cls_only");
@@ -531,11 +512,27 @@
         A.ld_qk = a->ld_qk; A.ld_vt = a->ld_vt; A.ld_ctx = a->ld_ctx; A.n_heads = a->n_heads;
         A.cls_only = a->cls_only ? 1 : 0; A.q_compact = a->q_compact ? 1 : 0;
         rc = launch_attention(A, a->n_seq, a->max_seq_len, st);
+    } else if (a->kind == 1 && image) {
+        rc = launch_attention_split((const _Float16 *)a->qk, (_Float16 *)a->ctx, (const int4 *)a->d_desc, a->n_seq, a->n_heads,
+                                    a->max_seq_len, a->cls_only ? 1 : 0, st);
     } else if (a->kind == 1) {
-        rc = launch_attention_split((const float *)a->qk, (_Float16 *)a->ctx, (const int4 *)a->d_desc, a->n_seq, a->n_heads,
-                                    a->max_seq_len, a->cls_only ? 1 : 0, st);
+        _Float16 *img = nullptr;
+        if (hipMalloc((void **)&img, (size_t)a->qk_rows * 6 * H * sizeof(_Float16)) != hipSuccess) {
+            set_last_error("ance_debug_attention: no memory for the Q | K | V image");
+            return ANCE_E_NOMEM;
+        }
+        launch_qkv_image((const float *)a->qk, img, a->qk_rows, a->n_heads, st);
+        rc = launch_attention_split(img, (_Float16 *)a->ctx, (const int4 *)a->d_desc, a->n_seq, a->n_heads, a->max_seq_len,
+                                    a->cls_only ? 1 : 0, st);
+        if (!rc) rc = check_launch("ance_debug_attention");
+        (void)hipStreamSynchronize(st);
+        (void)hipFree(img);
+        return rc;
     } else {
         rc = launch_attention32((const float *)a->qk, (float *)a->ctx, (const int *)a->d_desc, a->n_seq, a->n_heads, st);
     }
-    return rc ? rc : check_launch("ance_debug_attention");
-}
+    return rc ? rc : check_launch(image ? "ance_debug_attention_pair" : "ance_debug_attention");
+}
+
+extern "C" int ance_debug_attention(const AnceAttnDebugArgs *a, void *stream) { return debug_attention(a, stream, false); }
+extern "C" int ance_debug_attention_pair(const AnceAttnDebugArgs *a, void *stream) { return debug_attention(a, stream, true); }
diff --git a/ance_amd/csrc/common.h b/ance_amd/csrc/common.h
--- a/ance_amd/csrc/common.h
+++ b/ance_amd/csrc/common.h
@@ -84,6 +84,50 @@
                  (float)h[3] + (float)r[3] * PAIR_LO_INV};
 }
 
+constexpr float ATTN_QSCALE = 0.125f * 1.44269504088896340736f;
+constexpr float ATTN_LO_SCALE = 2048.0f, ATTN_LO_INV = 1.0f / 2048.0f;
+__device__ __forceinline__ void attn_split4(const f32x4 v, f16x4 *hi, f16x4 *lo) {
+#pragma clang fp contract(off)
+    const f16x4 h = cvt_f16x4_pinned(v);
+    *hi = h;
+#if defined(__HIP_DEVICE_COMPILE__)
+    typedef unsigned u32x2_t __attribute__((ext_vector_type(2)));
+    const u32x2_t hp = __builtin_bit_cast(u32x2_t, h);
+    const f32x4 w = v * ATTN_LO_SCALE;
+    const float ms = -ATTN_LO_SCALE;
+    u32x2_t lp;
+#pragma unroll
+    for (int j = 0; j < 2; ++j) {
+        unsigned r;
+        asm("v_fma_mixlo_f16 %0, %1, %2, %3 op_sel_hi:[1,0,0]" : "=v"(r) : "v"(hp[j]), "s"(ms), "v"(w[2 * j]));
+        asm("v_fma_mixhi_f16 %0, %1, %2, %3 op_sel:[1,0,0] op_sel_hi:[1,0,0]" : "+v"(r) : "v"(hp[j]), "s"(ms), "v"(w[2 * j + 1]));
+        lp[j] = r;
+    }
+    *lo = __builtin_bit_cast(f16x4, lp);
+#else
+    *lo = f16x4{(_Float16)((v[0] - (float)h[0]) * ATTN_LO_SCALE), (_Float16)((v[1] - (float)h[1]) * ATTN_LO_SCALE),
+                (_Float16)((v[2] - (float)h[2]) * ATTN_LO_SCALE), (_Float16)((v[3] - (float)h[3]) * ATTN_LO_SCALE)};
+#endif
+}
+template <bool NT>
+__device__ __forceinline__ void attn_image_store8(f32x4 va, f32x4 vb, float qs, _Float16 *row, int n) {
+#pragma clang fp contract(off)
+    va = va * qs;
+    vb = vb * qs;
+    f16x4 ha, ra, hb, rb;
+    attn_split4(va, &ha, &ra);
+    attn_split4(vb, &hb, &rb);
+    const f16x8 hi = f16x8{ha[0], ha[1], ha[2], ha[3], hb[0], hb[1], hb[2], hb[3]};
+    const f16x8 lo = f16x8{ra[0], ra[1], ra[2], ra[3], rb[0], rb[1], rb[2], rb[3]};
+    if constexpr (NT) {
+        __builtin_nontemporal_store(hi, reinterpret_cast<f16x8 *>(row + pair_hi_col(n, 0)));
+        __builtin_nontemporal_store(lo, reinterpret_cast<f16x8 *>(row + pair_lo_col(n, 0)));
+    } else {
+        *reinterpret_cast<f16x8 *>(row + pair_hi_col(n, 0)) = hi;
+        *reinterpret_cast<f16x8 *>(row + pair_lo_col(n, 0)) = lo;
+    }
+}
+
 constexpr float RANGE_LIMIT = 65504.0f;
 __device__ __forceinline__ void range_track4(const f32x4 v, float *mx) {
     float m = *mx;
diff --git a/ance_amd/csrc/encoder.hip b/ance_amd/csrc/encoder.hip
--- a/ance_amd/csrc/encoder.hip
+++ b/ance_amd/csrc/encoder.hip
@@ -90,7 +90,7 @@
         } f16;
         struct Split {
             Rows<FORM_PAIR> xa, xb;
-            float *qkv;
+            _Float16 *qkv;
             _Float16 *ctx, *ffn;
             Rows<FORM_PAIR> cls(int S_pad, int H) const { return {ffn, reinterpret_cast<float *>(ffn + (size_t)S_pad * 2 * H)}; }
         } sp;
@@ -208,7 +208,7 @@
         float *const ffn32 = wide ? a.take<float>(tcap * I) : nullptr;
         if (!e) continue;
         L.f16 = {{halves(preA), halves(preA) + tcap * H, partA}, {halves(preB), halves(preB) + tcap * H, partB}, qk16, vt16, ctx16, ffn16};
-        L.sp = {{halves(preA), partA}, {halves(preB), partB}, qkv32, halves(ctx32), halves(ffn32)};
+        L.sp = {{halves(preA), partA}, {halves(preB), partB}, halves(qkv32), halves(ctx32), halves(ffn32)};
         L.f32 = {{preA, statsA}, {preB, statsB}, h32, ha32, qkv32, ctx32, ffn32};
         e->lane[ln] = L;
     }
@@ -302,9 +302,10 @@
     return G;
 }
 template <int H>
-GemmArgs qkv_args(const Rows<FORM_PAIR> &x, int M, float eps, const LayerW &W, int c0, int n, float *qkv, unsigned *faults) {
+GemmArgs qkv_args(const Rows<FORM_PAIR> &x, int M, float eps, const LayerW &W, int c0, int n, _Float16 *qkv, unsigned *faults) {
     GemmArgs G = folded_args<H>(x, M, eps, W.wqkv_s + (size_t)c0 * 2 * H, n, W.bqkv_s + c0, W.cqkv_s + c0, W.sc_s + 4, faults);
-    G.out32 = qkv + c0; G.ldc = 3 * H;
+    G.out16 = qkv + pair_hi_col(c0, 3 * H); G.ldc = 2 * 3 * H;
+    G.scale_cols = c0 == 0 ? H : 0;
     return G;
 }
 
@@ -367,8 +368,8 @@
         {
             ProfScope ps(PC_GEMM_QK, st, tail ? 2.0 * T * (2.0 * H) * H + 2.0 * S * (double)H * H : 2.0 * T * (3.0 * H) * H);
             const int c0 = tail ? H : 0;
-            int rc = launch_gemm_f16(EPI_S_QKV, qkv_args<H>(V.xb, Tpad, eps_b, W, c0, 3 * H - c0, V.qkv, e->faults), st, H);
-            if (tail && !rc) rc = launch_gemm_f16(EPI_S_QKV, qkv_args<H>(cls, S_pad, eps_b, W, 0, H, V.qkv, e->faults), st, H);
+            int rc = launch_gemm_f16(EPI_S_QKV_PAIR, qkv_args<H>(V.xb, Tpad, eps_b, W, c0, 3 * H - c0, V.qkv, e->faults), st, H);
+            if (tail && !rc) rc = launch_gemm_f16(EPI_S_QKV_PAIR, qkv_args<H>(cls, S_pad, eps_b, W, 0, H, V.qkv, e->faults), st, H);
             if (rc) return rc;
         }
         {
diff --git a/ance_amd/csrc/gemm256_epilogue_split.h b/ance_amd/csrc/gemm256_epilogue_split.h
--- a/ance_amd/csrc/gemm256_epilogue_split.h
+++ b/ance_amd/csrc/gemm256_epilogue_split.h
@@ -51,6 +51,10 @@
         range_track4(a[h], vmax);
     }
     if constexpr (EPI == EPI_S_QKV) __builtin_nontemporal_store(a[0], reinterpret_cast<f32x4 *>(G.out32 + row * G.ldc + n));
+    else if constexpr (EPI == EPI_S_QKV_PAIR) {
+        const float qs = __builtin_amdgcn_readfirstlane(n) < G.scale_cols ? ATTN_QSCALE : 1.0f;
+        attn_image_store8<true>(a[0], a[NV - 1], qs, G.out16 + row * G.ldc, n);
+    }
     else epi_pair_store8_nt(a[0], a[NV - 1], G.out16 + row * G.ldc, G.N, n);
 }
 
@@ -150,7 +154,7 @@
 template <int EPI>
 __device__ __forceinline__ void gemm256_epilogue_split32(const GemmArgs &G, f32x4 (&acc)[4][8], float *slab, const float *stats,
                                                          const float *vec, int m0, int n0, int w, int l, float winv) {
-    static_assert(EPI == EPI_S_QKV || EPI == EPI_S_GELU, "the RESLN GEMMs run the launch-per-tile kernel (DESIGN_REJECTED.md round 6)");
+    static_assert(EPI == EPI_S_QKV || EPI == EPI_S_QKV_PAIR || EPI == EPI_S_GELU, "the RESLN GEMMs run the launch-per-tile kernel (DESIGN_REJECTED.md round 6)");
     const int i = l & 15, c4 = 4 * (l >> 4);
     const int wm = w >> 2, wn = w & 3;
     const int mw0 = m0 + wm * 128, nw0 = n0 + wn * 64;
diff --git a/ance_amd/csrc/gemm256_f16.hip b/ance_amd/csrc/gemm256_f16.hip
--- a/ance_amd/csrc/gemm256_f16.hip
+++ b/ance_amd/csrc/gemm256_f16.hip
@@ -217,6 +217,7 @@
     if (stream) {
         switch (epi) {
             case EPI_S_QKV: return gemm256_split_stream_kernel<EPI_S_QKV, HW>;
+            case EPI_S_QKV_PAIR: return gemm256_split_stream_kernel<EPI_S_QKV_PAIR, HW>;
             case EPI_S_GELU: return gemm256_split_stream_kernel<EPI_S_GELU, HW>;
             default: return nullptr;
         }
@@ -232,6 +233,7 @@
         case EPI_S_QKV: return gemm256_split_kernel<EPI_S_QKV, HW>;
         case EPI_S_GELU: return gemm256_split_kernel<EPI_S_GELU, HW>;
         case EPI_S_RESLN: return gemm256_split_kernel<EPI_S_RESLN, HW>;
+        case EPI_S_QKV_PAIR: return gemm256_split_kernel<EPI_S_QKV_PAIR, HW>;
         default: return nullptr;
     }
 }
@@ -251,7 +253,7 @@
     const unsigned blocks = (unsigned)gemm256_virtual_blocks(G);
     const int wi = hw == 1024 ? 1 : 0;
     const bool known = epi >= 0 && epi < EPI_COUNT && (hw == 768 || hw == 1024);
-    bool stream = (epi == EPI_S_QKV || epi == EPI_S_GELU) && gemm_stream_mode() == 1 && G.K >= 96 &&
+    bool stream = (epi == EPI_S_QKV || epi == EPI_S_QKV_PAIR || epi == EPI_S_GELU) && gemm_stream_mode() == 1 && G.K >= 96 &&
                   (uint64_t)G.M * (uint64_t)G.lda * 2u < (1ull << 31) && (uint64_t)G.N * (uint64_t)G.ldb * 2u < (1ull << 31);
 #ifdef ANCE_MEASURE
     const bool stamped = epi == g_gemm_stamps_epi && g_gemm_stamps_host;
diff --git a/ance_amd/csrc/gemm256_hooks.hip b/ance_amd/csrc/gemm256_hooks.hip
--- a/ance_amd/csrc/gemm256_hooks.hip
+++ b/ance_amd/csrc/gemm256_hooks.hip
@@ -75,6 +75,23 @@
     return rc ? rc : check_launch("ance_debug_gemm_hw");
 }
 
+extern "C" int ance_debug_gemm_qkv_pair(int hw, const AnceGemmDebugArgs *a, void *stream) {
+    using namespace ance;
+    if (!a || (hw != 768 && hw != 1024) || !a->a || !a->b || !a->bias || !a->csum || !a->part_in || !a->out || a->n_split != 0 ||
+        a->scale_cols < 0 || a->scale_cols % 64 != 0 || a->N <= 0 || a->ldc < 2 * a->N || a->ldc % 8 != 0 || (uintptr_t)a->out % 16 != 0) {
+        set_last_error("ance_debug_gemm_qkv_pair: invalid argument");
+        return ANCE_E_INVALID;
+    }
+    GemmArgs G;
+    memset(&G, 0, sizeof(G));
+    G.A = (const _Float16 *)a->a; G.B = (const _Float16 *)a->b; G.lda = a->lda; G.ldb = a->ldb;
+    G.M = a->M; G.N = a->N; G.K = a->K;
+    G.bias = a->bias; G.csum = a->csum; G.part_in = a->part_in; G.ln_eps = a->ln_eps;
+    G.scale_cols = a->scale_cols; G.ldc = a->ldc; G.out16 = (_Float16 *)a->out; G.wscale_inv = a->wscale_inv;
+    int rc = launch_gemm_f16(EPI_S_QKV_PAIR, G, (hipStream_t)stream, hw);
+    return rc ? rc : check_launch("ance_debug_gemm_qkv_pair");
+}
+
 extern "C" void ance_pair_layout(int n, int W, int *hi_col, int *lo_col, float *lo_scale) {
     if (hi_col) *hi_col = ance::pair_hi_col(n, W);
     if (lo_col) *lo_col = ance::pair_lo_col(n, W);
diff --git a/ance_amd/csrc/gemm_f16.h b/ance_amd/csrc/gemm_f16.h
--- a/ance_amd/csrc/gemm_f16.h
+++ b/ance_amd/csrc/gemm_f16.h
@@ -4,7 +4,7 @@
 namespace ance {
 
 enum { EPI_QK = 0, EPI_GELU = 1, EPI_RES32 = 2, EPI_VT = 3, EPI_RESLN = 4, EPI_QK_F = 5, EPI_GELU_F = 6, EPI_VT_F = 7,
-       EPI_S_QKV = 8, EPI_S_GELU = 9, EPI_S_RESLN = 10, EPI_COUNT = 11 };
+       EPI_S_QKV = 8, EPI_S_GELU = 9, EPI_S_RESLN = 10, EPI_S_QKV_PAIR = 11, EPI_COUNT = 12 };
 
 struct GemmArgs {
     const _Float16 *A;
diff --git a/include/ance_amd.h b/include/ance_amd.h
--- a/include/ance_amd.h
+++ b/include/ance_amd.h
@@ -379,6 +379,9 @@
 } AnceAttnDebugArgs;
 int ance_debug_attention(const AnceAttnDebugArgs *args, void *stream);
 
+int ance_debug_attention_pair(const AnceAttnDebugArgs *args, void *stream);
+int ance_debug_gemm_qkv_pair(int hw, const AnceGemmDebugArgs *args, void *stream);
+
 void ance_pair_layout(int n, int W, int *hi_col, int *lo_col, float *lo_scale);
 
 typedef struct AnceLambTensor {
```

Result: no change. 33660 passages/s (median of 6 runs) (+0.7%).
